# argsim/argsim

Hardware: AMD Instinct MI355X
Metric: sentences/sec per ELBO step (higher is better)
Workload: dtype f32; 1 GPU; BASELINE configs[1]: 1xMI355X fp32, latent_dim 128, vocab 8k, seq_len 64, batch 256 per GPU; FULL synthetic Zipf batches, dim_emb 512, 3 layers, step 20000; global_batch=256, seq_len=64, parallelism=dp1, gru=persistent

## Files before the change

### argsim_amd/csrc/ctx.h

```cpp
#pragma once
#include "../../include/argsim_vae.h"
#include "kernels.h"

#include <fcntl.h>
#include <sys/file.h>
#include <unistd.h>

#include <algorithm>
#include <cmath>
#include <cstdio>
#include <cstring>
#include <string>
#include <vector>

#pragma GCC visibility push(hidden)
namespace avae { namespace host {

struct ParamEntry {
    std::string name;
    int64_t offset;
    int ndim;
    int64_t shape[4];
    int g16;
    int bucket;
};

struct GruP { int64_t W, R, bW, bR; };

}}
#pragma GCC visibility pop

struct avae_ctx {
    avae_config cfg{};
    int device = 0;
    hipStream_t stream = nullptr;
    std::string err;
    std::vector<avae::host::ParamEntry> params;
    int64_t numel = 0;
    std::vector<std::pair<int64_t, int64_t>> buckets;
    float *P = nullptr, *G = nullptr, *M = nullptr, *Vv = nullptr;
    int64_t step = 0;
    avae_grad_hook hook = nullptr; void* hook_user = nullptr;
    std::vector<int> hook_pending;
    int persistent = 1;
    bool first_step_checked = false;
    int gru_ablate = 0, gru_force_slow = 0, gru_stagger = 0, gru_item = 2;
    int skinny = 1;
    int score_plan[4] = {0, 0, 0, 0};
    const int* expect_ptr[3] = {nullptr, nullptr, nullptr}; int expect_val[3] = {0, 0, 0};
    int compact = 2;
    int skip_pad = 1;
    int shared_device = 0; int lock_fd = -1;
    int dyn_split = 1;
    int dyn_thin = 1;
    int enc_top1 = 1;
    int table_l1 = 1;
    int bf16_act = 1;
    int bf16_sv = 1;
    int bf16_tn = 1;
    int logits16 = 1;
    int bf16_nt8 = 1;
    int bf16_direct = 0;
    int gru_spec = 2;
    int bwd_rs = 2;
    int knn_chunk = 0;
    int agg_chunk = 0;
    int ward_form = 0;
    int probe_chunk = 0;
    int gru_bf16 = 1;
    int64_t oE = 0, oKout = 0, oBout = 0, oWmu = 0, oBmu = 0, oWlv = 0, oBlv = 0, oWex = 0, oBex = 0;
    std::vector<avae::host::GruP> enc;
    std::vector<avae::host::GruP> dec;
    float* losses = nullptr;
    float* acc = nullptr;
    int* errw = nullptr;
    unsigned* counters = nullptr;
    float* scratch = nullptr;
    int64_t scratch_n = 0;
    char* ws = nullptr; size_t ws_cap = 0;
    int B = 0, Ss = 0, St = 0;
    int timing = 0, timing_on = 0;
    unsigned short *bfA = nullptr, *bfB = nullptr; size_t bfA_cap = 0, bfB_cap = 0;
    float* slab = nullptr; size_t slab_floats = 0;
    unsigned short* bfP = nullptr; size_t bfP_cap = 0;
    struct Stamp { hipEvent_t a, b; int cls; double flops; const int* dyn; int dyn_max; };
    std::vector<Stamp> stamps; size_t stamps_used = 0;
    int32_t* hint_dev = nullptr; volatile int32_t* hint_host = nullptr;
    const int32_t *cnt_src = nullptr, *cnt_tgt = nullptr;
};

#pragma GCC visibility push(hidden)
namespace avae { namespace host {

#define AV_CHECK(expr)                                                                              \
    do { hipError_t e_ = (expr); if (e_ != hipSuccess) {                                            \
        char b_[512]; snprintf(b_, sizeof b_, "%s:%d: %s -> %s", __FILE__, __LINE__, #expr, hipGetErrorString(e_)); \
        h->err = b_; return 1; } } while (0)
#define AV_TRY(expr) do { int r_ = (expr); if (r_) return r_; } while (0)

inline int fail(avae_ctx* h, const std::string& m) { h->err = m; return 1; }

#define AV_GRU(expr)                                                                                                \
    do { hipError_t e_ = (expr);                                                                                    \
         if (e_ == hipErrorCooperativeLaunchTooLarge)                                                               \
             return fail(h, "persistent GRU kernel: its workgroups cannot all be resident on this device at once (occupancy query x CU count < grid); " \
                            "run with avae_set_option(\"persistent\", 0)");                                         \
         if (e_ != hipSuccess) { char b_[512]; snprintf(b_, sizeof b_, "%s:%d: %s -> %s", __FILE__, __LINE__, #expr, hipGetErrorString(e_)); \
             h->err = b_; return 1; } } while (0)

struct DeviceTurn {
    avae_ctx* h; bool held = false;
    explicit DeviceTurn(avae_ctx* h_) : h(h_) {
        if (!h->shared_device || !h->persistent) return;
        if (h->lock_fd < 0) {
            char path[64]; snprintf(path, sizeof path, "/tmp/argsim_vae_dev%d.lock", h->device);
            h->lock_fd = open(path, O_CREAT | O_RDWR, 0666);
        }
        if (h->lock_fd >= 0 && flock(h->lock_fd, LOCK_EX) == 0) held = true;
    }
    ~DeviceTurn() { if (held) { (void)hipStreamSynchronize(h->stream); (void)flock(h->lock_fd, LOCK_UN); } }
};

struct Timed {
    avae_ctx* h; avae_ctx::Stamp* s = nullptr;
    Timed(avae_ctx* h_, int cls, double flops, const int* dyn = nullptr, int dyn_max = 0) : h(h_) {
        if (!h->timing) return;
        if (h->stamps_used == h->stamps.size()) {
            avae_ctx::Stamp n{};
            if (hipEventCreate(&n.a) != hipSuccess || hipEventCreate(&n.b) != hipSuccess) return;
            h->stamps.push_back(n);
        }
        s = &h->stamps[h->stamps_used++];
        s->cls = cls; s->flops = flops; s->dyn = dyn; s->dyn_max = dyn_max;
        (void)hipEventRecord(s->a, h->stream);
    }
    ~Timed() { if (s) (void)hipEventRecord(s->b, h->stream); }
};

struct Ws {
    int32_t *src_tm, *lens_src, *lens_tgt, *lead, *gold, *rank, *cidx, *ntok, *pred;
    float *emb_src, *emb_tgt, *ew, *dew;
    std::vector<float*> e_gi, e_hs, e_sv[2], e_hp[2];
    std::vector<float*> d_gi, d_hd, d_sv, d_hp;
    float *hpick, *mu, *lv, *z, *eps, *kld, *h0;
    float *xlast, *gib, *svb, *dgib, *dghb, *dxl;
    float *hc, *ho, *logits;
    float *loss_samp, *errt_samp;
    float *dho, *dhc, *dhd[2], *dgi_d, *dgh_d, *dh0, *carry, *dh0sum, *dz, *dmu, *dlv, *dhpick;
    float *dhs[2], *dgi_e, *dgh_e, *demb_src, *demb_tgt;
    std::vector<unsigned short*> e_hs16, d_hd16, e_hp16[2], d_hp16;
    std::vector<char> act_e, act_d, acth_e, acth_d;
    std::vector<unsigned short*> x16_e, x16_d;
    const unsigned short* x16_kept_e(int i) const { return x16_valid ? x16_e[i] : nullptr; }
    const unsigned short* x16_kept_d(int i) const { return x16_valid ? x16_d[i] : nullptr; }
    bool x16_valid = false;
    unsigned short *dgi16_d, *dgh16_d, *dgi16_e, *dgh16_e;
    int32_t* scat;
    int32_t *grp_src, *grp_tgt;
    int32_t *tokrow_src, *tokrow_tgt;
    float* xbuf; size_t xbuf_floats;
    int32_t *ord_perm[3], *ord_slens[3]; int ord_T[3], ord_cpj[3]; bool ord_ok[3];
    int32_t *map_src, *nact_src, *nsrc; bool compact;
    int32_t *map_tgt, *nact_tgt, *ntgt; bool compact_d;
    int Bx;
    int bx_enc() const { return compact ? Bx : 0; }
    int bx_dec() const { return compact_d ? Bx : 0; }
};

struct Bump {
    char* base; size_t off = 0;
    template <class T> T* take(size_t n) {
        off = (off + 255) & ~(size_t)255;
        T* p = base ? reinterpret_cast<T*>(base + off) : nullptr;
        off += n * sizeof(T);
        return p;
    }
    template <class T> T* opt(bool on, size_t n) { return on ? take<T>(n) : nullptr; }
};

struct Pair { const float* A; const float* B; float* C; const float* bias; };

struct GemmCall {
    const float* A; int lda; bool a_mc;
    const float* B; int ldb; bool b_nc;
    float* C; int ldc;
    int M, N, K;
    float alpha = 1.f; const float* bias = nullptr; int accumulate = 0;
    const int* dyn = nullptr; int dyn_kind = 0;
    const Pair* pair = nullptr;
    bool wgrad = false;
    bool allow_atomic = false;
    bool rows_are_batch = false;
    int thin = -1, split_k = 0;
    const unsigned short* A16 = nullptr; const unsigned short* B16 = nullptr;
    unsigned short* keep_a16 = nullptr;
    unsigned short* c16 = nullptr;

    GemmCall& scaled(float a) { alpha = a; return *this; }
    GemmCall& biased(const float* b) { bias = b; return *this; }
    GemmCall& plus() { accumulate = 1; return *this; }
    GemmCall& rows(const int* d) { dyn = d; dyn_kind = d ? 1 : 0; return *this; }
    GemmCall& depth(const int* d) { dyn = d; dyn_kind = d ? 2 : 0; return *this; }
    GemmCall& with(const Pair* p) { pair = p; return *this; }
    GemmCall& atomic() { allow_atomic = true; return *this; }
    GemmCall& batch_rows() { rows_are_batch = true; return *this; }
    GemmCall& form(int thin_, int split_k_ = 1) { thin = thin_; split_k = split_k_; return *this; }
    GemmCall& a16(const unsigned short* p) { A16 = p; return *this; }
    GemmCall& b16(const unsigned short* p) { B16 = p; return *this; }
    GemmCall& keep(unsigned short* p) { keep_a16 = p; return *this; }
};
inline GemmCall nt(const float* A, int lda, const float* B, int ldb, float* C, int ldc, int M, int N, int K) { return GemmCall{A, lda, false, B, ldb, false, C, ldc, M, N, K}; }
inline GemmCall nn(const float* A, int lda, const float* B, int ldb, float* C, int ldc, int M, int N, int K) { return GemmCall{A, lda, false, B, ldb, true, C, ldc, M, N, K}; }
inline GemmCall tn_grad(const float* A, int lda, const float* B, int ldb, float* C, int ldc, int M, int N, int K)
{
    GemmCall c{A, lda, true, B, ldb, true, C, ldc, M, N, K};
    c.wgrad = true;
// ... 59 lines not shown
```

### argsim_amd/csrc/gru.hip

```cpp
#include <algorithm>
#include "kernels.h"
#include "gru_dev.h"
#include <type_traits>

namespace avae {

template <int KS, bool STAMPS>
__global__ __launch_bounds__(256, 2) void gru_fwd_kernel(GruArgs a)
{
    constexpr int D = 16 * KS, HT = KS;
    constexpr int WK = 4 * KS;
    __shared__ __attribute__((aligned(16))) float part[2][2][4][3][256];
    __shared__ __attribute__((aligned(16))) float hps[2][2][16][16];

    const int tid = threadIdx.x, lane = tid & 63, wave = tid >> 6;
    const int n = lane & 15, kh = lane >> 4;
    int jb, g, ht;
    const bool second_half = wg_map(a, HT, &jb, &g, &ht);
    const GruJob& J = a.job[jb];
    const int B = a.B;
    const int row_beg = g * a.rows_per_group;
    const int row_end = min(B, row_beg + a.rows_per_group);
    const int ab = STAMPS ? a.ablate : 0;
    const bool one_sc = row_end - row_beg <= 32;
// ... 185 lines not shown
                 "buffer_load_dwordx4 %5, %8, %9, 0 offen offset:%c15 sc1\n\t"
                 "buffer_load_dwordx4 %6, %8, %9, 0 offen offset:%c16 sc1\n\t"
                 "buffer_load_dwordx4 %7, %8, %9, 0 offen offset:%c17 sc1"
                 : "=&v"(v[0]), "=&v"(v[1]), "=&v"(v[2]), "=&v"(v[3]), "=&v"(v[4]), "=&v"(v[5]), "=&v"(v[6]), "=&v"(v[7])
                 : "v"(voff), "s"(srd), "i"(OFF), "i"(OFF + 64), "i"(OFF + 128), "i"(OFF + 192), "i"(OFF + 256), "i"(OFF + 320),
                   "i"(OFF + 384), "i"(OFF + 448)
                 : "memory");
}
__device__ __forceinline__ void asm_wait8_all(u32x4 (&v)[8])
{
    asm volatile("s_waitcnt vmcnt(0)" : "+v"(v[0]), "+v"(v[1]), "+v"(v[2]), "+v"(v[3]), "+v"(v[4]), "+v"(v[5]), "+v"(v[6]), "+v"(v[7]) :: "memory");
}
__device__ __forceinline__ i32x4 make_srd(const float* p)
{
    const unsigned long long pa = (unsigned long long)p;
    return (i32x4){(int)(unsigned)(pa & 0xffffffffULL), (int)(unsigned)((pa >> 32) & 0xffffULL), -1, 0x00020000};
}

__global__ __launch_bounds__(256, 2) void gru_fwd_item_kernel(GruArgs a)
{
    constexpr int KS = 32, D = 512, HT = 32, WK = 128;
    __shared__ __attribute__((aligned(16))) float part[2][4][3][256];
    __shared__ __attribute__((aligned(16))) float hps[2][16][16];

    const int tid = threadIdx.x, lane = tid & 63, wave = tid >> 6;
    const int n = lane & 15, kh = lane >> 4;
    int jb, g, ht;
    const bool second_half = wg_map(a, HT, &jb, &g, &ht);
    const GruJob& J = a.job[jb];
    const int B = a.B;
    const int row_beg = g * 32;

    const bool bf = a.bf16 != 0;
    float w[3][KS];
#pragma unroll
    for (int gate = 0; gate < 3; ++gate) {
        const float* rp = J.R + (size_t)(ht * 48 + n * 3 + gate) * D + wave * WK;
#pragma unroll
        for (int q = 0; q < KS / 4; ++q) {
            float4 v = *reinterpret_cast<const float4*>(rp + 16 * q + 4 * kh);
            w[gate][4 * q + 0] = opnd(v.x, bf); w[gate][4 * q + 1] = opnd(v.y, bf); w[gate][4 * q + 2] = opnd(v.z, bf); w[gate][4 * q + 3] = opnd(v.w, bf);
        }
    }
    const int gn = tid & 15, gr = tid >> 4;
    const int j = ht * 16 + gn;
    float bR[3];
#pragma unroll
    for (int gate = 0; gate < 3; ++gate) bR[gate] = J.bR[ht * 48 + gn * 3 + gate];
    const int own_wave = (ht * 16) / WK, own_q = ((ht * 16) % WK) / 16;
    int len_a[2] = {0, 0}, len_g[2] = {0, 0};
    if (J.reverse) {
#pragma unroll
        for (int c = 0; c < 2; ++c) { len_a[c] = a.lens[row_beg + 16 * c + n]; len_g[c] = a.lens[row_beg + 16 * c + gr]; }
    }
    const i32x4 srd_hs = make_srd(J.hs), srd_h0 = make_srd(J.h0 ? J.h0 : J.hs);
    const bool fast = group_same_xcd(a.counters + 64 + jb * a.G + g, a.counters + 128 + (jb * a.G + g) * HT, ht, HT, a.err, a.force_slow);
    if (second_half) for (int i = 0; i < a.stagger; ++i) __builtin_amdgcn_s_sleep(32);

    const int total = 2 * (a.p_end - a.p_begin);
    auto item_off = [&](int it, bool* have, bool* from_h0) -> unsigned {
        const int p = a.p_begin + (it >> 1), c = it & 1;
        const int row = row_beg + 16 * c + n;
        *from_h0 = p == 0;
        *have = p > 0 || J.h0 != nullptr;
        if (p == 0) return (unsigned)((size_t)row * D * 4) + (wave * WK + 4 * kh) * 4;
        return (unsigned)((((size_t)pos_map(p - 1, len_a[c], J.reverse) * B + row) * a.ldh) * 4) + (wave * WK + 4 * kh) * 4;
    };
    u32x4 ra[2][8];
    {
        bool have, h0;
        const unsigned off = item_off(0, &have, &h0);
        if (have) asm_issue8<0>(ra[0], off, h0 ? srd_h0 : srd_hs);
        else {
#pragma unroll
            for (int q = 0; q < 8; ++q) ra[0][q] = (u32x4){0u, 0u, 0u, 0u};
        }
    }
    auto item = [&](int p, auto c_tag) __attribute__((always_inline)) {
        constexpr int c = decltype(c_tag)::value, buf = c;
        const int it = 2 * (p - a.p_begin) + c;
        u32x4 (&cur)[8] = ra[c];
        {
            bool have, h0;
            const unsigned off = item_off(it, &have, &h0);
            if (have) {
                asm_wait8_all(cur);
                if (p > a.p_begin) {
                    SpinGuard sg;
                    for (;;) {
                        unsigned mx = 0u;
#pragma unroll
                        for (int q = 0; q < 8; ++q) mx = max(max(mx, max(cur[q].x, cur[q].y)), max(cur[q].z, cur[q].w));
                        if (!__any(mx == kSentinel) || sg.expired(a.err)) break;
                        asm_issue8<0>(cur, off, srd_hs);
                        asm_wait8_all(cur);
                    }
                }
            }
        }
        if (it + 1 < total) {
            bool have, h0;
            const unsigned off = item_off(it + 1, &have, &h0);
            if (have) asm_issue8<0>(ra[c ^ 1], off, h0 ? srd_h0 : srd_hs);
            else {
#pragma unroll
                for (int q = 0; q < 8; ++q) ra[c ^ 1][q] = (u32x4){0u, 0u, 0u, 0u};
            }
        }
        const int grow = row_beg + 16 * c + gr;
        const int gpos = pos_map(p, len_g[c], J.reverse);
        const float* gp = J.gi + ((size_t)gpos * B + grow) * a.ldg + ht * 48 + gn * 3;
        const float gi0 = gp[0], gi1 = gp[1], gi2 = gp[2];
        f32x4 acc[3];
#pragma unroll
        for (int gate = 0; gate < 3; ++gate) acc[gate] = (f32x4){0.f, 0.f, 0.f, 0.f};
#pragma unroll
        for (int ks = 0; ks < KS; ++ks)
#pragma unroll
            for (int gate = 0; gate < 3; ++gate)
                acc[gate] = __builtin_amdgcn_mfma_f32_16x16x4f32(opnd(__uint_as_float(cur[ks >> 2][ks & 3]), bf), w[gate][ks], acc[gate], 0, 0, 0);
#pragma unroll
        for (int gate = 0; gate < 3; ++gate)
            *reinterpret_cast<f32x4*>(&part[buf][wave][gate][lane * 4]) = acc[gate];
        if (wave == own_wave) {
#pragma unroll
            for (int q = 0; q < 8; ++q)
                if (q == own_q) *reinterpret_cast<u32x4*>(&hps[buf][n][4 * kh]) = cur[q];
        }
        __syncthreads();
        {
            const int pidx = ((gr >> 2) * 16 + gn) * 4 + (gr & 3);
            float gh[3];
#pragma unroll
            for (int gate = 0; gate < 3; ++gate)
                gh[gate] = bR[gate] + ((part[buf][0][gate][pidx] + part[buf][1][gate][pidx]) + (part[buf][2][gate][pidx] + part[buf][3][gate][pidx]));
            const float hprev = hps[buf][gr][gn];
            const GruCellOut cell = gru_cell(gi0, gi1, gi2, gh[0], gh[1], gh[2], hprev);
            const float r = cell.r, u = cell.u, nn = cell.n, hnew = cell.h;
            const size_t rix = (size_t)gpos * B + grow;
            float* hdst = J.hs + rix * a.ldh + j;
            if (fast) *hdst = not_sentinel(hnew); else store4_sc1(hdst, not_sentinel(hnew));
            if (J.sv) *reinterpret_cast<float4*>(J.sv + (rix * HT + ht) * 64 + gn * 4) = make_float4(r, u, nn, gh[2]);
            if (J.hp) J.hp[rix * D + j] = hprev;
        }
    };
    for (int p = a.p_begin; p < a.p_end; ++p) {
        item(p, std::integral_constant<int, 0>{});
        item(p, std::integral_constant<int, 1>{});
    }
}


constexpr int kFwdTeamLdsBytes = (96 * 256 + 48 * 256 + 4 * 256) * 4 + 128;
template <bool DIAG, bool PIPE, int T, bool BF = false, bool CMP = false>
__global__ __launch_bounds__(1024, 4) void gru_fwd_team_kernel(GruArgs a)
{
    const int ab = DIAG ? a.ablate : 0;
    constexpr int D = 512, HT = 32, KS = 16 / T, WK = D / KS, NQ = WK / 16, RB = 16 * T;
    extern __shared__ __attribute__((aligned(16))) float lds[];
    float* Wl = lds;
    float* part = Wl + 96 * 256;
    float* hps = part + 48 * 256;
    unsigned* sync = reinterpret_cast<unsigned*>(hps + T * 256);

    const int tid = threadIdx.x, lane = tid & 63, wave = tid >> 6;
    int team, wk;
    if (T == 4 && PIPE && !CMP) { team = wave & 3; wk = wave >> 2; }
    else if (T == 4)         { team = wave >> 2; wk = wave & 3; }
    else if (PIPE && !CMP)   { team = (wave >> 1) & 1; wk = (wave & 1) + 2 * (wave >> 2); }
    else                     { team = (wave >> 2) & 1; wk = (wave & 3) + 4 * (wave >> 3); }
    const int n = lane & 15, kh = lane >> 4;
    const TeamMap tm = team_map(a, RB);
    const int cid = tm.cid, ht = tm.ht;
    const GruJob& J = a.job[tm.jb];
    const int Bs = a.B;
    const int B = (CMP && a.Bx > Bs) ? a.Bx : Bs;
    xcd_publish(a.counters + 64 + cid, a.counters + 128 + cid * HT, ht);

    if constexpr (BF) {
        for (int blk = wave; blk < 48; blk += 16) {
            const int wq = blk / (3 * (NQ / 2)), gate = (blk / (NQ / 2)) % 3, q2 = blk % (NQ / 2);
            const float* rp = J.R + (size_t)(ht * 48 + n * 3 + gate) * D + wq * WK + 32 * q2 + 8 * kh;
            const float4 v0 = *reinterpret_cast<const float4*>(rp), v1 = *reinterpret_cast<const float4*>(rp + 4);
            const u32x4 pk = {pack_bf16(v0.x, v0.y), pack_bf16(v0.z, v0.w), pack_bf16(v1.x, v1.y), pack_bf16(v1.z, v1.w)};
            *reinterpret_cast<u32x4*>(Wl + (size_t)blk * 256 + lane * 4) = pk;
        }
    } else
    for (int blk = wave; blk < 96; blk += 16) {
        const int wq = blk / (3 * NQ), gate = (blk / NQ) % 3, q = blk % NQ;
        const float4 v = *reinterpret_cast<const float4*>(J.R + (size_t)(ht * 48 + n * 3 + gate) * D + wq * WK + 16 * q + 4 * kh);
        *reinterpret_cast<float4*>(Wl + (size_t)blk * 256 + lane * 4) = v;
    }
    if (tid < 2 * T) sync[tid] = 0u;
    const int tt = wk * 64 + lane;
    const bool gate_thread = tt < 256;
    const int gn = tt & 15, gr = (tt >> 4) & 15;
    const int j = ht * 16 + gn;
    float bR[3];
#pragma unroll
    for (int gate = 0; gate < 3; ++gate) bR[gate] = J.bR[ht * 48 + gn * 3 + gate];
    const int own_wk = (ht * 16) / WK, own_q = ((ht * 16) % WK) / 16;
    const float* __restrict__ p_gi = J.gi;
    const int32_t* __restrict__ p_girows = J.gi_rows;
    float* __restrict__ p_svw = J.sv;
    float* __restrict__ p_hpw = J.hp;
    float* __restrict__ p_hsw = J.hs;
    float* const xh = BF ? a.xbuf + (size_t)tm.jb * (a.S + 1) * B * D / 2 : a.xbuf + (size_t)tm.jb * a.S * B * D;
    const __amdgpu_buffer_rsrc_t rs_hs = make_rsrc(xh), rs_h0 = make_rsrc(J.h0 ? J.h0 : xh);
    const __amdgpu_buffer_rsrc_t rs_gi = make_rsrc(p_gi), rs_hsw = make_rsrc(p_hsw);
    const __amdgpu_buffer_rsrc_t rs_svw = make_rsrc(p_svw ? p_svw : p_hsw), rs_hpw = make_rsrc(p_hpw ? p_hpw : p_hsw);
    unsigned short* __restrict__ p_hs16 = BF ? J.hs16 : nullptr;
    unsigned short* __restrict__ p_hp16 = BF ? J.hp16 : nullptr;
    const __amdgpu_buffer_rsrc_t rs_hs16 = make_rsrc(reinterpret_cast<const float*>(p_hs16 ? p_hs16 : reinterpret_cast<unsigned short*>(p_hsw)));
    const __amdgpu_buffer_rsrc_t rs_hp16 = make_rsrc(reinterpret_cast<const float*>(p_hp16 ? p_hp16 : reinterpret_cast<unsigned short*>(p_hsw)));
    auto to_bf16 = [](float v) -> unsigned short { return (unsigned short)(pack_bf16(v, 0.f) & 0xffffu); };
    const bool fast = group_same_xcd(a.counters + 64 + cid, a.counters + 128 + cid * HT, ht, HT, a.err, a.force_slow, true);
    float* tpart = part + team * (KS * 3 * 256);
    float* thps = hps + team * 256;
    unsigned* tsync = sync + team;
    unsigned* ready = sync + T + team;
    unsigned epoch = 0;
    if (ab & 256) { } else {
        const int tq = __builtin_amdgcn_readfirstlane(team);
        if (tq == 0) __builtin_amdgcn_s_setprio(3);
        else if (tq == 1) __builtin_amdgcn_s_setprio(2);
        else if (tq == 2) __builtin_amdgcn_s_setprio(1);
    }

    const bool stamp = (ab & 128) != 0;
    unsigned long long ph[8] = {0, 0, 0, 0, 0, 0, 0, 0}, tprev = __builtin_amdgcn_s_memrealtime();
#define TSTAMP(i) do { if (stamp) { unsigned long long t_ = __builtin_amdgcn_s_memrealtime(); ph[i] += t_ - tprev; tprev = t_; } } while (0)
    unsigned it = 0;
    constexpr int NQA = BF ? NQ / 2 : NQ;
    u32x4 ra[NQA];
    float hc = 0.f, hc0 = 0.f, hc1 = 0.f, hc2 = 0.f, hc3 = 0.f;
    const int* const lens_by_slot = a.slens ? a.slens : a.lens;
    const int* const perm = a.perm;
    auto a_offset = [&](int p, int row0, int len_a) -> unsigned {
        if constexpr (BF) return xch_lane_offset(p == 0 ? 0 : pos_map(p - 1, len_a, J.reverse) + 1, row0, wk * (WK / 8), n, kh, B, D / 2);
        if (p == 0) return (unsigned)((size_t)(CMP ? min(perm ? perm[row0 + n] : row0 + n, Bs - 1) : (perm ? perm[row0 + n] : row0 + n)) * D * 4) + (wk * WK + 4 * kh) * 4;
        return xch_lane_offset(pos_map(p - 1, len_a, J.reverse), row0, wk * (WK / 4), n, kh, B, D);
    };
    auto q_stride = [&](int p) -> unsigned { return (p == 0 && !BF) ? 64u : 1024u; };
    auto next_frag = [&](int p2, int r2, int len2) __attribute__((always_inline)) {
        if (BF || p2 > 0 || J.h0 != nullptr) {
            const int row2 = (tm.slot + r2 * tm.cpj) * RB + team * 16;
            frag_issue<NQA>(ra, (p2 == 0 && !BF) ? rs_h0 : rs_hs, a_offset(p2, row2, len2), q_stride(p2));
        } else {
#pragma unroll
            for (int q = 0; q < NQA; ++q) ra[q] = (u32x4){0u, 0u, 0u, 0u};
        }
    };
    int len_a = J.reverse ? lens_by_slot[tm.slot * RB + team * 16 + n] : 0, len_g = J.reverse ? lens_by_slot[tm.slot * RB + team * 16 + gr] : 0;
    const int len_p0 = J.reverse ? lens_by_slot[tm.slot * RB + team * 16 + 15] : 0;
    int nst0 = a.p_end, nst1 = a.p_end, nst2 = a.p_end, nst3 = a.p_end;
    if (a.slens) {
        nst3 = tm.nrb > 3 ? min(a.p_end, team_steps(a.slens, (tm.slot + 3 * tm.cpj) * RB + team * 16, lane)) : 0;
        nst2 = tm.nrb > 2 ? max(nst3, min(a.p_end, team_steps(a.slens, (tm.slot + 2 * tm.cpj) * RB + team * 16, lane))) : 0;
        nst1 = tm.nrb > 1 ? max(nst2, min(a.p_end, team_steps(a.slens, (tm.slot + 1 * tm.cpj) * RB + team * 16, lane))) : 0;
        nst0 = max(nst1, min(a.p_end, team_steps(a.slens, tm.slot * RB + team * 16, lane)));
    }
    auto nst_of = [&](int r) -> int { return r == 0 ? nst0 : (r == 1 ? nst1 : (r == 2 ? nst2 : nst3)); };
    const int p_stop = nst0;
    int ge_cur = tm.slot * RB + team * 16 + gr;
    if (perm) ge_cur = perm[ge_cur];
    const int* const rowmap = CMP ? a.rowmap : nullptr;
    if (a.slens && gate_thread && !rowmap) {
        for (int r = 0; r < tm.nrb; ++r) {
            const int gs = (tm.slot + r * tm.cpj) * RB + team * 16 + gr, ge = perm ? perm[gs] : gs;
            for (int p = nst_of(r); p < a.p_end; ++p) {
                const unsigned rix = (unsigned)p * (unsigned)Bs + (unsigned)ge;
                if (BF && p_hs16) __builtin_amdgcn_raw_buffer_store_b16((unsigned short)0, rs_hs16, (int)((rix * (unsigned)a.ldh + j) * 2u), 0, 0);
                else bstore1(0.f, rs_hsw, (rix * (unsigned)a.ldh + j) * 4u);
                if (BF && p_hp16) __builtin_amdgcn_raw_buffer_store_b16((unsigned short)0, rs_hp16, (int)((rix * D + j) * 2u), 0, 0);
                else if (p_hpw) bstore1(0.f, rs_hpw, (rix * D + j) * 4u);
            }
        }
    }
    if constexpr (PIPE) { if (a.p_begin < p_stop) next_frag(a.p_begin, 0, len_a); }
    for (int p = a.p_begin; p < p_stop; ++p) {
      for (int r = 0; r < tm.nrb && p < nst_of(r); ++r, ++it) {
        TSTAMP(5);
        const int row0 = (tm.slot + r * tm.cpj) * RB + team * 16;
        const bool poll = p > a.p_begin && !(ab & 16);
        const int grow = row0 + gr;
        const int gpos = pos_map(p, len_g, J.reverse);
        const unsigned prix = (unsigned)gpos * (unsigned)Bs + (unsigned)ge_cur;
        const int crow = (rowmap && gate_thread) ? (ge_cur < Bs ? rowmap[prix] : -1) : (int)prix;
        const bool real = !CMP || crow >= 0;
        const unsigned rix = (unsigned)crow;
        float gi0 = 0.f, gi1 = 0.f, gi2 = 0.f, h0_own = 0.f;
        if (gate_thread && real) {
            const unsigned grix = p_girows ? (unsigned)p_girows[prix] : rix;
            const u32x3 g3 = __builtin_amdgcn_raw_buffer_load_b96(rs_gi, (int)((grix * (unsigned)a.ldg + ht * 48 + gn * 3) * 4u), 0, 0);
            gi0 = __uint_as_float(g3.x); gi1 = __uint_as_float(g3.y); gi2 = __uint_as_float(g3.z);
            if constexpr (BF) { if (p == 0 && J.h0 != nullptr) h0_own = bload1(rs_h0, ((unsigned)ge_cur * D + j) * 4u); }
        }
        const bool same_p = r + 1 < tm.nrb && p < nst_of(r + 1);
        const int r2 = same_p ? r + 1 : 0, p2 = same_p ? p : p + 1;
        int len2 = len_a, len2g = len_g, ge2 = ge_cur;
        if constexpr (PIPE) {
            if (p2 < p_stop) {
                const int row2 = (tm.slot + r2 * tm.cpj) * RB + team * 16;
                if (J.reverse) { len2 = lens_by_slot[row2 + n]; len2g = lens_by_slot[row2 + gr]; }
                ge2 = perm ? perm[row2 + gr] : row2 + gr;
            }
        }
        const bool have = BF || p > 0 || J.h0 != nullptr;
        if (have) {
            const unsigned aoff = a_offset(p, row0, len_a);
            const __amdgpu_buffer_rsrc_t rs = (p == 0 && !BF) ? rs_h0 : rs_hs;
            if constexpr (!PIPE) {
                bool got = false;
                if (poll && a.spec) {
                    frag_issue<NQA>(ra, rs, aoff, q_stride(p));
                    if constexpr (BF) got = !frag_bad16<NQA>(ra); else got = !frag_bad<NQA>(ra);
                }
                if (poll) {
                    if (wk == 0) {
                        if (!got) {
                        const int prow = row0 + 15;
                        const int plen = len_p0;
                        const float* pp = BF ? xh + (xch16_index(pos_map(p - 1, plen, J.reverse) + 1, prow, (lane & 31) * 16 + 15, B, D) >> 1)
                                             : xh + xch_index(pos_map(p - 1, plen, J.reverse), prow, (lane & 31) * 16 + 15, B, D);
                        SpinGuard sg;
                        while (__any(BF ? (load4_sc1(pp) >> 16) == 0xffffu : load4_sc1(pp) == kSentinel) && !sg.expired(a.err)) { }
                        }
                        if (lane == 0) __hip_atomic_store(ready, it + 1u, __ATOMIC_RELAXED, __HIP_MEMORY_SCOPE_WORKGROUP);
                    } else if (!got) {
                        while (__hip_atomic_load(ready, __ATOMIC_RELAXED, __HIP_MEMORY_SCOPE_WORKGROUP) < it + 1u) __builtin_amdgcn_s_sleep(1);
                    }
                }
                if (!got) frag_issue<NQA>(ra, rs, aoff, q_stride(p));
            }
            if (poll) { if constexpr (BF) frag_ensure16<NQA>(ra, rs, aoff, a.err, q_stride(p)); else frag_ensure<NQA>(ra, rs, aoff, a.err, q_stride(p)); }
        } else if constexpr (!PIPE) {
#pragma unroll
            for (int q = 0; q < NQA; ++q) ra[q] = (u32x4){0u, 0u, 0u, 0u};
        }
        TSTAMP(0);
        f32x4 acc[3];
#pragma unroll
        for (int gate = 0; gate < 3; ++gate) acc[gate] = (f32x4){0.f, 0.f, 0.f, 0.f};
        if constexpr (BF) {
#pragma unroll
            for (int q2 = 0; q2 < NQ / 2; ++q2) {
                const bf16x8 a8 = __builtin_bit_cast(bf16x8, ra[q2]);
#pragma unroll
                for (int gate = 0; gate < 3; ++gate) {
                    const bf16x8 b8 = __builtin_bit_cast(bf16x8, *reinterpret_cast<const u32x4*>(Wl + (size_t)((wk * 3 + gate) * (NQ / 2) + q2) * 256 + lane * 4));
                    acc[gate] = __builtin_amdgcn_mfma_f32_16x16x32_bf16(a8, b8, acc[gate], 0, 0, 0);
                }
            }
        } else
        {
            f32x4 bn[3];
#pragma unroll
            for (int gate = 0; gate < 3; ++gate)
                bn[gate] = *reinterpret_cast<const f32x4*>(Wl + (size_t)((wk * 3 + gate) * NQ + 0) * 256 + lane * 4);
#pragma unroll
            for (int q = 0; q < NQ; ++q) {
                f32x4 b[3];
#pragma unroll
                for (int gate = 0; gate < 3; ++gate) b[gate] = bn[gate];
                if (q + 1 < NQ) {
#pragma unroll
                    for (int gate = 0; gate < 3; ++gate)
                        bn[gate] = *reinterpret_cast<const f32x4*>(Wl + (size_t)((wk * 3 + gate) * NQ + q + 1) * 256 + lane * 4);
                }
                __builtin_amdgcn_sched_barrier(0);
#pragma unroll
                for (int e = 0; e < 4; ++e)
#pragma unroll
                    for (int gate = 0; gate < 3; ++gate)
                        acc[gate] = __builtin_amdgcn_mfma_f32_16x16x4f32(__uint_as_float(ra[q][e]), b[gate][e], acc[gate], 0, 0, 0);
                __builtin_amdgcn_sched_barrier(0);
            }
        }
        TSTAMP(1);
        if (it > 0) { epoch += KS; team_barrier(tsync, epoch); }
        TSTAMP(6);
#pragma unroll
        for (int gate = 0; gate < 3; ++gate)
            *reinterpret_cast<f32x4*>(tpart + (wk * 3 + gate) * 256 + lane * 4) = acc[gate];
        if constexpr (!BF) {
            if (wk == own_wk) {
#pragma unroll
                for (int q = 0; q < NQ; ++q)
                    if (q == own_q) *reinterpret_cast<u32x4*>(thps + n * 16 + 4 * kh) = ra[q];
            }
        }
        if constexpr (PIPE) {
            asm volatile("" :: "v"(gi0), "v"(gi1), "v"(gi2), "v"(h0_own), "v"(len2), "v"(len2g), "v"(ge2));
            __builtin_amdgcn_sched_barrier(0);
            if (p2 < p_stop) next_frag(p2, r2, len2);
            __builtin_amdgcn_sched_barrier(0);
        }
        TSTAMP(7);
        epoch += KS; team_barrier(tsync, epoch);
        TSTAMP(2);
        if (gate_thread) {
            const int pidx = ((gr >> 2) * 16 + gn) * 4 + (gr & 3);
            float gh[3];
#pragma unroll
            for (int gate = 0; gate < 3; ++gate) {
                float s4[4] = {0.f, 0.f, 0.f, 0.f};
#pragma unroll
                for (int k = 0; k < KS; ++k) s4[k & 3] += tpart[(k * 3 + gate) * 256 + pidx];
                gh[gate] = bR[gate] + ((s4[0] + s4[1]) + (s4[2] + s4[3]));
            }
            float hprev;
            if constexpr (BF) {
                if (p == 0) hprev = h0_own;
                else if constexpr (PIPE) hprev = r == 0 ? hc0 : (r == 1 ? hc1 : (r == 2 ? hc2 : hc3));
                else hprev = hc;
            } else hprev = thps[gr * 16 + gn];
            const GruCellOut cell = gru_cell(gi0, gi1, gi2, gh[0], gh[1], gh[2], hprev);
            const float r_ = cell.r, u = cell.u, nn = cell.n, hnew = cell.h;
            if constexpr (BF) {
                const unsigned xo = xch16_index(gpos + 1, grow, j, B, D) * 2u;
                if (fast) __builtin_amdgcn_raw_buffer_store_b16(bf16_not_sentinel(hnew), rs_hs, (int)xo, 0, 0);
                else __builtin_amdgcn_raw_buffer_store_b16(bf16_not_sentinel(hnew), rs_hs, (int)xo, 0, 16);
                if constexpr (PIPE) { if (r == 0) hc0 = hnew; else if (r == 1) hc1 = hnew; else if (r == 2) hc2 = hnew; else hc3 = hnew; }
                else hc = hnew;
            } else {
                const unsigned xo = xch_index(gpos, grow, j, B, D) * 4u;
                if (fast) bstore1(not_sentinel(hnew), rs_hs, xo); else bstore1_sc1(not_sentinel(hnew), rs_hs, xo);
            }
            if (real) {
            if (BF && p_hs16) __builtin_amdgcn_raw_buffer_store_b16(to_bf16(hnew), rs_hs16, (int)((rix * (unsigned)a.ldh + j) * 2u), 0, 0);
            else bstore1(hnew, rs_hsw, (rix * (unsigned)a.ldh + j) * 4u);
            if (p_svw) {
                if (BF && a.sv16) {
                    typedef unsigned u32x2 __attribute__((ext_vector_type(2)));
                    const u32x2 s2 = {pack_bf16(r_, u), pack_bf16(nn, gh[2])};
                    __builtin_amdgcn_raw_buffer_store_b64(s2, rs_svw, (int)(((rix * HT + ht) * 64 + gn * 4) * 2u), 0, 0);
                } else bstore4(r_, u, nn, gh[2], rs_svw, ((rix * HT + ht) * 64 + gn * 4) * 4u);
            }
            if (BF && p_hp16) __builtin_amdgcn_raw_buffer_store_b16(to_bf16(hprev), rs_hp16, (int)((rix * D + j) * 2u), 0, 0);
            else if (p_hpw) bstore1(hprev, rs_hpw, (rix * D + j) * 4u);
            }
        }
        len_a = len2; len_g = len2g; ge_cur = ge2;
        TSTAMP(3);
      }
    }
    if (stamp && tt == 0 && a.stamps) {
        for (int i = 0; i < 8; ++i) atomicAdd(a.stamps + i, ph[i]);
        atomicAdd(a.stamps + 8, (unsigned long long)(a.p_end - a.p_begin));
        atomicAdd(a.stamps + 10, 1ULL);
    }
#undef TSTAMP
}

template <int KS, bool STAMPS>
__global__ __launch_bounds__(256, 2) void gru_bwd_kernel(GruArgs a)
{
    constexpr int D = 16 * KS, HT = KS, NKS = 3 * KS;
    __shared__ __attribute__((aligned(16))) float part[2][2][4][256];
    __shared__ float red[4][16];

    const int tid = threadIdx.x, lane = tid & 63, wave = tid >> 6;
    const int n = lane & 15, kh = lane >> 4;
    int jb, g, ht;
    const bool second_half = wg_map(a, HT, &jb, &g, &ht);
    const GruJob& J = a.job[jb];
    const int B = a.B, S = a.S;
    const int row_beg = g * a.rows_per_group;
    const int row_end = min(B, row_beg + a.rows_per_group);
    const int ab = STAMPS ? a.ablate : 0;
    const bool one_sc = row_end - row_beg <= 32;

    const bool bf = a.bf16 != 0;
    float w[NKS];
#pragma unroll
    for (int ks = 0; ks < NKS; ++ks)
        w[ks] = opnd(J.R[(size_t)(wave * 12 * KS + kperm<NKS>(ks, kh)) * D + ht * 16 + n], bf);

    const int gn = tid & 15, gr = tid >> 4;
    const int j = ht * 16 + gn;
    int len_a[2] = {0, 0}, len_g[2] = {0, 0};
    if (J.reverse) {
#pragma unroll
        for (int c = 0; c < 2; ++c) {
            len_a[c] = a.lens[min(row_beg + 16 * c + n, B - 1)];
            len_g[c] = a.lens[min(row_beg + 16 * c + gr, B - 1)];
        }
    }
    const bool want_dh0 = (J.dh0 != nullptr) && a.p_begin == 0;
    const int p_last = want_dh0 ? -1 : a.p_begin;
    const __amdgpu_buffer_rsrc_t rs_dgh = make_rsrc(J.dgh);
    float sb_r = 0.f, sb_u = 0.f, sb_n = 0.f, sb_nr = 0.f;
    bool fast = false;
    if (a.p_end - 1 > p_last && !(ab & 16))
        fast = group_same_xcd(a.counters + 64 + jb * a.G + g, a.counters + 128 + (jb * a.G + g) * HT, ht, HT, a.err, a.force_slow);
    if (second_half && a.p_end - 1 > p_last) for (int i = 0; i < a.stagger; ++i) __builtin_amdgcn_s_sleep(32);
    int buf = 0, done = 0;
    unsigned long long ph[8] = {0, 0, 0, 0, 0, 0, 0, 0}, tprev = __builtin_amdgcn_s_memrealtime();
    for (int p = a.p_end - 1; p >= p_last; --p, ++done) {
        const bool have_next = (p + 1 < S);
        const bool poll = done > 0 && !(ab & 16);
        for (int rb = row_beg; rb < row_end; rb += 32, buf ^= 1) {
            AVAE_STAMP(7);
            float s_r[2], s_u[2], s_n[2], s_hn[2], s_hp[2], s_do[2]; int rix[2]; bool gok[2];
#pragma unroll
            for (int c = 0; c < 2; ++c) {
                const int row = rb + 16 * c + gr;
                gok[c] = row < row_end && p >= 0;
                rix[c] = 0; s_r[c] = s_u[c] = s_n[c] = s_hn[c] = s_hp[c] = s_do[c] = 0.f;
                if (gok[c]) {
                    const int len = J.reverse ? (one_sc ? len_g[c] : a.lens[row]) : 0;
                    rix[c] = pos_map(p, len, J.reverse) * B + row;
                    if (!(ab & 2)) {
                        const float4 sv = *reinterpret_cast<const float4*>(J.sv + ((size_t)rix[c] * HT + ht) * 64 + gn * 4);
                        s_r[c] = sv.x; s_u[c] = sv.y; s_n[c] = sv.z; s_hn[c] = sv.w;
                        s_hp[c] = J.hp[(size_t)rix[c] * D + j];
                        if (J.dh_out) s_do[c] = J.dh_out[(size_t)rix[c] * a.ldh + j];
                    }
                }
            }
            AVAE_STAMP(0);
            const bool c1 = rb + 16 < row_end;
            constexpr int NH = (NKS % 16 == 0) ? 4 : ((NKS % 8 == 0) ? 2 : 1);
            constexpr int HK = NKS / NH;
            constexpr int PQ = (NKS % 4 == 0) ? HK / 4 : 1;
            constexpr int NB = 3;
            u32x4 hv[NB][PQ];
            float hs_[HK];
            auto piece_off = [&](int c, int hf) -> unsigned {
                const int row = min(rb + 16 * c + n, B - 1);
                const int len = J.reverse ? (one_sc ? len_a[c] : a.lens[row]) : 0;
                const int pos1 = pos_map(p + 1, len, J.reverse);
                return (unsigned)((((size_t)pos1 * B + row) * a.ldg + wave * 12 * KS + hf * 4 * HK) * 4);
            };
            const bool do_mm = have_next && !(ab & 1);
            const int nstage = (c1 ? 2 : 1) * NH;
            f32x4 acc[4];
            if constexpr (KS == 32) {
                if (!do_mm) {
#pragma unroll
                    for (int c = 0; c < 2; ++c)
                        if (c == 0 || c1) *reinterpret_cast<f32x4*>(&part[buf][c][wave][lane * 4]) = (f32x4){0.f, 0.f, 0.f, 0.f};
                } else {
                    const unsigned long long pa = (unsigned long long)J.dgh;
                    const i32x4 srd = {(int)(unsigned)(pa & 0xffffffffULL), (int)(unsigned)((pa >> 32) & 0xffffULL), -1, 0x00020000};
                    const unsigned voff0 = piece_off(0, 0) + 16 * kh, voff1 = c1 ? piece_off(1, 0) + 16 * kh : voff0;
                    auto pass = [&](auto nst_tag) __attribute__((always_inline)) -> bool {
                        constexpr int NST = decltype(nst_tag)::value;
                        unsigned mx = 0u;
                        asm_issue6<0>(hv[0], voff0, srd);
                        asm_issue6<384>(hv[1], voff0, srd);
#pragma unroll
                        for (int st = 0; st < NST; ++st) {
                            const int c = st / NH, hf = st % NH;
                            if (st + 2 < NST) {
                                const unsigned vo = ((st + 2) / NH) ? voff1 : voff0;
                                if ((st + 2) % NH == 0) asm_issue6<0>(hv[(st + 2) % NB], vo, srd);
                                if ((st + 2) % NH == 1) asm_issue6<384>(hv[(st + 2) % NB], vo, srd);
                                if ((st + 2) % NH == 2) asm_issue6<768>(hv[(st + 2) % NB], vo, srd);
                                if ((st + 2) % NH == 3) asm_issue6<1152>(hv[(st + 2) % NB], vo, srd);
                            }
                            if (st + 2 < NST) asm_wait6<12>(hv[st % NB]);
                            else if (st + 1 < NST) asm_wait6<6>(hv[st % NB]);
                            else asm_wait6<0>(hv[st % NB]);
                            if (hf == 0) {
#pragma unroll
                                for (int i = 0; i < 4; ++i) acc[i] = (f32x4){0.f, 0.f, 0.f, 0.f};
                            }
#pragma unroll
                            for (int q = 0; q < PQ; ++q)
                                mx = max(max(mx, max(hv[st % NB][q].x, hv[st % NB][q].y)), max(hv[st % NB][q].z, hv[st % NB][q].w));
                            asm volatile("" : "+v"(mx));
#pragma unroll
                            for (int ks = 0; ks < HK; ++ks)
                                acc[ks & 3] = __builtin_amdgcn_mfma_f32_16x16x4f32(opnd(__uint_as_float(hv[st % NB][ks >> 2][ks & 3]), bf),
                                                                                   w[ks + hf * HK], acc[ks & 3], 0, 0, 0);
                            if (hf == NH - 1) {
                                f32x4 s = (acc[0] + acc[1]) + (acc[2] + acc[3]);
                                *reinterpret_cast<f32x4*>(&part[buf][c][wave][lane * 4]) = s;
                            }
                        }
                        return __any(mx == kSentinel);
                    };
                    SpinGuard sg;
                    for (;;) {
                        if (poll) {
                            const int pc = c1 ? (lane >> 5) : 0, prow = min(min(rb + 16 * pc + 15, row_end - 1), B - 1);
                            const int plen = J.reverse ? a.lens[prow] : 0;
                            const float* pp = J.dgh + ((size_t)pos_map(p + 1, plen, J.reverse) * B + prow) * a.ldg + (lane & 31) * 48 + 47;
                            while (__any(load4_sc1(pp) == kSentinel) && !sg.expired(a.err)) { }
                        }
                        const bool bad = c1 ? pass(std::integral_constant<int, 2 * NH>{}) : pass(std::integral_constant<int, NH>{});
                        if (!poll || !bad || sg.expired(a.err)) break;
                    }
                }
            } else {
            if constexpr (NKS % 4 == 0) {
                if (do_mm) {
#pragma unroll
                    for (int s0 = 0; s0 < NB - 1; ++s0)
                        if (s0 < nstage) frag_issue<PQ>(hv[s0], rs_dgh, piece_off(s0 / NH, s0 % NH) + 16 * kh);
                }
            }
#pragma unroll
            for (int c = 0; c < 2; ++c) {
#pragma unroll
                for (int hf = 0; hf < NH; ++hf) {
                    const int st = c * NH + hf;
                    if (st < nstage) {
                        if (hf == 0) {
#pragma unroll
                            for (int i = 0; i < 4; ++i) acc[i] = (f32x4){0.f, 0.f, 0.f, 0.f};
                        }
                        if (do_mm) {
                            if constexpr (NKS % 4 == 0) {
                                if (st + NB - 1 < nstage)
                                    frag_issue<PQ>(hv[(st + NB - 1) % NB], rs_dgh, piece_off((st + NB - 1) / NH, (st + NB - 1) % NH) + 16 * kh);
                                if (poll) frag_ensure<PQ>(hv[st % NB], rs_dgh, piece_off(c, hf) + 16 * kh, a.err);
#pragma unroll
                                for (int ks = 0; ks < HK; ++ks)
                                    acc[ks & 3] = __builtin_amdgcn_mfma_f32_16x16x4f32(opnd(__uint_as_float(hv[st % NB][ks >> 2][ks & 3]), bf),
                                                                                       w[ks + hf * HK], acc[ks & 3], 0, 0, 0);
                            } else {
                                load_frag_scalar<HK, NKS>(hs_, J.dgh + piece_off(c, 0) / 4, hf * HK, kh, poll, a.err);
#pragma unroll
                                for (int ks = 0; ks < HK; ++ks)
                                    acc[ks & 3] = __builtin_amdgcn_mfma_f32_16x16x4f32(opnd(hs_[ks], bf), w[ks + hf * HK], acc[ks & 3], 0, 0, 0);
                            }
                        }
                        if (hf == NH - 1) {
                            f32x4 s = (acc[0] + acc[1]) + (acc[2] + acc[3]);
                            *reinterpret_cast<f32x4*>(&part[buf][c][wave][lane * 4]) = s;
                        }
                    }
                }
            }
            }
            AVAE_STAMP(2);
            __syncthreads();
            AVAE_STAMP(3);
            float o_dr[2], o_du[2], o_dn[2], o_car[2];
#pragma unroll
            for (int c = 0; c < 2; ++c) {
                const int row = rb + 16 * c + gr;
                if (row >= row_end) continue;
                const int pidx = ((gr >> 2) * 16 + gn) * 4 + (gr & 3);
                float carried = (part[buf][c][0][pidx] + part[buf][c][1][pidx]) + (part[buf][c][2][pidx] + part[buf][c][3][pidx]);
                float* carryp = J.carry + (size_t)row * D + j;
                if (have_next) carried += *carryp;
                if (p < 0) { J.dh0[(size_t)row * D + j] = carried; continue; }
                const float dH = carried + s_do[c];
                const float r = s_r[c], u = s_u[c], nn = s_n[c];
                const float dn = dH * (1.f - u) * (1.f - nn * nn);
                const float du = dH * (s_hp[c] - nn) * u * (1.f - u);
                const float dr = dn * s_hn[c] * r * (1.f - r);
                float* dgh = J.dgh + (size_t)rix[c] * a.ldg + ht * 48 + gn * 3;
                const float x0 = not_sentinel(dr), x1 = not_sentinel(du), x2 = not_sentinel(dn * r);
                if (fast) { dgh[0] = x0; dgh[1] = x1; dgh[2] = x2; }
                else { store4_sc1(dgh, x0); store4_sc1(dgh + 1, x1); store4_sc1(dgh + 2, x2); }
                o_dr[c] = dr; o_du[c] = du; o_dn[c] = dn; o_car[c] = dH * u;
                sb_r += dr; sb_u += du; sb_n += dn; sb_nr += dn * r;
            }
            AVAE_STAMP(4);
            if (p >= 0) {
#pragma unroll
                for (int c = 0; c < 2; ++c) {
                    const int row = rb + 16 * c + gr;
                    if (row >= row_end) continue;
                    J.carry[(size_t)row * D + j] = o_car[c];
                    if (!(ab & 4)) {
                        float* dgi = J.dgi + (size_t)rix[c] * a.ldg + ht * 48 + gn * 3;
                        dgi[0] = o_dr[c]; dgi[1] = o_du[c]; dgi[2] = o_dn[c];
                    }
                }
            }
            AVAE_STAMP(6);
        }
    }
    if (STAMPS && tid == 0 && a.stamps) {
        for (int i = 0; i < 8; ++i) atomicAdd(a.stamps + 16 + i, ph[i]);
        atomicAdd(a.stamps + 16 + 8, (unsigned long long)(a.p_end - a.p_begin));
        atomicAdd(a.stamps + 16 + 9, (unsigned long long)(fast ? 1 : 0));
        atomicAdd(a.stamps + 16 + 10, 1ULL);
    }
    if (J.dbW || J.dbR) {
        if (tid < 64) red[tid >> 4][tid & 15] = 0.f;
        __syncthreads();
        atomicAdd(&red[0][gn], sb_r); atomicAdd(&red[1][gn], sb_u); atomicAdd(&red[2][gn], sb_n); atomicAdd(&red[3][gn], sb_nr);
        __syncthreads();
        if (tid < 48) {
            const int gate = tid >> 4, u = tid & 15;
            if (J.dbW) atomicAdd(J.dbW + ht * 48 + u * 3 + gate, red[gate][u]);
            if (J.dbR) atomicAdd(J.dbR + ht * 48 + u * 3 + gate, red[gate == 2 ? 3 : gate][u]);
        }
    }
}

constexpr int kBwdTeamLdsBytes = (4 * 24 * 256 + 16 * 256 + 64) * 4 + 64;
template <int NB, bool PIPE, int T, bool DIAG = false, bool BF = false, bool CMP = false>
__global__ __launch_bounds__(1024, 4) void gru_bwd_team_kernel(GruArgs a)
{
    unsigned long long ph[8] = {0, 0, 0, 0, 0, 0, 0, 0}, tprev = DIAG ? __builtin_amdgcn_s_memrealtime() : 0ULL;
#define BSTAMP(i) do { if constexpr (DIAG) { unsigned long long t_ = __builtin_amdgcn_s_memrealtime(); ph[i] += t_ - tprev; tprev = t_; } } while (0)
    constexpr int D = 512, HT = 32, PQ = 6, KS = 16 / T, WKB = 3 * D / KS, KPL = BF ? 32 : 16, NH = WKB / (PQ * KPL), KB4 = 96 / KS, RB = 16 * T;
    extern __shared__ __attribute__((aligned(16))) float lds[];
    float* Wl = lds;
    float* part = Wl + 96 * 256;
    float* red = part + 16 * 256;
    unsigned* sync = reinterpret_cast<unsigned*>(red + 64);

    const int tid = threadIdx.x, lane = tid & 63, wave = tid >> 6;
    int team, wk;
    if (T == 4 && PIPE && !CMP) { team = wave & 3; wk = wave >> 2; }
    else if (T == 4)         { team = wave >> 2; wk = wave & 3; }
    else if (PIPE && !CMP)   { team = (wave >> 1) & 1; wk = (wave & 1) + 2 * (wave >> 2); }
    else                     { team = wave >> 3; wk = wave & 7; }
    const int n = lane & 15, kh = lane >> 4;
    const TeamMap tm = team_map(a, RB);
    const int cid = tm.cid, ht = tm.ht;
    const GruJob& J = a.job[tm.jb];
    const int Bs = a.B, S = a.S;
    const int B = (CMP && a.Bx > Bs) ? a.Bx : Bs;
    xcd_publish(a.counters + 64 + cid, a.counters + 128 + cid * HT, ht);

    auto r_row = [&](int kx) -> const float* { const int rem = kx % 48; return J.R + (size_t)((kx - rem) + (rem & 15) * 3 + (rem >> 4)) * D + ht * 16 + n; };
    if constexpr (BF) {
        for (int blk = wave; blk < 48; blk += 16) {
            const int wq = blk / (KB4 / 2), kp = blk % (KB4 / 2);
            const float* r0 = r_row(wq * WKB + 32 * kp + 8 * kh);
            const u32x4 pk = {pack_bf16(r0[0], r0[3 * D]), pack_bf16(r0[6 * D], r0[9 * D]), pack_bf16(r0[12 * D], r0[15 * D]), pack_bf16(r0[18 * D], r0[21 * D])};
            *reinterpret_cast<u32x4*>(Wl + (size_t)blk * 256 + lane * 4) = pk;
        }
    } else
    for (int blk = wave; blk < 96; blk += 16) {
        const int wq = blk / KB4, ks4 = blk % KB4;
        const float* rp = r_row(wq * WKB + 16 * ks4 + 4 * kh);
        *reinterpret_cast<float4*>(Wl + (size_t)blk * 256 + lane * 4) = make_float4(rp[0], rp[3 * D], rp[6 * D], rp[9 * D]);
    }
    if (tid < 2 * T) sync[tid] = 0u;
    if (tid < 64) red[tid] = 0.f;
    const int tt = wk * 64 + lane, gn = tt & 15, gr = (tt >> 4) & 15;
    const bool gate_thread = tt < 256;
    const int j = ht * 16 + gn;
    unsigned long long tp0 = 0, tp1 = 0;
    if constexpr (DIAG) { asm volatile("s_waitcnt vmcnt(0) lgkmcnt(0)" ::: "memory"); tp0 = __builtin_amdgcn_s_memrealtime(); }
    const bool fast = group_same_xcd(a.counters + 64 + cid, a.counters + 128 + cid * HT, ht, HT, a.err, a.force_slow, true);
    if constexpr (DIAG) {
        tp1 = __builtin_amdgcn_s_memrealtime();
        if (tt == 0 && a.stamps && ((a.ablate & 256) ? T == 2 : T == 4)) {
            atomicAdd(a.stamps + 16 + 11, tp0 - tprev);
            atomicAdd(a.stamps + 16 + 12, tp1 - tp0);
        }
    }
    float* tpart = part + team * (KS * 256);
    unsigned* tsync = sync + team;
    unsigned* ready = sync + T + team;
    unsigned epoch = 0;
    {
        const int tq = __builtin_amdgcn_readfirstlane(team);
        if (tq == 0) __builtin_amdgcn_s_setprio(3);
        else if (tq == 1) __builtin_amdgcn_s_setprio(2);
        else if (tq == 2) __builtin_amdgcn_s_setprio(1);
    }
    const float* __restrict__ p_sv = J.sv;
    const float* __restrict__ p_hp = J.hp;
    const float* __restrict__ p_do = J.dh_out;
    float* __restrict__ p_dgi = J.dgi;
    float* __restrict__ p_dghw = J.dgh;
    unsigned short* __restrict__ p_dgi16 = BF ? J.dgi16 : nullptr;
    unsigned short* __restrict__ p_dgh16 = BF ? J.dgh16 : nullptr;
    float* p_dh0 = J.dh0;
    float* p_carry = J.carry;
    const int* p_lens = a.slens ? a.slens : a.lens;
    const int* const perm = a.perm;
    int* p_err = a.err;
    const int j_rev = J.reverse, ldg = a.ldg, ldh = a.ldh;
    float* const xg = a.xbuf + (size_t)tm.jb * S * B * (3 * D) / (BF ? 2 : 1);
    const unsigned long long pa = (unsigned long long)xg;
    const i32x4 srd = {(int)(unsigned)(pa & 0xffffffffULL), (int)(unsigned)((pa >> 32) & 0xffffULL), -1, 0x00020000};
    float sb_r = 0.f, sb_u = 0.f, sb_n = 0.f, sb_nr = 0.f;
    const bool want_dh0 = (p_dh0 != nullptr) && a.p_begin == 0;
    const int p_last = want_dh0 ? -1 : a.p_begin;
    int done = 0;
    unsigned it = 0;
    float carry_reg = 0.f;
    float carry_r0 = 0.f, carry_r1 = 0.f, carry_r2 = 0.f, carry_r3 = 0.f;
    u32x4 hv[NB][PQ];
    const __amdgpu_buffer_rsrc_t rs_dgh = make_rsrc(xg);
    const __amdgpu_buffer_rsrc_t rs_sv = make_rsrc(p_sv), rs_hp = make_rsrc(p_hp), rs_do = make_rsrc(p_do ? p_do : p_hp);
    const unsigned short* __restrict__ p_hp16 = BF ? J.hp16 : nullptr;
    const __amdgpu_buffer_rsrc_t rs_hp16 = make_rsrc(reinterpret_cast<const float*>(p_hp16 ? p_hp16 : reinterpret_cast<const unsigned short*>(p_hp)));
    const __amdgpu_buffer_rsrc_t rs_dgi = make_rsrc(p_dgi), rs_dghw = make_rsrc(p_dghw);
    const __amdgpu_buffer_rsrc_t rs_dgi16 = make_rsrc(reinterpret_cast<const float*>(p_dgi16 ? p_dgi16 : reinterpret_cast<unsigned short*>(p_dgi)));
    const __amdgpu_buffer_rsrc_t rs_dgh16 = make_rsrc(reinterpret_cast<const float*>(p_dgh16 ? p_dgh16 : reinterpret_cast<unsigned short*>(p_dghw)));
    auto a_offset = [&](int p, int row0, int len_a) -> unsigned {
        if constexpr (BF) return xch_lane_offset(pos_map(p + 1, len_a, j_rev), row0, wk * (WKB / 8), n, kh, B, 3 * D / 2);
        return xch_lane_offset(pos_map(p + 1, len_a, j_rev), row0, wk * (WKB / 4), n, kh, B, 3 * D);
    };
    auto issue_piece = [&](int piece, u32x4 (&dst)[PQ], unsigned vo) __attribute__((always_inline)) {
        asm_issue6x(dst, vo, srd, 6144 * piece, 6144 * piece + 4096);
    };
    auto head = [&](unsigned vo) __attribute__((always_inline)) {
#pragma unroll
        for (int s0 = 0; s0 < NB && s0 < NH; ++s0) issue_piece(s0, hv[s0], vo);
    };
    int nst0 = a.p_end, nst1 = a.p_end, nst2 = a.p_end, nst3 = a.p_end;
    if (a.slens) {
        nst3 = tm.nrb > 3 ? min(a.p_end, team_steps(a.slens, (tm.slot + 3 * tm.cpj) * RB + team * 16, lane)) : 0;
        nst2 = tm.nrb > 2 ? max(nst3, min(a.p_end, team_steps(a.slens, (tm.slot + 2 * tm.cpj) * RB + team * 16, lane))) : 0;
        nst1 = tm.nrb > 1 ? max(nst2, min(a.p_end, team_steps(a.slens, (tm.slot + 1 * tm.cpj) * RB + team * 16, lane))) : 0;
        nst0 = max(nst1, min(a.p_end, team_steps(a.slens, tm.slot * RB + team * 16, lane)));
    }
    auto nst_of = [&](int r) -> int { return r == 0 ? nst0 : (r == 1 ? nst1 : (r == 2 ? nst2 : nst3)); };
    auto next_head = [&](int p2, int r2, int len2) __attribute__((always_inline)) {
        if (p2 + 1 < nst_of(r2)) {
            const int row2 = (tm.slot + r2 * tm.cpj) * RB + team * 16;
            const unsigned vo2 = a_offset(p2, row2, len2);
#pragma unroll
            for (int s0 = 0; s0 < NB && s0 < NH; ++s0)
#pragma unroll
                for (int q = 0; q < PQ; ++q) hv[s0][q] = load16_sc1(rs_dgh, vo2 + 6144u * s0 + 1024u * q);
        }
    };
    int len_a = j_rev ? p_lens[tm.slot * RB + team * 16 + n] : 0, len_g = j_rev ? p_lens[tm.slot * RB + team * 16 + gr] : 0;
    const int len_p0 = j_rev ? p_lens[tm.slot * RB + team * 16 + 15] : 0;
    int ge_cur = tm.slot * RB + team * 16 + gr;
    if (perm) ge_cur = perm[ge_cur];
    const int* const rowmap = CMP ? a.rowmap : nullptr;
    const bool dgi_by_pos = rowmap != nullptr && J.dgi_by_pos != 0;
    if (a.slens && gate_thread && (!rowmap || dgi_by_pos)) {
        for (int r = 0; r < tm.nrb; ++r) {
            const int gs = (tm.slot + r * tm.cpj) * RB + team * 16 + gr, ge = perm ? perm[gs] : gs;
            if (CMP && ge >= Bs) continue;
            for (int p = nst_of(r); p < a.p_end; ++p) {
                const unsigned orow = (((unsigned)p * (unsigned)Bs + (unsigned)ge) * (unsigned)ldg + ht * 48 + gn * 3) * 4u;
                if (BF && p_dgh16 != nullptr) {
                    if ((gn & 1) == 0) {
                        const u32x3 z3 = {0u, 0u, 0u};
                        if (!rowmap) __builtin_amdgcn_raw_buffer_store_b96(z3, rs_dgh16, (int)(orow >> 1), 0, 0);
                        if (p_dgi16 != nullptr) __builtin_amdgcn_raw_buffer_store_b96(z3, rs_dgi16, (int)(orow >> 1), 0, 0);
                    }
                    if (p_dgi16 == nullptr) bstore3(0.f, 0.f, 0.f, rs_dgi, orow);
                } else { if (!rowmap) bstore3(0.f, 0.f, 0.f, rs_dghw, orow); bstore3(0.f, 0.f, 0.f, rs_dgi, orow); }
            }
        }
    }
    const int p_first = nst0 - 1;
    if constexpr (PIPE) next_head(p_first, 0, len_a);
    for (int p = p_first; p >= p_last; --p, ++done) {
      for (int r = 0; r < tm.nrb && (p < 0 || p < nst_of(r)); ++r, ++it) {
        const int row0 = (tm.slot + r * tm.cpj) * RB + team * 16;
        int gn_l = gn, gr_l = gr, ln_l = lane;
        asm volatile("" : "+v"(gn_l), "+v"(gr_l), "+v"(ln_l));
        const int grow = row0 + gr_l, j_l = ht * 16 + gn_l;
        const bool have_next = p + 1 < nst_of(r);
        const bool poll = done > 0 && !(DIAG && (a.ablate & 16));
        const bool same_p = r + 1 < tm.nrb && (p < 0 || p < nst_of(r + 1));
        const int r2 = same_p ? r + 1 : 0, p2 = same_p ? p : p - 1;
        int len2 = len_a, len2g = len_g, ge2 = ge_cur;
        if constexpr (PIPE) {
            if (p2 >= p_last) {
                const int row2 = (tm.slot + r2 * tm.cpj) * RB + team * 16;
                if (j_rev) { len2 = p_lens[row2 + n]; len2g = p_lens[row2 + gr]; }
                ge2 = perm ? perm[row2 + gr] : row2 + gr;
            }
        }
        BSTAMP(7);
        const int gpos = pos_map(p < 0 ? 0 : p, len_g, j_rev);
        const unsigned prix = (unsigned)gpos * (unsigned)Bs + (unsigned)ge_cur;
        const bool inb = !CMP || ge_cur < Bs;
        const int crow = (rowmap && gate_thread && p >= 0) ? (inb ? rowmap[prix] : -1) : (int)prix;
        const bool real = !CMP || crow >= 0;
        const unsigned rix = (unsigned)crow;
        float4 sv = make_float4(0.f, 0.f, 0.f, 0.f); float s_hp = 0.f, s_do = 0.f;
        if (p >= 0 && gate_thread && real) {
            if (BF && a.sv16) {
                typedef unsigned u32x2 __attribute__((ext_vector_type(2)));
                const u32x2 s2 = __builtin_amdgcn_raw_buffer_load_b64(rs_sv, (int)(((rix * HT + ht) * 64 + gn_l * 4) * 2u), 0, 0);
                sv = make_float4(__uint_as_float(s2.x << 16), __uint_as_float(s2.x & 0xffff0000u), __uint_as_float(s2.y << 16), __uint_as_float(s2.y & 0xffff0000u));
            } else
            sv = bload4(rs_sv, ((rix * HT + ht) * 64 + gn_l * 4) * 4u);
            if (BF && p_hp16) s_hp = __uint_as_float((unsigned)(unsigned short)__builtin_amdgcn_raw_buffer_load_b16(rs_hp16, (int)((rix * D + j_l) * 2u), 0, 0) << 16);
            else s_hp = bload1(rs_hp, (rix * D + j_l) * 4u);
            s_do = p_do ? bload1(rs_do, (rix * (unsigned)ldh + j_l) * 4u) : 0.f;
        }
        float* carryp = p_carry + (size_t)grow * D + j_l;
        float s_carry = 0.f;
        if constexpr (PIPE) {
            if (done == 0 && have_next && gate_thread) { const float c0 = *carryp; if (r == 0) carry_r0 = c0; else if (r == 1) carry_r1 = c0; else if (r == 2) carry_r2 = c0; else carry_r3 = c0; }
            s_carry = r == 0 ? carry_r0 : (r == 1 ? carry_r1 : (r == 2 ? carry_r2 : carry_r3));
        }
        else { if (done == 0 && have_next && gate_thread) carry_reg = *carryp; }
        BSTAMP(0);
        f32x4 sum = {0.f, 0.f, 0.f, 0.f};
        if (have_next) {
            const unsigned voff = a_offset(p, row0, len_a);
            f32x4 acc[2];
            auto pass = [&]() __attribute__((always_inline)) -> bool {
                unsigned mx = 0u;
                auto ldsB = [&](int st_, int q_) __attribute__((always_inline)) {
                    return *reinterpret_cast<const f32x4*>(Wl + (size_t)((wk * KB4 + st_ * 6 + q_) * 64 + lane) * 4);
                };
                f32x4 bq = {0.f, 0.f, 0.f, 0.f};
                if constexpr (!BF) bq = ldsB(0, 0);
#pragma unroll
                for (int st = 0; st < NH; ++st) {
                    const int issued = (NB + st < NH) ? NB + st : NH;
                    const int younger = issued - 1 - st;
                    if (younger == 2) asm_wait6<12>(hv[st % NB]);
                    else if (younger == 1) asm_wait6<6>(hv[st % NB]);
                    else asm_wait6<0>(hv[st % NB]);
                    if (st == 0) { acc[0] = (f32x4){0.f, 0.f, 0.f, 0.f}; acc[1] = (f32x4){0.f, 0.f, 0.f, 0.f}; }
#pragma unroll
                    for (int q = 0; q < PQ; ++q) {
                        if constexpr (BF) mx = pk_max_u16(pk_max_u16(mx, pk_max_u16(hv[st % NB][q].x, hv[st % NB][q].y)), pk_max_u16(hv[st % NB][q].z, hv[st % NB][q].w));
                        else mx = max(max(mx, max(hv[st % NB][q].x, hv[st % NB][q].y)), max(hv[st % NB][q].z, hv[st % NB][q].w));
                    }
                    asm volatile("" : "+v"(mx));
                    if constexpr (BF) {
#pragma unroll
                        for (int q = 0; q < PQ; ++q) {
                            const bf16x8 b8 = __builtin_bit_cast(bf16x8, *reinterpret_cast<const u32x4*>(Wl + (size_t)((wk * (KB4 / 2) + st * PQ + q) * 64 + lane) * 4));
                            acc[q & 1] = __builtin_amdgcn_mfma_f32_16x16x32_bf16(__builtin_bit_cast(bf16x8, hv[st % NB][q]), b8, acc[q & 1], 0, 0, 0);
                        }
                    } else
#pragma unroll
                    for (int q = 0; q < PQ; ++q) {
                        const f32x4 b = bq;
                        if (q + 1 < PQ) bq = ldsB(st, q + 1); else if (st + 1 < NH) bq = ldsB(st + 1, 0);
                        __builtin_amdgcn_sched_barrier(0);
#pragma unroll
                        for (int e = 0; e < 4; ++e)
                            acc[e & 1] = __builtin_amdgcn_mfma_f32_16x16x4f32(__uint_as_float(hv[st % NB][q][e]), b[e], acc[e & 1], 0, 0, 0);
                        __builtin_amdgcn_sched_barrier(0);
                    }
                    if (st + NB < NH) issue_piece(st + NB, hv[st % NB], voff);
                }
                sum = acc[0] + acc[1];
                if constexpr (BF) return __any(any_half_sentinel(mx));
                return __any(mx == kSentinel);
            };
            auto probe = [&](SpinGuard& sg) __attribute__((always_inline)) {
                const int len_p = PIPE ? (j_rev ? p_lens[row0 + 15] : 0) : len_p0;
                const float* pp = BF ? xg + (xch16_index(pos_map(p + 1, len_p, j_rev), row0 + 15, (ln_l & 31) * 48 + 47, B, 3 * D) >> 1)
                                     : xg + xch_index(pos_map(p + 1, len_p, j_rev), row0 + 15, (ln_l & 31) * 48 + 47, B, 3 * D);
                for (;;) {
                    unsigned v = 0u;
                    if (ln_l < 32) v = load4_sc1(pp);
                    if (!__any(BF ? (v >> 16) == 0xffffu : v == kSentinel) || sg.expired(p_err)) break;
                }
            };
            SpinGuard sg;
            if constexpr (!PIPE) {
                if (poll) {
                    if (wk == 0) {
                        probe(sg);
                        if (lane == 0) __hip_atomic_store(ready, it + 1u, __ATOMIC_RELAXED, __HIP_MEMORY_SCOPE_WORKGROUP);
                    } else {
                        while (__hip_atomic_load(ready, __ATOMIC_RELAXED, __HIP_MEMORY_SCOPE_WORKGROUP) < it + 1u) __builtin_amdgcn_s_sleep(1);
                    }
                }
                head(voff);
            }
            BSTAMP(1);
            for (;;) {
                const bool bad = pass();
                if (!poll || !bad || sg.expired(p_err)) break;
                probe(sg);
                head(voff);
            }
        }
        if constexpr (PIPE) {
            asm volatile("" :: "v"(sv.x), "v"(sv.y), "v"(sv.z), "v"(sv.w), "v"(s_hp), "v"(s_do), "v"(s_carry), "v"(len2), "v"(len2g), "v"(ge2));
            __builtin_amdgcn_sched_barrier(0);
            if (p2 >= p_last) next_head(p2, r2, len2);
            __builtin_amdgcn_sched_barrier(0);
        }
        BSTAMP(2);
        if (it > 0) { epoch += KS; team_barrier(tsync, epoch); }
        BSTAMP(3);
        *reinterpret_cast<f32x4*>(tpart + wk * 256 + lane * 4) = sum;
        BSTAMP(4);
        epoch += KS; team_barrier(tsync, epoch);
        BSTAMP(5);
        if (gate_thread) {
            const int pidx = ((gr >> 2) * 16 + gn) * 4 + (gr & 3);
            float s4[4] = {0.f, 0.f, 0.f, 0.f};
#pragma unroll
            for (int k = 0; k < KS; ++k) s4[k & 3] += tpart[k * 256 + pidx];
            float carried = (s4[0] + s4[1]) + (s4[2] + s4[3]);
            if constexpr (PIPE) carried += s_carry;
            else if (have_next) carried += carry_reg;
            if (p < 0) { if (inb) p_dh0[(size_t)ge_cur * D + j_l] = carried; len_a = len2; len_g = len2g; ge_cur = ge2; continue; }
            const float dH = carried + s_do;
            const float r_ = sv.x, u = sv.y, nn = sv.z;
            const float dn = dH * (1.f - u) * (1.f - nn * nn);
            const float du = dH * (s_hp - nn) * u * (1.f - u);
            const float dr = dn * sv.w * r_ * (1.f - r_);
            if constexpr (BF) {
                const unsigned short x0 = bf16_not_sentinel(dr), x1 = bf16_not_sentinel(du), x2 = bf16_not_sentinel(dn * r_);
                const unsigned o0 = xch16_index(gpos, grow, ht * 48 + gn_l, B, 3 * D) * 2u;
                if (fast) {
                    __builtin_amdgcn_raw_buffer_store_b16(x0, rs_dgh, (int)o0, 0, 0); __builtin_amdgcn_raw_buffer_store_b16(x1, rs_dgh, (int)(o0 + 512u), 0, 0);
                    __builtin_amdgcn_raw_buffer_store_b16(x2, rs_dgh, (int)(o0 + 1024u), 0, 0);
                } else {
                    __builtin_amdgcn_raw_buffer_store_b16(x0, rs_dgh, (int)o0, 0, 16); __builtin_amdgcn_raw_buffer_store_b16(x1, rs_dgh, (int)(o0 + 512u), 0, 16);
                    __builtin_amdgcn_raw_buffer_store_b16(x2, rs_dgh, (int)(o0 + 1024u), 0, 16);
                }
            } else {
                const float x0 = not_sentinel(dr), x1 = not_sentinel(du), x2 = not_sentinel(dn * r_);
                const unsigned o0 = xch_index(gpos, grow, ht * 48 + gn_l, B, 3 * D) * 4u;
                if (fast) { bstore1(x0, rs_dgh, o0); bstore1(x1, rs_dgh, o0 + 1024u); bstore1(x2, rs_dgh, o0 + 2048u); }
                else { bstore1_sc1(x0, rs_dgh, o0); bstore1_sc1(x1, rs_dgh, o0 + 1024u); bstore1_sc1(x2, rs_dgh, o0 + 2048u); }
            }
            const unsigned orow = (rix * (unsigned)ldg + ht * 48 + gn_l * 3) * 4u;
            const unsigned orow_i = dgi_by_pos ? (prix * (unsigned)ldg + ht * 48 + gn_l * 3) * 4u : orow;
            if (BF && p_dgh16 != nullptr) {
                const float dnr = dn * r_;
                const float o_r = __int_as_float(__builtin_amdgcn_update_dpp(0, __float_as_int(dr), 0xF5, 0xF, 0xF, false));
                const float o_u = __int_as_float(__builtin_amdgcn_update_dpp(0, __float_as_int(du), 0xF5, 0xF, 0xF, false));
                const float o_n = __int_as_float(__builtin_amdgcn_update_dpp(0, __float_as_int(dn), 0xF5, 0xF, 0xF, false));
                const float o_nr = __int_as_float(__builtin_amdgcn_update_dpp(0, __float_as_int(dnr), 0xF5, 0xF, 0xF, false));
                if ((gn_l & 1) == 0) {
                    const u32x3 vh = {pack_bf16(dr, du), pack_bf16(dnr, o_r), pack_bf16(o_u, o_nr)};
                    const u32x3 vi = {pack_bf16(dr, du), pack_bf16(dn, o_r), pack_bf16(o_u, o_n)};
                    if (real) __builtin_amdgcn_raw_buffer_store_b96(vh, rs_dgh16, (int)(orow >> 1), 0, 0);
                    if (p_dgi16 != nullptr && (real || (dgi_by_pos && inb))) __builtin_amdgcn_raw_buffer_store_b96(vi, rs_dgi16, (int)(orow_i >> 1), 0, 0);
                }
                if (p_dgi16 == nullptr && (real || (dgi_by_pos && inb))) bstore3(dr, du, dn, rs_dgi, orow_i);
                if constexpr (PIPE) { const float c1 = dH * u; if (r == 0) carry_r0 = c1; else if (r == 1) carry_r1 = c1; else if (r == 2) carry_r2 = c1; else carry_r3 = c1; }
                else carry_reg = dH * u;
            } else {
            if (real) bstore3(dr, du, dn * r_, rs_dghw, orow);
            if constexpr (PIPE) { const float c1 = dH * u; if (r == 0) carry_r0 = c1; else if (r == 1) carry_r1 = c1; else if (r == 2) carry_r2 = c1; else carry_r3 = c1; }
            else carry_reg = dH * u;
            if (real || (dgi_by_pos && inb)) bstore3(dr, du, dn, rs_dgi, orow_i);
            }
            sb_r += dr; sb_u += du; sb_n += dn; sb_nr += dn * r_;
        }
        len_a = len2; len_g = len2g; ge_cur = ge2;
        BSTAMP(6);
      }
    }
    if (gate_thread && p_last >= 0 && a.p_end - 1 >= p_last) {
        if constexpr (!PIPE) p_carry[(size_t)(tm.slot * RB + team * 16 + gr) * D + j] = carry_reg;
        else
            for (int r = 0; r < tm.nrb; ++r)
                p_carry[(size_t)((tm.slot + r * tm.cpj) * RB + team * 16 + gr) * D + j] = r == 0 ? carry_r0 : (r == 1 ? carry_r1 : (r == 2 ? carry_r2 : carry_r3));
    }
    if constexpr (DIAG) {
        if (tt == 0 && a.stamps && ((a.ablate & 256) ? T == 2 : T == 4)) {
            for (int i = 0; i < 8; ++i) atomicAdd(a.stamps + 16 + i, ph[i]);
            atomicAdd(a.stamps + 16 + 8, (unsigned long long)(a.p_end - a.p_begin));
            atomicAdd(a.stamps + 16 + 10, 1ULL);
        }
    }
#undef BSTAMP
    if (J.dbW || J.dbR) {
        atomicAdd(&red[gn], sb_r); atomicAdd(&red[16 + gn], sb_u); atomicAdd(&red[32 + gn], sb_n); atomicAdd(&red[48 + gn], sb_nr);
        __syncthreads();
        if (tid < 48) {
            const int gate = tid >> 4, u = tid & 15;
            if (J.dbW) atomicAdd(J.dbW + ht * 48 + u * 3 + gate, red[gate * 16 + u]);
            if (J.dbR) atomicAdd(J.dbR + ht * 48 + u * 3 + gate, red[(gate == 2 ? 3 : gate) * 16 + u]);
        }
    }
}

__global__ __launch_bounds__(256) void gru_first_step_fwd_kernel(const float* __restrict__ gi, const float* __restrict__ bR, float* __restrict__ h_out,
                                                                 int ldo, float* __restrict__ sv, int B, int D, const int32_t* __restrict__ lens)
{
    const int i = blockIdx.x * blockDim.x + threadIdx.x;
    if (i >= B * D) return;
    const int b = i / D, j = i - b * D, c = (j >> 4) * 48 + (j & 15) * 3;
    const float* g = gi + (size_t)b * 3 * D + c;
    const bool live = !lens || lens[b] > 0;
    const GruCellOut cell = gru_cell(g[0], g[1], g[2], bR[c], bR[c + 1], bR[c + 2], 0.f);
    h_out[(size_t)b * ldo + j] = live ? cell.h : 0.f;
    if (sv) *reinterpret_cast<float4*>(sv + ((size_t)b * D + j) * 4) = make_float4(cell.r, cell.u, cell.n, bR[c + 2]);
}
hipError_t gru_first_step_fwd(hipStream_t st, const float* gi, const float* bR, float* h_out, int ldo, float* sv, int B, int D, const int32_t* lens)
{
    hipLaunchKernelGGL(gru_first_step_fwd_kernel, dim3((B * D + 255) / 256), dim3(256), 0, st, gi, bR, h_out, ldo, sv, B, D, lens);
    return hipGetLastError();
}
__global__ __launch_bounds__(256) void gru_first_step_bwd_kernel(const float* __restrict__ dh, int ldd, const float* __restrict__ sv,
                                                                 float* __restrict__ dgi, float* __restrict__ dgh, int B, int D, const int32_t* __restrict__ lens)
{
    const int i = blockIdx.x * blockDim.x + threadIdx.x;
    if (i >= B * D) return;
    const int b = i / D, j = i - b * D, c = (j >> 4) * 48 + (j & 15) * 3;
    const float4 s = *reinterpret_cast<const float4*>(sv + ((size_t)b * D + j) * 4);
    const float dH = (!lens || lens[b] > 0) ? dh[(size_t)b * ldd + j] : 0.f;
    const float r_ = s.x, u = s.y, nn = s.z;
    const float dn = dH * (1.f - u) * (1.f - nn * nn);
    const float du = dH * (0.f - nn) * u * (1.f - u);
    const float dr = dn * s.w * r_ * (1.f - r_);
    float* a = dgi + (size_t)b * 3 * D + c; float* g = dgh + (size_t)b * 3 * D + c;
    a[0] = dr; a[1] = du; a[2] = dn;
    g[0] = dr; g[1] = du; g[2] = dn * r_;
}
hipError_t gru_first_step_bwd(hipStream_t st, const float* dh, int ldd, const float* sv, float* dgi, float* dgh, int B, int D, const int32_t* lens)
{
    hipLaunchKernelGGL(gru_first_step_bwd_kernel, dim3((B * D + 255) / 256), dim3(256), 0, st, dh, ldd, sv, dgi, dgh, B, D, lens);
    return hipGetLastError();
}

constexpr int kGruSyncWords = 64 + 64 + 1536;
bool gru_dim_supported(int D) { return D == 16 || D == 32 || D == 64 || D == 128 || D == 256 || D == 512; }

#ifdef AVAE_DIAG
constexpr bool kDiagBuild = true;
#else
constexpr bool kDiagBuild = false;
#endif
bool gru_diag_build() { return kDiagBuild; }

template <bool FWD, int KSV, bool DIAG>
static hipError_t launch_ks(hipStream_t st, const GruArgs& a, int grid, bool need_resident)
{
    auto kernel = [] { if constexpr (FWD) return gru_fwd_kernel<KSV, DIAG>; else return gru_bwd_kernel<KSV, DIAG>; }();
    if (need_resident) { hipError_t e = resident(kernel, 256, 0, grid); if (e != hipSuccess) return e; }
    hipLaunchKernelGGL(kernel, dim3(grid), dim3(256), 0, st, a);
    return hipGetLastError();
}
template <bool FWD>
static hipError_t launch(hipStream_t st, const GruArgs& a, int grid, bool need_resident)
{
#ifdef AVAE_DIAG
#define AVAE_GRU_CASE(KSV) case KSV: return a.ablate ? launch_ks<FWD, KSV, true>(st, a, grid, need_resident) : launch_ks<FWD, KSV, false>(st, a, grid, need_resident);
#else
#define AVAE_GRU_CASE(KSV) case KSV: return launch_ks<FWD, KSV, false>(st, a, grid, need_resident);
#endif
    switch (a.D / 16) {
        AVAE_GRU_CASE(1)
        AVAE_GRU_CASE(2)
        AVAE_GRU_CASE(4)
        AVAE_GRU_CASE(8)
        AVAE_GRU_CASE(16)
        AVAE_GRU_CASE(32)
        default: return hipErrorInvalidValue;
    }
#undef AVAE_GRU_CASE
}

static hipError_t check(const GruArgs& a, int* grid)
{
    if (!gru_dim_supported(a.D) || a.njobs < 1 || a.njobs > kMaxGruJobs) return hipErrorInvalidValue;
    if (a.rows_per_group % 16 || a.G * a.rows_per_group < a.B) return hipErrorInvalidValue;
    if (!kDiagBuild && a.ablate) return hipErrorInvalidValue;
    *grid = a.njobs * a.G * (a.D / 16);
    return hipSuccess;
}

__global__ __launch_bounds__(256) void gru_prepare_kernel(unsigned* sync_words, int nsync, uint4* buf, size_t n16)
{
    const size_t stride = (size_t)gridDim.x * blockDim.x;
    size_t i = (size_t)blockIdx.x * blockDim.x + threadIdx.x;
    if (i < (size_t)nsync) sync_words[i] = 0u;
    const uint4 s4 = make_uint4(kSentinel, kSentinel, kSentinel, kSentinel);
    for (; i < n16; i += stride) buf[i] = s4;
}
struct GruH0 { const float* p[kMaxGruJobs]; };
__global__ __launch_bounds__(256) void gru_prepare16_kernel(unsigned* sync_words, int nsync, uint4* buf, size_t n16, size_t chunks_per_job,
                                                            size_t seed_chunks, GruH0 h0s, int D, const int* perm, int ext_rows)
{
    const size_t stride = (size_t)gridDim.x * blockDim.x;
    size_t i = (size_t)blockIdx.x * blockDim.x + threadIdx.x;
    if (i < (size_t)nsync) sync_words[i] = 0u;
    const uint4 s4 = make_uint4(kSentinel, kSentinel, kSentinel, kSentinel);
    for (; i < n16; i += stride) {
        const size_t job = i / chunks_per_job, c = i - job * chunks_per_job;
        uint4 v = s4;
        if (c < seed_chunks) {
            v = make_uint4(0u, 0u, 0u, 0u);
            const float* h0 = h0s.p[job];
            if (h0) {
                const size_t rb = c / ((size_t)(D >> 3) * 16), rem = c - rb * ((size_t)(D >> 3) * 16);
                const size_t k8 = rem >> 4, slot = rb * 16 + (rem & 15), row = perm ? (size_t)perm[slot] : slot;
                if (row < (size_t)ext_rows) {
                const float4 a0 = *reinterpret_cast<const float4*>(h0 + row * D + k8 * 8), a1 = *reinterpret_cast<const float4*>(h0 + row * D + k8 * 8 + 4);
                v = make_uint4(pack_bf16(a0.x, a0.y), pack_bf16(a0.z, a0.w), pack_bf16(a1.x, a1.y), pack_bf16(a1.z, a1.w));
                }
            }
        }
        buf[i] = v;
    }
}
static hipError_t fill_sentinel2d(hipStream_t st, float* base, size_t rows, size_t width, size_t ld)
{
    return hipMemset2DAsync(base, ld * sizeof(float), 0xFF, width * sizeof(float), rows, st);
}

static hipError_t prepare_exchange(hipStream_t st, const GruArgs& a, bool fwd, const GruPlan& p)
{
    const bool team = p.form == GruForm::team, bf = team && a.bf16 && !p.diag;
    const size_t Bg = p.Bg;
    const size_t rows = (size_t)a.S * Bg, width = fwd ? a.D : 3 * (size_t)a.D, ld = fwd ? a.ldh : a.ldg;
    if (bf && fwd) {
        GruH0 h0s{};
        for (int i = 0; i < a.njobs; ++i) h0s.p[i] = a.job[i].h0;
        const size_t chunks_per_job = ((size_t)a.S + 1) * Bg * a.D / 8;
        hipLaunchKernelGGL(gru_prepare16_kernel, dim3(2048), dim3(256), 0, st, a.counters, kGruSyncWords, reinterpret_cast<uint4*>(a.xbuf),
                           (size_t)a.njobs * chunks_per_job, chunks_per_job, Bg * a.D / 8, h0s, a.D, a.perm, a.B);
        return hipGetLastError();
    }
    if (team) {
        const size_t n16 = (size_t)a.njobs * rows * width / 4;
        hipLaunchKernelGGL(gru_prepare_kernel, dim3(2048), dim3(256), 0, st, a.counters, kGruSyncWords,
                           reinterpret_cast<uint4*>(a.xbuf), bf ? n16 / 2 : n16);
        return hipGetLastError();
    }
    float* base0 = fwd ? a.job[0].hs : a.job[0].dgh;
    bool side_by_side = (size_t)a.njobs * width == ld && (((uintptr_t)base0) & 15) == 0 && ((rows * ld) & 3) == 0;
    for (int i = 0; i < a.njobs && side_by_side; ++i)
        side_by_side = (fwd ? a.job[i].hs : a.job[i].dgh) == base0 + i * width;
    if (side_by_side) {
        hipLaunchKernelGGL(gru_prepare_kernel, dim3(2048), dim3(256), 0, st, a.counters, kGruSyncWords,
                           reinterpret_cast<uint4*>(base0), rows * ld / 4);
        return hipGetLastError();
    }
    hipError_t e = hipMemsetAsync(a.counters, 0, sizeof(unsigned) * kGruSyncWords, st);
    for (int i = 0; i < a.njobs && e == hipSuccess; ++i)
        e = fill_sentinel2d(st, fwd ? a.job[i].hs : a.job[i].dgh, rows, width, ld);
    return e;
}

static bool team_rows(int njobs, int B, int* T, int* C)
{
    for (int t = 4; t >= 2; t >>= 1) {
        const int rb = 16 * t;
        if (B % rb) continue;
        const int nrbj = B / rb, np = njobs * nrbj;
        if (np < 8) continue;
        if (np == 8) { *T = t; *C = 8; return true; }
        const int cpj = 8 / njobs;
        if (nrbj % cpj || nrbj / cpj > 4) continue;
        *T = t; *C = 8;
        return true;
    }
    for (int i = 0; i < 2; ++i) {
        const int t = (njobs == 2) == (i == 0) ? 4 : 2, rb = 16 * t;
        if (B % rb == 0 && njobs * (B / rb) <= 8) { *T = t; *C = njobs * (B / rb); return true; }
    }
    return false;
}
int gru_team_batch(int B)
{
    int T = 0, C = 0;
    for (int bx = (B + 15) / 16 * 16; bx <= B + 256; bx += 16)
        if (team_rows(1, bx, &T, &C) && team_rows(2, bx, &T, &C)) return bx;
    return 0;
}
static bool team_geometry(const GruArgs& a, bool fwd, int Bg, int* T, int* C)
{
    if (a.D != 512 || a.njobs > 2 || a.p_begin != 0) return false;
    const size_t per_job = (size_t)a.S * Bg * a.D * (fwd ? 1 : 3);
    if (!a.xbuf || (((uintptr_t)a.xbuf) & 15) || a.xbuf_floats < per_job * a.njobs || per_job * 4 >= (1ull << 32)) return false;
    const size_t widest = std::max<size_t>((size_t)std::max(a.ldg, a.ldh), (size_t)4 * a.D);
    if ((size_t)a.S * a.B * widest * 4 >= (1ull << 32)) return false;
    return team_rows(a.njobs, Bg, T, C);
}

GruPlan gru_plan(const GruArgs& a, bool fwd, bool persistent)
{
    GruPlan p{};
    p.Bg = a.Bx > a.B ? a.Bx : a.B;
    if (!persistent || (fwd && a.p_end - a.p_begin < 2)) { p.form = GruForm::stepwise; return p; }
    const bool ablate_ok = !a.ablate || (kDiagBuild && !(a.ablate & ~(16 | 128 | 256)));
    int T = 0, C = 0;
    if (!(team_geometry(a, fwd, p.Bg, &T, &C) && a.item_pipeline == 2 && ablate_ok && (!fwd || !a.ablate || T == 4))) {
        const bool item = fwd && a.D == 512 && a.rows_per_group == 32 && a.B % 32 == 0 && a.G * 32 == a.B && !a.ablate && a.item_pipeline;
        p.form = item ? GruForm::item : GruForm::persistent;
        return p;
    }
    const bool rs = !fwd && a.bwd_rs && !a.bf16 && !a.ablate && a.p_end == a.S && a.xbuf_floats >= gru_bwd_rs_xbuf_floats(a.njobs, p.Bg);
    p.form = rs ? GruForm::team_rs : GruForm::team;
    p.T = T; p.C = C; p.cpj = C / a.njobs;
    p.pipe = a.njobs * (p.Bg / (16 * T)) > C;
    p.diag = kDiagBuild && (fwd ? a.ablate != 0 : (a.ablate & 128) != 0);
    return p;
}

static hipError_t check_operands(const GruArgs& a, const GruPlan& p, bool fwd)
{
    const bool team = p.team(), bf = p.full() && a.bf16;
    bool ok = (!a.sv16 || bf) && (!(a.rowmap || a.Bx > a.B) || p.full())
              && (a.Bx <= a.B || (a.slens && a.perm && a.rowmap));
    for (int i = 0; i < a.njobs; ++i) {
        const GruJob& j = a.job[i];
        ok = ok && (!j.hp16 || bf) && (fwd ? (!j.hs16 || bf) && (!j.gi_rows || team) : (!(j.dgi16 || j.dgh16) || bf));
    }
    return ok ? hipSuccess : hipErrorInvalidValue;
}

hipError_t gru_forward(hipStream_t st, const GruArgs& a, bool persistent)
{
    int grid; hipError_t e = check(a, &grid); if (e != hipSuccess) return e;
    const GruPlan p = gru_plan(a, true, persistent);
    e = check_operands(a, p, true); if (e != hipSuccess) return e;
    if (p.form == GruForm::stepwise) {
        for (int q = a.p_begin; q < a.p_end; ++q) {
            GruArgs b = a; b.p_begin = q; b.p_end = q + 1;
            e = launch<true>(st, b, grid, false); if (e != hipSuccess) return e;
        }
        return hipSuccess;
    }
    e = prepare_exchange(st, a, true, p); if (e != hipSuccess) return e;
    switch (p.form) {
    case GruForm::team: {
        return team_dispatch(p.T, [&](auto T, auto PIPE, auto BF, auto CMP) {
            if constexpr (kDiagBuild && T == 4 && !BF && !CMP) if (p.diag) return launch_team(st, gru_fwd_team_kernel<true, PIPE, 4>, a, kFwdTeamLdsBytes, p.C);
            return launch_team(st, gru_fwd_team_kernel<false, PIPE, T, BF, CMP>, a, kFwdTeamLdsBytes, p.C);
        }, p.pipe, a.bf16 && !p.diag, a.rowmap != nullptr);
    }
    case GruForm::item:
        e = resident(gru_fwd_item_kernel, 256, 0, grid); if (e != hipSuccess) return e;
        hipLaunchKernelGGL(gru_fwd_item_kernel, dim3(grid), dim3(256), 0, st, a);
        return hipGetLastError();
    default:
        return launch<true>(st, a, grid, true);
    }
}

hipError_t gru_backward(hipStream_t st, const GruArgs& a, bool persistent)
{
    int grid; hipError_t e = check(a, &grid); if (e != hipSuccess) return e;
    const GruPlan p = gru_plan(a, false, persistent);
    e = check_operands(a, p, false); if (e != hipSuccess) return e;
    switch (p.form) {
    case GruForm::team_rs:
        hipLaunchKernelGGL(gru_prepare_kernel, dim3(2048), dim3(256), 0, st, a.counters, kGruSyncWords,
                           reinterpret_cast<uint4*>(a.xbuf), gru_bwd_rs_xbuf_floats(a.njobs, p.Bg) / 4);
        e = hipGetLastError(); if (e != hipSuccess) return e;
        return gru_bwd_rs_launch(st, a, p);
    case GruForm::team: {
        e = prepare_exchange(st, a, false, p); if (e != hipSuccess) return e;
        return team_dispatch(p.T, [&](auto T, auto PIPE, auto BF, auto CMP) {
            if constexpr (kDiagBuild && !BF && !CMP) if (p.diag) return launch_team(st, gru_bwd_team_kernel<2, PIPE, T, true>, a, kBwdTeamLdsBytes, p.C);
            return launch_team(st, gru_bwd_team_kernel<2, PIPE, T, false, BF, CMP>, a, kBwdTeamLdsBytes, p.C);
        }, p.pipe, a.bf16 && !p.diag, a.rowmap != nullptr);
    }
    case GruForm::persistent:
        e = prepare_exchange(st, a, false, p); if (e != hipSuccess) return e;
        return launch<false>(st, a, grid, true);
    default:
        break;
    }
    for (int q = a.p_end - 1; q >= a.p_begin; --q) {
        GruArgs b = a; b.p_begin = q; b.p_end = q + 1;
        for (int i = 0; i < b.njobs; ++i) b.job[i].dh0 = nullptr;
        e = launch<false>(st, b, grid, false); if (e != hipSuccess) return e;
        if (q == 0) {
            bool any = false; for (int i = 0; i < a.njobs; ++i) any |= a.job[i].dh0 != nullptr;
            if (any) {
                GruArgs d = a; d.p_begin = 0; d.p_end = 0;
                e = launch<false>(st, d, grid, false); if (e != hipSuccess) return e;
            }
        }
    }
    return hipSuccess;
}

}
```

### argsim_amd/csrc/gru_dev.h

```cpp
#pragma once
#include <type_traits>
#include "kernels.h"
#include "mfma_tile.h"

namespace avae {

typedef unsigned short u16x2 __attribute__((ext_vector_type(2)));
__device__ __forceinline__ unsigned xch16_index(int pos, int row, int k, int B, int K)
{
    return ((((unsigned)pos * (unsigned)(B >> 4) + (unsigned)(row >> 4)) * (unsigned)(K >> 3) + (unsigned)(k >> 3)) * 16u + (unsigned)(row & 15)) * 8u + (unsigned)(k & 7);
}
__device__ __forceinline__ unsigned short bf16_not_sentinel(float v)
{
    const unsigned short h = (unsigned short)(pack_bf16(v, 0.f) & 0xffffu);
    return h == 0xffffu ? (unsigned short)0x7fc0u : h;
}
__device__ __forceinline__ unsigned pk_max_u16(unsigned a, unsigned b)
{
    return __builtin_bit_cast(unsigned, __builtin_elementwise_max(__builtin_bit_cast(u16x2, a), __builtin_bit_cast(u16x2, b)));
}
__device__ __forceinline__ bool any_half_sentinel(unsigned mx) { return (mx & 0xffffu) == 0xffffu || (mx >> 16) == 0xffffu; }
__device__ __forceinline__ float opnd(float x, bool bf) { return bf ? __uint_as_float(pack_bf16(0.f, x)) : x; }
__device__ __forceinline__ bf16x8 pack_bf16x8(const u32x4& p0, const u32x4& p1)
{
// ... 125 lines not shown
#pragma unroll
    for (int q = 0; q < NQ; ++q) mx = max(max(mx, max(v[q].x, v[q].y)), max(v[q].z, v[q].w));
    return __any(mx == kSentinel);
}
template <int NQ>
__device__ __forceinline__ void frag_ensure(u32x4 (&v)[NQ], __amdgpu_buffer_rsrc_t rs, unsigned off, int* err)
{
    if (frag_bad<NQ>(v)) {
        SpinGuard sg;
        do { frag_issue<NQ>(v, rs, off); } while (frag_bad<NQ>(v) && !sg.expired(err));
    }
}
template <int NQ>
__device__ __forceinline__ void frag_ensure(u32x4 (&v)[NQ], __amdgpu_buffer_rsrc_t rs, unsigned off, int* err, unsigned qstride)
{
    if (frag_bad<NQ>(v)) {
        SpinGuard sg;
        do { frag_issue<NQ>(v, rs, off, qstride); } while (frag_bad<NQ>(v) && !sg.expired(err));
    }
}
template <int NQ>
__device__ __forceinline__ bool frag_bad16(const u32x4 (&v)[NQ])
{
    unsigned mx = 0u;
#pragma unroll
    for (int q = 0; q < NQ; ++q) {
        const unsigned a = __builtin_bit_cast(unsigned, __builtin_elementwise_max(__builtin_bit_cast(unsigned short __attribute__((ext_vector_type(2))), v[q].x), __builtin_bit_cast(unsigned short __attribute__((ext_vector_type(2))), v[q].y)));
        const unsigned b = __builtin_bit_cast(unsigned, __builtin_elementwise_max(__builtin_bit_cast(unsigned short __attribute__((ext_vector_type(2))), v[q].z), __builtin_bit_cast(unsigned short __attribute__((ext_vector_type(2))), v[q].w)));
        const unsigned c = __builtin_bit_cast(unsigned, __builtin_elementwise_max(__builtin_bit_cast(unsigned short __attribute__((ext_vector_type(2))), a), __builtin_bit_cast(unsigned short __attribute__((ext_vector_type(2))), b)));
        mx = __builtin_bit_cast(unsigned, __builtin_elementwise_max(__builtin_bit_cast(unsigned short __attribute__((ext_vector_type(2))), mx), __builtin_bit_cast(unsigned short __attribute__((ext_vector_type(2))), c)));
    }
    return __any((mx & 0xffffu) == 0xffffu || (mx >> 16) == 0xffffu);
}
template <int NQ>
__device__ __forceinline__ void frag_ensure16(u32x4 (&v)[NQ], __amdgpu_buffer_rsrc_t rs, unsigned off, int* err, unsigned qstride)
{
    if (frag_bad16<NQ>(v)) {
        SpinGuard sg;
        do { frag_issue<NQ>(v, rs, off, qstride); } while (frag_bad16<NQ>(v) && !sg.expired(err));
    }
}

typedef int i32x4 __attribute__((ext_vector_type(4)));
template <int OFF>
__device__ __forceinline__ void asm_issue6(u32x4 (&v)[6], unsigned voff, i32x4 srd)
{
    asm volatile("buffer_load_dwordx4 %0, %6, %7, 0 offen offset:%c8 sc1\n\t"
                 "buffer_load_dwordx4 %1, %6, %7, 0 offen offset:%c9 sc1\n\t"
                 "buffer_load_dwordx4 %2, %6, %7, 0 offen offset:%c10 sc1\n\t"
                 "buffer_load_dwordx4 %3, %6, %7, 0 offen offset:%c11 sc1\n\t"
                 "buffer_load_dwordx4 %4, %6, %7, 0 offen offset:%c12 sc1\n\t"
                 "buffer_load_dwordx4 %5, %6, %7, 0 offen offset:%c13 sc1"
                 : "=&v"(v[0]), "=&v"(v[1]), "=&v"(v[2]), "=&v"(v[3]), "=&v"(v[4]), "=&v"(v[5])
                 : "v"(voff), "s"(srd), "i"(OFF), "i"(OFF + 64), "i"(OFF + 128), "i"(OFF + 192), "i"(OFF + 256), "i"(OFF + 320)
                 : "memory");
}
__device__ __forceinline__ void asm_issue6x(u32x4 (&v)[6], unsigned voff, i32x4 srd, int soff0, int soff1)
{
    asm volatile("buffer_load_dwordx4 %0, %6, %7, %8 offen offset:0 sc1\n\t"
                 "buffer_load_dwordx4 %1, %6, %7, %8 offen offset:1024 sc1\n\t"
                 "buffer_load_dwordx4 %2, %6, %7, %8 offen offset:2048 sc1\n\t"
                 "buffer_load_dwordx4 %3, %6, %7, %8 offen offset:3072 sc1\n\t"
                 "buffer_load_dwordx4 %4, %6, %7, %9 offen offset:0 sc1\n\t"
                 "buffer_load_dwordx4 %5, %6, %7, %9 offen offset:1024 sc1"
                 : "=&v"(v[0]), "=&v"(v[1]), "=&v"(v[2]), "=&v"(v[3]), "=&v"(v[4]), "=&v"(v[5])
                 : "v"(voff), "s"(srd), "s"(soff0), "s"(soff1)
                 : "memory");
}
template <int N>
__device__ __forceinline__ void asm_wait6(u32x4 (&v)[6])
{
    asm volatile("s_waitcnt vmcnt(%c6)" : "+v"(v[0]), "+v"(v[1]), "+v"(v[2]), "+v"(v[3]), "+v"(v[4]), "+v"(v[5]) : "i"(N) : "memory");
}

template <int N, int NKS>
__device__ __forceinline__ void load_frag_scalar(float* dst, const float* base, int ks0, int kh, bool poll, int* err)
{
    SpinGuard sg;
    for (;;) {
        unsigned v[N]; bool bad = false;
#pragma unroll
        for (int i = 0; i < N; ++i) { v[i] = load4_sc1(base + kperm<NKS>(ks0 + i, kh)); bad |= v[i] == kSentinel; }
        if (!poll || !__any(bad) || sg.expired(err)) {
#pragma unroll
            for (int i = 0; i < N; ++i) dst[i] = __uint_as_float(v[i]);
            return;
        }
    }
}

__device__ __forceinline__ void xcd_publish(unsigned* ctr2, unsigned* ids, int ht)
{
    if (threadIdx.x == 0) {
        const unsigned my = __builtin_amdgcn_s_getreg((31 << 11) | 20) & 0xfu;
        __hip_atomic_store(ids + ht, my + 1u, __ATOMIC_RELAXED, __HIP_MEMORY_SCOPE_AGENT);
        asm volatile("s_waitcnt vmcnt(0)" ::: "memory");
        __hip_atomic_fetch_add(ctr2, 1u, __ATOMIC_RELAXED, __HIP_MEMORY_SCOPE_AGENT);
    }
}
__device__ __forceinline__ bool group_same_xcd(unsigned* ctr2, unsigned* ids, int ht, int HT, int* err, int force_slow, bool published = false)
{
    __shared__ int s_fast;
    if (threadIdx.x < 64) {
        const unsigned my = __builtin_amdgcn_s_getreg((31 << 11) | 20) & 0xfu;
        bool ok = true;
        if (threadIdx.x == 0) {
            if (!published) {
            __hip_atomic_store(ids + ht, my + 1u, __ATOMIC_RELAXED, __HIP_MEMORY_SCOPE_AGENT);
            asm volatile("s_waitcnt vmcnt(0)" ::: "memory");
            __hip_atomic_fetch_add(ctr2, 1u, __ATOMIC_RELAXED, __HIP_MEMORY_SCOPE_AGENT);
            }
            SpinGuard sg;
            while (__hip_atomic_load(ctr2, __ATOMIC_RELAXED, __HIP_MEMORY_SCOPE_AGENT) < (unsigned)HT)
                if (sg.expired(err)) { ok = false; break; }
        }
        ok = __all(ok);
        bool same = true;
        for (int i = threadIdx.x; i < HT; i += 64)
            same = same && __hip_atomic_load(ids + i, __ATOMIC_RELAXED, __HIP_MEMORY_SCOPE_AGENT) == my + 1u;
        same = __all(same) && ok && !force_slow;
        if (threadIdx.x == 0) s_fast = same ? 1 : 0;
    }
    __syncthreads();
    return s_fast != 0;
}

__device__ __forceinline__ bool wg_map(const GruArgs& a, int HT, int* jb, int* g, int* ht)
{
    const int per_job = a.G * HT, bid = blockIdx.x;
    const int alt = (bid >> 3) & 1, idx = ((bid >> 4) << 3) | (bid & 7);
    if (a.njobs == 2 && (per_job & 7) == 0) {
        *jb = alt; *g = idx % a.G; *ht = idx / a.G;
        return alt != 0;
    }
    if (a.njobs == 1 && a.G == 16) {
        *jb = 0; *g = (bid & 7) + 8 * alt; *ht = bid >> 4;
        return alt != 0;
    }
    *jb = bid / per_job;
    const int rem = bid - *jb * per_job;
    *g = rem % a.G; *ht = rem / a.G;
    return false;
}

__device__ __forceinline__ unsigned xch_index(int pos, int row, int k, int B, int K)
{
    return ((((unsigned)pos * (unsigned)(B >> 4) + (unsigned)(row >> 4)) * (unsigned)(K >> 2) + (unsigned)(k >> 2)) * 16u + (unsigned)(row & 15)) * 4u + (unsigned)(k & 3);
}
__device__ __forceinline__ unsigned xch_lane_offset(int pos, int row0, int kc0, int n, int kh, int B, int K)
{
    return ((((unsigned)pos * (unsigned)(B >> 4) + (unsigned)(row0 >> 4)) * (unsigned)(K >> 2) + (unsigned)(kc0 + kh)) * 16u + (unsigned)n) * 16u;
}

__device__ __forceinline__ void team_barrier(unsigned* word, unsigned target)
{
    asm volatile("s_waitcnt lgkmcnt(0)" ::: "memory");
    if ((threadIdx.x & 63) == 0) __hip_atomic_fetch_add(word, 1u, __ATOMIC_RELAXED, __HIP_MEMORY_SCOPE_WORKGROUP);
    while (__hip_atomic_load(word, __ATOMIC_RELAXED, __HIP_MEMORY_SCOPE_WORKGROUP) < target) __builtin_amdgcn_s_sleep(1);
    __builtin_amdgcn_fence(__ATOMIC_ACQUIRE, "workgroup");
}


struct TeamMap { int cid, ht, jb, slot, cpj, nrb; };
__device__ __forceinline__ TeamMap team_map(const GruArgs& a, int rows_per_block)
{
    TeamMap m;
    const int C = gridDim.x / 32;
    m.cid = blockIdx.x % C; m.ht = blockIdx.x / C;
    m.cpj = C / a.njobs;
    m.jb = m.cid / m.cpj; m.slot = m.cid % m.cpj;
    m.nrb = ((a.Bx > a.B ? a.Bx : a.B) / rows_per_block) / m.cpj;
    return m;
}

__device__ __forceinline__ int team_steps(const int* slens, int row0, int lane)
{
    int v = slens[row0 + (lane & 15)];
#pragma unroll
    for (int o = 1; o < 16; o <<= 1) v = max(v, __shfl_xor(v, o, 64));
    return __builtin_amdgcn_readfirstlane(v);
}

template <class K>
static hipError_t resident(K kernel, int threads, int dyn_lds, int grid)
{
    struct Entry { const void* k; int threads, lds, cap; };
    static Entry cache[32]; static int ncache = 0;
    const void* kp = reinterpret_cast<const void*>(kernel);
    for (int i = 0; i < ncache; ++i)
        if (cache[i].k == kp && cache[i].threads == threads && cache[i].lds == dyn_lds)
            return grid <= cache[i].cap ? hipSuccess : hipErrorCooperativeLaunchTooLarge;
    int per_cu = 0, dev = 0, cus = 0;
    hipError_t e = hipOccupancyMaxActiveBlocksPerMultiprocessor(&per_cu, kernel, threads, (size_t)dyn_lds);
    if (e == hipSuccess) e = hipGetDevice(&dev);
    if (e == hipSuccess) e = hipDeviceGetAttribute(&cus, hipDeviceAttributeMultiprocessorCount, dev);
    if (e != hipSuccess) return e;
    const int cap = per_cu * cus;
    if (ncache < 32) cache[ncache++] = Entry{kp, threads, dyn_lds, cap};
    return grid <= cap ? hipSuccess : hipErrorCooperativeLaunchTooLarge;
}

template <class K>
static hipError_t launch_team(hipStream_t st, K kernel, const GruArgs& a, int lds_bytes, int C)
{
    static const void* attr_done[64]; static int nattr = 0;
    const void* kp = reinterpret_cast<const void*>(kernel);
    bool seen = false;
    for (int i = 0; i < nattr; ++i) seen |= attr_done[i] == kp;
    if (!seen) {
        hipError_t e = hipFuncSetAttribute(kp, hipFuncAttributeMaxDynamicSharedMemorySize, lds_bytes);
        if (e != hipSuccess) return e;
        if (nattr < 64) attr_done[nattr++] = kp;
    }
    const int grid = C * 32;
    hipError_t e = resident(kernel, 1024, lds_bytes, grid);
    if (e != hipSuccess) return e;
    hipLaunchKernelGGL(kernel, dim3(grid), dim3(1024), lds_bytes, st, a);
    return hipGetLastError();
}

template <class F>
static hipError_t with_flags(F&& f) { return f(); }
template <class F, class... Bs>
static hipError_t with_flags(F&& f, bool b, Bs... rest)
{
    return b ? with_flags([&](auto... c) { return f(std::true_type{}, c...); }, rest...)
             : with_flags([&](auto... c) { return f(std::false_type{}, c...); }, rest...);
}
template <class F, class... Bs>
static hipError_t team_dispatch(int T, F&& f, Bs... flags)
{
    return T == 4 ? with_flags([&](auto... c) { return f(std::integral_constant<int, 4>{}, c...); }, flags...)
                  : with_flags([&](auto... c) { return f(std::integral_constant<int, 2>{}, c...); }, flags...);
}

}
```

### argsim_amd/csrc/handle.cpp

```cpp
#include "ctx.h"

using namespace avae;
using namespace avae::host;

static std::string g_create_err;

namespace avae { namespace host {

int grow_scratch(avae_ctx* h, size_t need, const char* what)
{
    if (h->scratch_n >= (int64_t)need) return 0;
    AV_CHECK(hipStreamSynchronize(h->stream));
    if (h->scratch) AV_CHECK(hipFree(h->scratch));
    h->scratch = nullptr; h->scratch_n = 0;
    if (hipMalloc(reinterpret_cast<void**>(&h->scratch), need) != hipSuccess) {
        (void)hipGetLastError();
        h->scratch = nullptr;
        char b_[256]; snprintf(b_, sizeof b_, "%s: %.0f MB of scratch could not be allocated on the device", what, (double)need / 1048576.0);
        return fail(h, b_);
    }
    h->scratch_n = (int64_t)need;
    return 0;
}

// ... 68 lines not shown

int check_gru_err(avae_ctx* h)
{
    int e = 0;
    AV_CHECK(hipMemcpyAsync(&e, h->errw, sizeof(int), hipMemcpyDeviceToHost, h->stream));
    AV_CHECK(hipStreamSynchronize(h->stream));
    if (e) {
        (void)hipMemsetAsync(h->errw, 0, sizeof(int), h->stream);
        return fail(h, "GRU persistent kernel: an exchange wait timed out -- its workgroups were not all resident at once.  A persistent "
                       "launch needs every CU of the device (one handle = one GPU = one process, include/argsim_vae.h): another process or "
                       "stream computing on this GPU holds CUs the launch is waiting for.  Give the handle the device to itself, or "
                       "run with avae_set_option(\"persistent\", 0) (one launch per time step)");
    }
    return 0;
}
int dyn_fraction(avae_ctx* h, const avae_ctx::Stamp& s, std::vector<std::pair<const int*, int>>& seen, double* f)
{
    *f = 1.0;
    if (!s.dyn || s.dyn_max <= 0) return 0;
    int c = -1;
    for (auto& e : seen) if (e.first == s.dyn) c = e.second;
    if (c < 0) {
        AV_CHECK(hipMemcpy(&c, s.dyn, sizeof(int), hipMemcpyDeviceToHost));
        if (c < 0) c = 0;
        seen.push_back({s.dyn, c});
    }
    *f = (double)std::min(c, s.dyn_max) / (double)s.dyn_max;
    return 0;
}

}}

extern "C" {

int avae_create(const avae_config* cfg, int device, avae_handle* out)
{
    if (!cfg || !out) { g_create_err = "null argument"; return 1; }
    *out = nullptr;
    if (!gru_dim_supported(cfg->dim_emb)) { g_create_err = "dim_emb must be one of 16, 32, 64, 128, 256, 512 (the GRU kernels are instantiated for these widths only; the reference leaves dim_emb free, config.json uses 512)"; return 1; }
    if (cfg->compute_dtype < 0 || cfg->compute_dtype > 2) { g_create_err = "compute_dtype must be 0 (fp32 MFMA), 1 (bf16 GEMM operands) or 2 (fp32 via split bf16 MFMA)"; return 1; }
    if (cfg->dim_rep % 4 || cfg->dim_tgt % 4 || cfg->rnn_layers < 1 || cfg->rnn_layers > 8) { g_create_err = "dim_rep and dim_tgt must be multiples of 4 (16-byte rows); 1 <= rnn_layers <= 8"; return 1; }
    int ndev = 0;
    if (hipGetDeviceCount(&ndev) != hipSuccess || ndev <= 0) { g_create_err = "no HIP device available: the gfx950 kernels cannot run (no CPU fallback)"; return 1; }
    if (device < 0 || device >= ndev) { g_create_err = "bad device index"; return 1; }
    avae_ctx* h = new avae_ctx();
    h->cfg = *cfg; h->device = device;
    if (h->cfg.kl_beta == 0.f) h->cfg.kl_beta = 1.f;
    build_params(h);
    hipError_t e = hipSetDevice(device);
    if (e == hipSuccess) e = hipMalloc(reinterpret_cast<void**>(&h->losses), 64 * sizeof(float));
    if (e == hipSuccess) e = hipMalloc(reinterpret_cast<void**>(&h->errw), 128 * sizeof(int));
    if (e == hipSuccess) e = hipMalloc(reinterpret_cast<void**>(&h->counters), 2048 * sizeof(unsigned));
    if (e == hipSuccess) e = hipMemset(h->losses, 0, 64 * sizeof(float));
    if (e == hipSuccess) e = hipMemset(h->errw, 0, 128 * sizeof(int));
    if (e == hipSuccess) e = hipMemset(h->counters, 0, 2048 * sizeof(unsigned));
    if (e != hipSuccess) { g_create_err = std::string("hip init failed: ") + hipGetErrorString(e); delete h; return 1; }
    h->acc = h->losses + 8;
    *out = h;
    return 0;
}

void avae_destroy(avae_handle h)
{
    if (!h) return;
    (void)hipSetDevice(h->device);
    if (h->stream) (void)hipStreamSynchronize(h->stream); else (void)hipDeviceSynchronize();
    if (h->ws) (void)hipFree(h->ws);
    if (h->losses) (void)hipFree(h->losses);
    if (h->errw) (void)hipFree(h->errw);
    if (h->hint_host) (void)hipHostFree(const_cast<int32_t*>(h->hint_host));
    if (h->counters) (void)hipFree(h->counters);
    if (h->scratch) (void)hipFree(h->scratch);
    if (h->bfA) (void)hipFree(h->bfA);
    if (h->slab) (void)hipFree(h->slab);
    if (h->bfP) (void)hipFree(h->bfP);
    if (h->bfB) (void)hipFree(h->bfB);
    if (h->lock_fd >= 0) (void)close(h->lock_fd);
    delete h;
}

const char* avae_last_error(avae_handle h) { return h ? h->err.c_str() : g_create_err.c_str(); }

int avae_set_stream(avae_handle h, void* s) { if (!h) return 1; h->stream = reinterpret_cast<hipStream_t>(s); return 0; }

int avae_get_dims(avae_handle h, int32_t* V, int32_t* D, int32_t* R, int32_t* L)
{
    if (!h) return 1;
    if (V) *V = h->cfg.dim_tgt; if (D) *D = h->cfg.dim_emb; if (R) *R = h->cfg.dim_rep; if (L) *L = h->cfg.rnn_layers;
    return 0;
}

int64_t avae_state_numel(avae_handle h) { return h ? h->numel : 0; }

int avae_bind_state(avae_handle h, float* p, float* g, float* m, float* v)
{
    if (!h) return 1;
    if (((uintptr_t)p | (uintptr_t)g | (uintptr_t)m | (uintptr_t)v) & 15) return fail(h, "state buffers must be 16-byte aligned");
    h->P = p; h->G = g; h->M = m; h->Vv = v;
    return 0;
}

int avae_param_count(avae_handle h) { return h ? (int)h->params.size() : 0; }
const char* avae_param_name(avae_handle h, int i) { return (h && i >= 0 && i < (int)h->params.size()) ? h->params[i].name.c_str() : nullptr; }

int avae_param_info(avae_handle h, const char* name, int64_t* offset, int32_t* ndim, int64_t shape[4])
{
    if (!h) return 1;
    const ParamEntry* e = find_param(h, name);
    if (!e) return fail(h, std::string("unknown variable: ") + (name ? name : "(null)"));
    if (offset) *offset = e->offset; if (ndim) *ndim = e->ndim;
    if (shape) for (int i = 0; i < 4; ++i) shape[i] = e->shape[i];
    return 0;
}

static int xfer_tensor(avae_handle h, const char* name, int kind, float* buf, bool get)
{
    if (!h) return 1;
    AV_TRY(check_bound(h));
    const ParamEntry* e = find_param(h, name);
    if (!e) return fail(h, std::string("unknown variable: ") + (name ? name : "(null)"));
    float* base = state_buf(h, kind);
    if (!base) return fail(h, "bad tensor kind");
    float* flat = base + e->offset;
    int64_t n = e->shape[0] * e->shape[1] * e->shape[2] * e->shape[3];
    if (!e->g16) {
        AV_CHECK(hipMemcpyAsync(get ? buf : flat, get ? flat : buf, n * sizeof(float), hipMemcpyDeviceToDevice, h->stream));
    } else {
        int D = h->cfg.dim_emb, cols = (int)(e->ndim == 2 ? e->shape[1] : 1);
        if (get) AV_CHECK(g16_permute(h->stream, buf, flat, D, cols, false));
        else     AV_CHECK(g16_permute(h->stream, flat, buf, D, cols, true));
    }
    return 0;
}
int avae_get_tensor(avae_handle h, const char* name, int kind, float* buf) { return xfer_tensor(h, name, kind, buf, true); }
int avae_set_tensor(avae_handle h, const char* name, int kind, const float* buf) { return xfer_tensor(h, name, kind, const_cast<float*>(buf), false); }

int avae_get_step(avae_handle h, int64_t* s) { if (!h || !s) return 1; *s = h->step; return 0; }
int avae_set_step(avae_handle h, int64_t s) { if (!h) return 1; h->step = s; return 0; }

int avae_set_grad_hook(avae_handle h, avae_grad_hook hook, void* user) { if (!h) return 1; h->hook = hook; h->hook_user = user; return 0; }

int avae_set_option(avae_handle h, const char* key, int value)
{
    if (!h || !key) return 1;
    if (!strcmp(key, "persistent")) { h->persistent = value; return 0; }
    if (!strcmp(key, "gru_item")) { h->gru_item = value; return 0; }
    if (!strcmp(key, "gru_stagger")) { h->gru_stagger = value; return 0; }
    if (!strcmp(key, "gru_force_slow")) { h->gru_force_slow = value; return 0; }
    if (!strcmp(key, "gru_bf16")) { h->gru_bf16 = value != 0; return 0; }
    if (!strcmp(key, "bwd_rs")) { h->bwd_rs = value; return 0; }
    if (!strcmp(key, "dyn_split")) { h->dyn_split = value != 0; return 0; }
    if (!strcmp(key, "shared_device")) { h->shared_device = value != 0; return 0; }
    if (!strcmp(key, "gru_spec")) { h->gru_spec = value; return 0; }
    if (!strcmp(key, "bf16_nt8")) { h->bf16_nt8 = value != 0; return 0; }
    if (!strcmp(key, "logits16")) { h->logits16 = value != 0; return 0; }
    if (!strcmp(key, "bf16_direct")) { h->bf16_direct = value != 0; return 0; }
    if (!strcmp(key, "bf16_tn")) { h->bf16_tn = value != 0; return 0; }
    if (!strcmp(key, "bf16_sv")) { h->bf16_sv = value != 0; return 0; }
    if (!strcmp(key, "bf16_act")) { h->bf16_act = value != 0; return 0; }
    if (!strcmp(key, "table_l1")) { h->table_l1 = value != 0; return 0; }
    if (!strcmp(key, "enc_top1")) { h->enc_top1 = value != 0; return 0; }
    if (!strcmp(key, "dyn_thin")) { h->dyn_thin = value != 0; return 0; }
    if (!strcmp(key, "skip_pad")) { h->skip_pad = value != 0; return 0; }
    if (!strcmp(key, "compact")) { h->compact = value; return 0; }
    if (!strcmp(key, "skinny")) { h->skinny = value; return 0; }
    if (!strcmp(key, "knn_chunk")) { if (value < 0) return fail(h, "knn_chunk must be >= 0"); h->knn_chunk = value; return 0; }
    if (!strcmp(key, "agg_chunk")) { if (value < 0) return fail(h, "agg_chunk must be >= 0"); h->agg_chunk = value; return 0; }
    if (!strcmp(key, "ward_form")) { if (value < 0 || value > 2) return fail(h, "ward_form must be 0 (planner), 1 (one-workgroup) or 2 (launch-per-merge)"); h->ward_form = value; return 0; }
    if (!strcmp(key, "probe_chunk")) { if (value < 0) return fail(h, "probe_chunk must be >= 0"); h->probe_chunk = value; return 0; }
    if (!strcmp(key, "gru_ablate")) {
        if (value && !gru_diag_build()) return fail(h, "gru_ablate needs the diagnostic build of libargsim_vae.so (make -C argsim_amd/csrc DIAG=1)");
        h->gru_ablate = value; return 0;
    }
    if (!strcmp(key, "timing")) { h->timing = value; h->timing_on = value; h->stamps_used = 0; return 0; }
    if (!strcmp(key, "timing_pause")) { h->timing = value ? 0 : h->timing_on; return 0; }
    return fail(h, "unknown option");
}
int avae_timing_collect(avae_handle h, double* out)
{
    if (!h || !out) return 1;
    AV_CHECK(hipStreamSynchronize(h->stream));
    for (int i = 0; i < 9; ++i) out[i] = 0.0;
    std::vector<std::pair<const int*, int>> seen;
    for (size_t i = 0; i < h->stamps_used; ++i) {
        float ms = 0.f;
        AV_CHECK(hipEventElapsedTime(&ms, h->stamps[i].a, h->stamps[i].b));
        double f = 1.0;
        AV_TRY(dyn_fraction(h, h->stamps[i], seen, &f));
        int c = h->stamps[i].cls;
        out[3 * c] += ms; out[3 * c + 1] += 1.0; out[3 * c + 2] += h->stamps[i].flops * f;
    }
    h->stamps_used = 0;
    return 0;
}
int avae_bucket_count(avae_handle h) { return h ? (int)h->buckets.size() : 0; }
int avae_bucket_info(avae_handle h, int i, int64_t* offset, int64_t* count)
{
    if (!h || i < 0 || i >= (int)h->buckets.size()) return 1;
    *offset = h->buckets[i].first; *count = h->buckets[i].second; return 0;
}

}
```

### argsim_amd/csrc/hooks.cpp

```cpp
#include "ctx.h"

using namespace avae;
using namespace avae::host;

extern "C" {

int avae_debug_team_batch(int32_t B) { return B > 0 ? gru_team_batch(B) : 0; }
int avae_debug_gemm_plan(const int32_t* in, int32_t n, int32_t* out)
{
    if (!in || !out || n < 0) return 1;
    for (int r = 0; r < n; ++r, in += 19, out += 15) {
        const GemmShape s{in[0] != 0, in[1] != 0, in[2], in[3], in[4], in[5], in[6], in[7], in[8], in[9], in[10], in[11] != 0, in[12] != 0,
                          in[13] != 0, in[14] != 0, in[15], in[16] != 0, in[17] != 0, in[18] != 0};
        const GemmPlan p = gemm_plan(s);
        out[0] = p.n;
        for (int i = 0; i < 2; ++i) {
            const GemmLaunch l = i < p.n ? p.launch[i] : GemmLaunch{0, 0, 0, 0, 0, 0, 0};
            const int32_t f[7] = {l.row0, l.rows, l.thin, l.split_k, l.accumulate, l.zero, l.dyn};
            std::copy(f, f + 7, out + 1 + 7 * i);
        }
    }
    return 0;
}
int avae_debug_gemm_call(avae_handle h, int a_mc, int b_nc, const float* A, const float* Bm, float* Cm, const float* bias, int M, int N, int K,
// ... 64 lines not shown
    if (!h || !out || !n_out) return 1;
    if (h->B < 1) return fail(h, "avae_debug_train_ce: no training forward has run on this handle");
    Ws w;
    AV_TRY(get_ws(h, w, h->B, h->Ss, h->St, true));
    int n = 0;
    AV_CHECK(hipMemcpyAsync(&n, w.ntok, sizeof(int), hipMemcpyDeviceToHost, h->stream));
    AV_CHECK(hipStreamSynchronize(h->stream));
    n = std::min(n, (int)max_n);
    AV_CHECK(hipMemcpyAsync(out, w.loss_samp, (size_t)n * sizeof(float), hipMemcpyDeviceToDevice, h->stream));
    *n_out = n;
    return 0;
}
int avae_debug_timing(avae_handle h, double* out, int max_n, int* n)
{
    if (!h || !out || !n) return 1;
    AV_CHECK(hipStreamSynchronize(h->stream));
    *n = (int)std::min<size_t>(h->stamps_used, (size_t)max_n);
    std::vector<std::pair<const int*, int>> seen;
    for (int i = 0; i < *n; ++i) {
        float ms = 0.f;
        AV_CHECK(hipEventElapsedTime(&ms, h->stamps[i].a, h->stamps[i].b));
        double f = 1.0;
        AV_TRY(dyn_fraction(h, h->stamps[i], seen, &f));
        const double fl = h->stamps[i].flops * f;
        out[3 * i] = h->stamps[i].cls; out[3 * i + 1] = ms; out[3 * i + 2] = fl;
    }
    return 0;
}
int avae_debug_stamps(avae_handle h, unsigned long long* out)
{
    if (!h || !out) return 1;
    AV_CHECK(hipStreamSynchronize(h->stream));
    AV_CHECK(hipMemcpy(out, h->errw + 16, 32 * sizeof(unsigned long long), hipMemcpyDeviceToHost));
    AV_CHECK(hipMemset(h->errw + 16, 0, 32 * sizeof(unsigned long long)));
    return 0;
}
int avae_debug_gemm(avae_handle h, int a_mc, int b_nc, const float* A, const float* Bm, float* Cm, const float* bias,
                    int M, int N, int K, int lda, int ldb, int ldc, float alpha, int accumulate, int split_k)
{
    if (!h) return 1;
    GemmCall c{A, lda, a_mc != 0, Bm, ldb, b_nc != 0, Cm, ldc, M, N, K};
    c.alpha = alpha; c.bias = bias; c.accumulate = accumulate;
    return gemm(h, c.form(split_k == -3 ? 3 : (split_k < 0 ? 1 : (split_k >= 1000 ? 2 : 0)), split_k < 0 ? 1 : (split_k >= 1000 ? split_k - 1000 : split_k)));
}
int avae_debug_gemm_dyn(avae_handle h, const float* A, const float* Bm, float* Cm, int M, int N, int K, const int* rows)
{
    if (!h) return 1;
    return gemm(h, nt(A, K, Bm, K, Cm, N, M, N, K).rows(rows).form(0));
}
int avae_debug_gemm_c16(avae_handle h, const float* A, const float* Bm, unsigned short* C16, int M, int N, int K, float alpha, const int* rows)
{
    if (!h) return 1;
    if (h->cfg.compute_dtype != 1 || !gemm_bf16_c16_takes(M, N, K, rows, h->bf16_nt8)) return 3;
    GemmCall c = nt(A, K, Bm, K, nullptr, N, M, N, K).scaled(alpha).rows(rows).form(0);
    c.c16 = C16;
    return gemm(h, c);
}
int avae_debug_gemm_tn16(avae_handle h, const float* A, const float* Bm, float* Cm, int M, int N, int K, int lda, int ldb, int ldc, float alpha)
{
    if (!h) return 1;
    return gemm_tn16(h, tn_grad(A, lda, Bm, ldb, Cm, ldc, M, N, K).scaled(alpha));
}
int avae_debug_softmax_ce(avae_handle h, float* logits, unsigned short* panel, int logits16, const int32_t* gold, const int32_t* cidx,
                          const int32_t* n_dev, int n_max, int V, int write_grad, float inv_n, float* loss_samp, float* errt,
                          int32_t* pred, int* form_out)
{
    if (!h || !form_out) return 1;
    CeArgs c{};
    c.logits = logits; c.gold = gold; c.cidx = cidx; c.n_dev = n_dev; c.n_max = n_max; c.V = V;
    c.write_grad = write_grad; c.inv_n = inv_n;
    c.loss_samp = loss_samp; c.errt_samp = errt; c.pred = pred; c.loss_acc = nullptr;
    c.grad16 = panel; c.logits16 = logits16;
    *form_out = softmax_ce_form(c);
    AV_CHECK(softmax_ce(h->stream, c));
    return 0;
}
int avae_debug_argmax_rows(avae_handle h, const float* logits, int32_t* pred, int n, int V)
{
    if (!h) return 1;
    AV_CHECK(argmax_rows(h->stream, logits, pred, n, V));
    return 0;
}
int avae_debug_op_layout(int64_t n, int64_t V, int64_t out[6])
{
    if (!out || n < 0 || V < 0) return 1;
    int32_t base[1];
    out[0] = (int64_t)embed_scatter_scratch_ints((size_t)n, (size_t)V);
    out[1] = (int64_t)id_groups_ints((size_t)n, (size_t)V);
    out[2] = id_groups_rank(base, (int)n, (int)V) - base;
    out[3] = id_groups_uid(base, (int)n, (int)V) - base;
    out[4] = id_groups_count(base, (int)n, (int)V) - base;
    out[5] = id_groups_supported((int)V) ? 1 : 0;
    return 0;
}
int avae_debug_op(avae_handle h, const char* op, void* const* p, const int64_t* i, const float* f)
{
    if (!h || !op || !p || !i || !f) return 1;
    const std::string o(op);
    hipStream_t st = h->stream;
    auto F = [&](int k) { return static_cast<float*>(p[k]); };
    auto I = [&](int k) { return static_cast<int32_t*>(p[k]); };
    if (o == "prep_ids") {
        PrepArgs a{};
        a.src = I(0); a.tgt = I(1); a.keep_mask = static_cast<const uint8_t*>(p[2]); a.src_tm = I(3); a.lens_src = I(4); a.lens_tgt = I(5);
        a.lead = I(6); a.gold = I(7); a.rank = I(8); a.cidx = I(9); a.ntok = I(10); a.zero2 = F(11); a.chunk_counts = I(12);
        a.B = (int)i[0]; a.Ss = (int)i[1]; a.St = (int)i[2]; a.eos = (int)i[3]; a.bos = (int)i[4]; a.train = (int)i[5]; a.seed = (uint64_t)i[6];
        a.keepwd = f[0];
        AV_CHECK(prep_ids(st, a));
    } else if (o == "embed_gather") AV_CHECK(embed_gather(st, F(0), I(1), F(2), (int)i[0], (int)i[1], (int)i[2]));
    else if (o == "embed_scatter_add2") AV_CHECK(embed_scatter_add2(st, F(0), I(1), F(2), (int)i[0], I(3), F(4), (int)i[1], (int)i[2], (int)i[3], I(5)));
    else if (o == "id_groups_build") AV_CHECK(id_groups_build(st, I(0), (int)i[0], (int)i[1], I(1), i[2] != 0));
    else if (o == "rank_rows") AV_CHECK(rank_rows(st, I(0), I(1), I(2), (int)i[0], (int)i[1]));
    else if (o == "rows_gather_ranked") AV_CHECK(rows_gather_ranked(st, F(0), F(1), I(2), I(3), (int)i[0], (int)i[1], (int)i[2]));
    else if (o == "rows_group_sum") AV_CHECK(rows_group_sum(st, F(0), I(1), F(2), (int)i[0], (int)i[1], (int)i[2], I(3)));
    else if (o == "rows_add_indexed") AV_CHECK(rows_add_indexed(st, F(0), F(1), I(2), I(3), (int)i[0], (int)i[1]));
    else if (o == "rows_gather") AV_CHECK(rows_gather(st, F(0), F(1), I(2), I(3), (int)i[0], (int)i[1], I(4)));
    else if (o == "rows_expand") AV_CHECK(rows_expand(st, F(0), F(1), I(2), (int)i[0], (int)i[1], I(3)));
    else if (o == "zero_rows_dyn") AV_CHECK(zero_rows_dyn(st, F(0), I(1), (int)i[0], (int)i[1]));
    else if (o == "zero_fill") AV_CHECK(zero_fill(st, p[0], (size_t)i[0]));
    else if (o == "row_order") {
        RowOrder ro[4];
        const int n = (int)i[0];
        for (int k = 0; k < std::min(n, 4); ++k) ro[k] = RowOrder{I(3 * k), (int)i[5 + 3 * k], (int)i[6 + 3 * k], (int)i[7 + 3 * k], I(3 * k + 1), I(3 * k + 2)};
        AV_CHECK(row_order(st, ro, n, (int)i[1], (int)i[2], (int)i[3], I(3 * std::min(std::max(n, 0), 4)), (int)i[4]));
    } else if (o == "row_map") AV_CHECK(row_map(st, I(0), (int)i[0], (int)i[1], (int)i[2], I(1), I(2), I(3)));
    else if (o == "pick_last") AV_CHECK(pick_last(st, F(0), F(1), I(2), (int)i[0], (int)i[1], I(3)));
    else if (o == "pick_last16") AV_CHECK(pick_last16(st, F(0), static_cast<const unsigned short*>(p[1]), I(2), (int)i[0], (int)i[1], I(3)));
    else if (o == "pick_last_add") AV_CHECK(pick_last_add(st, F(0), F(1), I(2), (int)i[0], (int)i[1], I(3)));
    else if (o == "pick_last_bwd") AV_CHECK(pick_last_bwd(st, F(0), F(1), I(2), (int)i[0], (int)i[1], (int)i[2]));
    else if (o == "latent_fwd") AV_CHECK(latent_fwd(st, F(0), F(1), F(2), F(3), F(4), F(5), (int)i[0], (int)i[1], (uint64_t)i[2], f[0], F(6)));
    else if (o == "latent_bwd") AV_CHECK(latent_bwd(st, F(0), F(1), F(2), F(3), F(4), F(5), (int)i[0], (int)i[1], f[0], f[1]));
    else if (o == "colsum") AV_CHECK(colsum(st, F(0), (int)i[0], (int)i[1], (int)i[2], F(1), I(2)));
    else if (o == "add3") AV_CHECK(add3(st, F(0), F(1), F(2), F(3), i[0]));
    else if (o == "finalize_losses") AV_CHECK(finalize_losses(st, F(0), F(1), I(2), (int)i[0], F(3), (int)i[1], f[0], f[1], f[2]));
    else if (o == "adam_tf") {
        const AdamArgs a{F(0), F(1), F(2), F(3), i[0], f[0], f[1], f[2], f[3], static_cast<const int*>(p[4])};
        AV_CHECK(adam_tf(st, a));
    } else if (o == "g16_permute") AV_CHECK(g16_permute(st, F(0), F(1), (int)i[0], (int)i[1], i[2] != 0));
    else if (o == "gru_first_step_fwd") AV_CHECK(gru_first_step_fwd(st, F(0), F(1), F(2), (int)i[0], F(3), (int)i[1], (int)i[2], I(4)));
    else if (o == "gru_first_step_bwd") AV_CHECK(gru_first_step_bwd(st, F(0), (int)i[0], F(1), F(2), F(3), (int)i[1], (int)i[2], I(4)));
    else return fail(h, "avae_debug_op: no such launcher: " + o);
    return 0;
}

static void gru_shape(const int64_t* i, GruArgs& a)
{
    a.njobs = (int)i[0]; a.S = (int)i[1]; a.B = (int)i[2]; a.D = (int)i[3]; a.ldg = (int)i[4]; a.ldh = (int)i[5]; a.Bx = (int)i[6];
    a.G = (int)i[7]; a.rows_per_group = (int)i[8]; a.p_begin = (int)i[9]; a.p_end = (int)i[10]; a.item_pipeline = (int)i[11];
    a.bf16 = (int)i[12]; a.bwd_rs = (int)i[13]; a.xbuf_floats = (size_t)std::max<int64_t>(i[14], 0);
    if (a.G == 0 && a.D >= 16 && a.njobs >= 1 && a.B >= 1) gru_geometry(a.D, a.njobs, a.B, &a.G, &a.rows_per_group);
}
static void gru_plan_out(const GruArgs& a, const GruPlan& p, int64_t out[10])
{
    const int64_t v[10] = {(int64_t)p.form, p.T, p.C, p.cpj, p.Bg, p.pipe, a.G, a.rows_per_group, (int64_t)gru_bwd_rs_xbuf_floats(a.njobs, p.Bg), 0};
    std::copy(v, v + 10, out);
}
int avae_debug_gru_plan(const int64_t* i, int fwd, int persistent, int64_t out[10])
{
    if (!i || !out) return 1;
    alignas(16) static float dummy[4] = {0.f, 0.f, 0.f, 0.f};
    GruArgs a{};
    gru_shape(i, a);
    a.xbuf = a.xbuf_floats > 0 ? dummy : nullptr;
    gru_plan_out(a, gru_plan(a, fwd != 0, persistent != 0), out);
    return 0;
}
int avae_debug_gru(avae_handle h, int fwd, int persistent, const int64_t* i, void* const* jobs, void* const* shared, int64_t plan_out[10])
{
    if (!h || !i || !jobs || !shared || !plan_out) return 1;
    GruArgs a{};
    gru_shape(i, a);
    if (a.njobs < 1 || a.njobs > kMaxGruJobs) return fail(h, "avae_debug_gru: njobs in 1..3");
    if (a.p_begin != 0 || a.p_end != a.S) return fail(h, "avae_debug_gru: whole-sequence launches only (p_begin = 0, p_end = S)");
    a.stagger = (int)i[15]; a.force_slow = (int)i[16]; a.sv16 = (int)i[17]; a.spec = (int)i[18];
    for (int k = 0; k < a.njobs; ++k) {
        void* const* p = jobs + 19 * k;
        auto F = [&](int q) { return static_cast<float*>(p[q]); };
        auto H = [&](int q) { return static_cast<unsigned short*>(p[q]); };
        GruJob& j = a.job[k];
        j.gi = F(0); j.gi_rows = static_cast<const int32_t*>(p[1]); j.R = F(2); j.bR = F(3); j.h0 = F(4); j.hs = F(5); j.sv = F(6); j.hp = F(7);
        j.hs16 = H(8); j.hp16 = H(9); j.dh_out = F(10); j.dgi = F(11); j.dgh = F(12); j.dgi16 = H(13); j.dgh16 = H(14); j.dh0 = F(15);
        j.carry = F(16); j.dbW = F(17); j.dbR = F(18);
        j.reverse = (int)i[19 + 2 * k]; j.dgi_by_pos = (int)i[20 + 2 * k];
    }
    a.lens = static_cast<const int*>(shared[0]); a.slens = static_cast<const int*>(shared[1]); a.perm = static_cast<const int*>(shared[2]);
    a.rowmap = static_cast<const int*>(shared[3]); a.xbuf = static_cast<float*>(shared[4]);
    a.counters = h->counters; a.err = h->errw; a.stamps = reinterpret_cast<unsigned long long*>(h->errw + 16); a.ablate = 0;
    gru_plan_out(a, gru_plan(a, fwd != 0, persistent != 0), plan_out);
    AV_CHECK(hipSetDevice(h->device));
    AV_GRU(fwd ? gru_forward(h->stream, a, persistent != 0) : gru_backward(h->stream, a, persistent != 0));
    return check_gru_err(h);
}

int avae_debug_sample_rows(avae_handle h, const float* logits, int n, int V, int t0, const avae_sample_config* sc, int32_t* pred, float* logp)
{
    if (!h) return 1;
    SampleParams sp{};
    if (!sample_params(h, sc, V, &sp)) return 1;
    if (n < 1 || V < 1 || t0 < 0 || t0 >= (1 << 20)) return fail(h, "sample rows: bad shape or step");
    AV_CHECK(sample_rows(h->stream, logits, n, V, t0, sp, nullptr, h->cfg.eos, pred, logp));
    return 0;
}

int avae_debug_sample_rows_p(avae_handle h, const float* logits, int n, int V, int t0, const avae_sample_p_config* sc, int32_t* pred, float* logp,
                             int32_t* nkept, const int32_t* lead)
{
    if (!h) return 1;
    SampleParams sp{};
    float top_p = 0.f;
    if (!sample_params_p(h, sc, V, &sp, &top_p)) return 1;
    if (n < 1 || V < 1 || t0 < 0 || t0 >= (1 << 20)) return fail(h, "sample rows: bad shape or step");
    if (top_p > 0.f) AV_CHECK(sample_rows_p(h->stream, logits, n, V, t0, sp, top_p, lead, h->cfg.eos, pred, logp, nkept));
    else {
        AV_CHECK(sample_rows(h->stream, logits, n, V, t0, sp, lead, h->cfg.eos, pred, logp));
        if (nkept) AV_CHECK(hipMemsetAsync(nkept, 0xff, (size_t)n * sizeof(int32_t), h->stream));
    }
    return 0;
}

int avae_debug_beam_select(avae_handle h, const float* logits, int n, int width, int V, const float* cum, const int32_t* fin,
                           int32_t* parent, int32_t* token, float* cum_out, int32_t* fin_out)
{
    if (!h) return 1;
    if (!logits || !cum || !fin || !parent || !token || !cum_out || !fin_out) return fail(h, "beam select: every array must be given");
    if (n < 1 || n > (1 << 20) || V < 1 || width < 1 || width > 32 || width > V) return fail(h, "beam select: bad shape or width");
    AV_CHECK(hipSetDevice(h->device));
    const size_t rows = (size_t)n * width;
    float *cand_sc, *lat_cum; int32_t *cand_tok, *cand_cnt, *len_out, *live;
    AV_TRY(place_scratch(h, "beam select", [&](Bump& b) {
        cand_sc = b.take<float>(rows * width); lat_cum = b.take<float>(rows);
        cand_tok = b.take<int32_t>(rows * width); cand_cnt = b.take<int32_t>(rows); len_out = b.take<int32_t>(rows); live = b.take<int32_t>(1);
    }));
    AV_CHECK(beam_rows(h->stream, logits, (int)rows, V, width, cum, fin, h->cfg.eos, cand_sc, cand_tok, cand_cnt));
    BeamStep a{};
    a.n = n; a.Win = width; a.W = width; a.eos = h->cfg.eos;
    a.cand_sc = cand_sc; a.cand_tok = cand_tok; a.cand_cnt = cand_cnt; a.fin_in = fin; a.len_in = nullptr;
    a.lat_parent = parent; a.lat_token = token; a.lat_cum = lat_cum; a.cum_out = cum_out; a.fin_out = fin_out; a.len_out = len_out;
    a.live = live;
    AV_CHECK(hipMemsetAsync(a.live, 0, sizeof(int32_t), h->stream));
    AV_CHECK(beam_select(h->stream, a));
    return 0;
}

}
```

### argsim_amd/csrc/kernels.h

```cpp
#pragma once
#include <hip/hip_runtime.h>
#include <stdint.h>

#include "gemm_plan.h"

namespace avae {

struct GemmArgs {
    const float* A; const float* B; float* C; const float* bias;
    int M, N, K, lda, ldb, ldc;
    float alpha;
    int accumulate;
    int split_k;
    const int* dyn; int dyn_kind;
    int dyn_expect;
    int thin;
    const float* A2; const float* B2; float* C2; const float* bias2;
    float* slab = nullptr; size_t slab_floats = 0;
    unsigned short* c16 = nullptr;
    int nt8 = 1;
};
hipError_t gemm_f32(hipStream_t st, bool a_mc, bool b_nc, const GemmArgs& g);
struct GemmF32Form { int tile; bool fast, db, persist; unsigned gx, gy, gz; hipError_t err; };
GemmF32Form gemm_f32_form(bool a_mc, bool b_nc, const GemmArgs& g);
hipError_t gemm_f32s(hipStream_t st, bool a_mc, bool b_nc, const GemmArgs& g);
hipError_t gemm_bf16_direct(hipStream_t st, bool a_mc, bool b_nc, const GemmArgs& g);

hipError_t cvt_bf16(hipStream_t st, const float* src, int ld, bool transpose, int rows_or_K, int cols_or_X,
                    unsigned short* dst, int ldd);
hipError_t gemm_bf16_nt(hipStream_t st, const unsigned short* A, int lda, const unsigned short* B, int ldb, const GemmArgs& g);
bool gemm_bf16_p8_ok(const GemmArgs& g, int lda, int ldb);
hipError_t gemm_bf16_p8(hipStream_t st, const unsigned short* A, int lda, const unsigned short* B, int ldb, const GemmArgs& g, int s2);
bool gemm_bf16_c16_ok(const GemmArgs& g, int lda, int ldb);
bool gemm_bf16_c16_takes(int M, int N, int K, const int* rows, int nt8);
bool gemm_bf16_p8_tn_ok(const GemmArgs& g, int lda, int ldb);
hipError_t gemm_bf16_p8_tn(hipStream_t st, const unsigned short* A, int lda, const unsigned short* B, int ldb, const GemmArgs& g, int s2);
hipError_t gemm_bf16_tn(hipStream_t st, const unsigned short* A, int lda, const unsigned short* B, int ldb, const GemmArgs& g);
hipError_t transpose_bf16(hipStream_t st, const unsigned short* src, int ld, int K, int X, unsigned short* dst, int ldk);

constexpr int kMaxGruJobs = 3;
struct GruJob {
    const float* gi;
    const int32_t* gi_rows;
    const float* R;
    const float* bR;
    const float* h0;
    float* hs;
    float* sv;
    float* hp;
    int reverse;
    unsigned short* hs16;
    unsigned short* hp16;
    const float* dh_out;
    float* dgi;
    float* dgh;
    unsigned short* dgi16;
    unsigned short* dgh16;
    float* dh0;
    float* carry;
    int dgi_by_pos;
    float* dbW;
    float* dbR;
};
struct GruArgs {
    GruJob job[kMaxGruJobs];
    int njobs, S, B, D, ldg, ldh;
    const int* lens;
    const int* slens;
    const int* perm;
    const int* rowmap;
    int Bx;
    int G;
    int rows_per_group;
    int p_begin, p_end;
    unsigned* counters;
    int* err;
    unsigned long long* stamps;
    int item_pipeline;
    float* xbuf;
    size_t xbuf_floats;
    int stagger;
    int force_slow;
    int sv16;
    int bf16;
    int spec;
    int bwd_rs;
    int ablate;
};
enum class GruForm { stepwise, persistent, item, team, team_rs };
struct GruPlan {
    GruForm form;
    int T, C, cpj, Bg;
    bool pipe, diag;
    bool team() const { return form == GruForm::team || form == GruForm::team_rs; }
    bool full() const { return team() && !diag; }
};
GruPlan gru_plan(const GruArgs& a, bool fwd, bool persistent);
hipError_t gru_forward(hipStream_t st, const GruArgs& a, bool persistent);
hipError_t gru_backward(hipStream_t st, const GruArgs& a, bool persistent);
int gru_team_batch(int B);
bool gru_dim_supported(int D);
size_t gru_bwd_rs_xbuf_floats(int njobs, int rows);
hipError_t gru_bwd_rs_launch(hipStream_t st, const GruArgs& a, const GruPlan& p);
hipError_t gru_first_step_fwd(hipStream_t st, const float* gi, const float* bR, float* h_out, int ldo, float* sv, int B, int D, const int32_t* lens = nullptr);
hipError_t gru_first_step_bwd(hipStream_t st, const float* dh, int ldd, const float* sv, float* dgi, float* dgh, int B, int D, const int32_t* lens = nullptr);
bool gru_diag_build();

struct PrepArgs {
    const int32_t* src; const int32_t* tgt;
    int B, Ss, St, eos, bos;
    int train; float keepwd; uint64_t seed; const uint8_t* keep_mask;
    int32_t* src_tm;
    int32_t* lens_src;
    int32_t* lens_tgt;
    int32_t* lead;
    int32_t* gold;
    int32_t* rank;
    int32_t* cidx;
    int32_t* ntok;
    float* zero2;
    int32_t* chunk_counts;
};
constexpr int kPrepChunks = 1024;
hipError_t prep_ids(hipStream_t st, const PrepArgs& p);

hipError_t embed_gather(hipStream_t st, const float* E, const int32_t* ids, float* out, int n, int D, int V);
hipError_t embed_scatter_add2(hipStream_t st, float* dE, const int32_t* ids0, const float* dout0, int n0, const int32_t* ids1,
                              const float* dout1, int n1, int D, int V, int32_t* scratch);
bool id_groups_supported(int V);
inline size_t id_groups_ints(size_t n, size_t V) { return 4 * V + 2 + n + (n / 32 + V + 1) + 2 * V + 4; }
hipError_t id_groups_build(hipStream_t st, const int32_t* ids, int n, int V, int32_t* scratch, bool lists);
const int32_t* id_groups_rank(int32_t* scratch, int n, int V);
const int32_t* id_groups_uid(int32_t* scratch, int n, int V);
const int32_t* id_groups_count(int32_t* scratch, int n, int V);
hipError_t rank_rows(hipStream_t st, int32_t* out, const int32_t* ids, const int32_t* rank, int n, int V);
hipError_t rows_gather_ranked(hipStream_t st, float* dst, const float* src, const int32_t* ids, const int32_t* rank, int n, int W, int V);
hipError_t rows_group_sum(hipStream_t st, float* dst, const int32_t* ids, const float* src, int n, int W, int V, int32_t* scratch);
hipError_t rows_add_indexed(hipStream_t st, float* dst, const float* src, const int32_t* uid, const int32_t* nuniq, int n_max, int D);
inline size_t embed_scatter_scratch_ints(size_t n, size_t V) { return 4 * V + 2 + n + (n / 32 + V + 1); }
struct RowOrder { const int32_t* lens; int add, T, cpj; int32_t* perm; int32_t* slens; };
hipError_t row_order(hipStream_t st, const RowOrder* orders, int n, int Breal, int B, int S, int32_t* steps_sum = nullptr, int sum_rows = 0);
hipError_t rows_gather(hipStream_t st, float* dst, const float* src, const int32_t* idx, const int32_t* n_dev, int n_max, int D, const int32_t* map = nullptr);
hipError_t rows_expand(hipStream_t st, float* dst, const float* src, const int32_t* rank, int rows, int D, const int32_t* map = nullptr);
hipError_t pick_last(hipStream_t st, float* h, const float* hs, const int32_t* lens, int B, int W, const int32_t* map = nullptr);
hipError_t pick_last16(hipStream_t st, float* h, const unsigned short* hs16, const int32_t* lens, int B, int W, const int32_t* map = nullptr);
hipError_t pick_last_add(hipStream_t st, float* dhs, const float* d, const int32_t* lens, int B, int W, const int32_t* map = nullptr);
hipError_t row_map(hipStream_t st, const int32_t* lens, int add, int S, int B, int32_t* map, int32_t* nact, int32_t* count);
hipError_t zero_rows_dyn(hipStream_t st, float* X, const int32_t* count, int rows_max, int W);
hipError_t pick_last_bwd(hipStream_t st, float* dhs, const float* dh, const int32_t* lens, int S, int B, int W);

hipError_t latent_fwd(hipStream_t st, const float* mu, const float* lv, const float* eps_in, float* eps_out, float* z,
                      float* kld, int n, int train, uint64_t seed, float free_bits, float* acc);
hipError_t latent_bwd(hipStream_t st, const float* dz, const float* mu, const float* lv, const float* eps_used,
                      float* dmu, float* dlv, int B, int R, float coef, float free_bits);

struct CeArgs {
    float* logits;
    const int32_t* gold;
    const int32_t* cidx;
    const int32_t* n_dev;
    int n_max, V;
    int write_grad; float inv_n;
    float* loss_samp; float* errt_samp; int32_t* pred;
    float* loss_acc;
    unsigned short* grad16;
    int logits16;
};
int softmax_ce_form(const CeArgs& a);
hipError_t softmax_ce(hipStream_t st, const CeArgs& a);
hipError_t argmax_rows(hipStream_t st, const float* logits, int32_t* pred, int n, int V);
struct SampleParams { float inv_t; int top_k; int noise; uint64_t seed; };
hipError_t sample_rows(hipStream_t st, const float* logits, int n, int V, int t, const SampleParams& sp, const int32_t* lead, int eos,
                       int32_t* pred, float* logp);
hipError_t sample_rows_p(hipStream_t st, const float* logits, int n, int V, int t, const SampleParams& sp, float top_p, const int32_t* lead,
                         int eos, int32_t* pred, float* logp, int32_t* nkept);

hipError_t colsum(hipStream_t st, const float* X, int M, int N, int ldx, float* out, const int32_t* m_dev);
hipError_t add3(hipStream_t st, float* out, const float* a, const float* b, const float* c, int64_t n);
hipError_t zero_fill(hipStream_t st, void* p, size_t bytes);

struct AdamArgs { float* p; const float* g; float* m; float* v; int64_t n; float lr_t, b1, b2, eps;
                  const int* skip_if; };
hipError_t adam_tf(hipStream_t st, const AdamArgs& a);

struct ScoreDraw {
    const float* mu; const float* lv;
    const float* eps_in;
    float* eps_out;
    float* z;
    float* lat;
    int* err;
    int k, B, R, rc; uint64_t seed;
};
hipError_t score_draw(hipStream_t st, const ScoreDraw& a);
hipError_t tile_ids(hipStream_t st, int32_t* dst, const int32_t* src, int n, int rc, int S);
hipError_t lead_rows(hipStream_t st, const int32_t* lead, int T, int n, int rc, int32_t* ids0, int32_t* tokrow);
struct ScoreRows {
    const float* loss;
    const int32_t* rank;
    int T, n, rc, k0, r0, B;
    float* logpx;
    int32_t* ntok;
};
hipError_t score_rows(hipStream_t st, const ScoreRows& a);
hipError_t score_bound(hipStream_t st, const float* logpx, const float* lat, int k, int B, float* logw, float* bound);

hipError_t beam_rows(hipStream_t st, const float* logits, int rows, int V, int W, const float* cum, const int32_t* fin, int eos,
                     float* cand_sc, int32_t* cand_tok, int32_t* cand_cnt);
struct BeamStep {
    int n, Win, W, eos;
    const float* cand_sc; const int32_t* cand_tok; const int32_t* cand_cnt;
    const int32_t* fin_in; const int32_t* len_in;
    int32_t* lat_parent; int32_t* lat_token; float* lat_cum;
    float* cum_out; int32_t* fin_out; int32_t* len_out;
    int32_t* live;
};
hipError_t beam_select(hipStream_t st, const BeamStep& a);
hipError_t beam_gather(hipStream_t st, const float* const* hd, int L, int n, int Win, int W, int D, const int32_t* parent, float* state_out);
struct BeamEnd {
    int n, W, n_run, steps, eos;
    const int32_t* lat_parent; const int32_t* lat_token; const float* lat_cum;
    const float* cum; const int32_t* len;
    const float* lenpow;
    int32_t* out_ids;
    float* score_out; float* cum_out; int32_t* len_out;
    int32_t* o_parent; int32_t* o_token; float* o_cum; size_t out_step;
};
hipError_t beam_backtrack(hipStream_t st, const BeamEnd& a);

struct KnnArgs {
    const float* q; const float* bank;
    int n, N, dim, k, metric;
    int64_t idx_base, self_base; int carry;
    int64_t* out_idx; float* out_score;
};
struct KnnPlan { int qrows, qtiles, parts, chunk; };
KnnPlan knn_plan(int n, int N, int k, int chunk_opt);
size_t knn_ws_bytes(const KnnPlan& p, int n, int N, int k);
hipError_t knn_search(hipStream_t st, const KnnArgs& g, const KnnPlan& p, void* ws);

struct AggArgs {
    const float* z; const float* mu; const float* lv;
    int n, N, dim;
    int64_t self_base;
    float* logq; float* logqx;
};
// ... 76 lines not shown
```

### argsim_amd/csrc/model.cpp

```cpp
#include "ctx.h"

using namespace avae;

namespace avae { namespace host {

static bool phantom_batch(const avae_ctx* h, int B)
{
    return h->compact && h->skip_pad && h->persistent && h->cfg.dim_emb == 512 && gru_team_batch(B) > B;
}
bool use_table(const avae_ctx* h, int rows, int B)
{
    if (!h->table_l1 || !id_groups_supported(h->cfg.dim_tgt)) return false;
    return rows >= h->cfg.dim_tgt || (rows >= 1024 && phantom_batch(h, B));
}

void layout(avae_ctx* h, Bump& b, Ws& w, int B, int Ss, int St, bool train)
{
    const int D = h->cfg.dim_emb, V = h->cfg.dim_tgt, R = h->cfg.dim_rep, L = h->cfg.rnn_layers;
    const size_t T = St + 1, rs = (size_t)Ss * B, rt = T * B;
    w.src_tm = b.take<int32_t>(rs); w.lens_src = b.take<int32_t>(B); w.lens_tgt = b.take<int32_t>(B);
    w.lead = b.take<int32_t>(rt); w.gold = b.take<int32_t>(rt); w.rank = b.take<int32_t>(rt);
    w.cidx = b.take<int32_t>(rt); w.ntok = b.take<int32_t>(4 + kPrepChunks); w.pred = b.take<int32_t>(rt);
    w.emb_src = b.take<float>(rs * D); w.emb_tgt = b.take<float>(rt * D);
    const bool tab_s = use_table(h, (int)rs, B), tab_t = use_table(h, (int)rt, B);
// ... 134 lines not shown
        return gemm_launch(h, two, l);
    }
    const float* A = c.A + (size_t)l.row0 * c.lda; float* C = c.C + (size_t)l.row0 * c.ldc;
    const int M = l.rows, N = c.N, K = c.K;
    const int* dyn = l.dyn ? c.dyn : nullptr; const int dyn_kind = l.dyn ? c.dyn_kind : 0;
    const Pair* pair = c.pair;
    GemmArgs g{A, c.B, C, c.bias, M, N, K, c.lda, c.ldb, c.ldc, c.alpha, l.accumulate, l.split_k, dyn, dyn_kind, dyn_expected(h, dyn, dyn_kind), l.thin,
               pair ? pair->A : nullptr, pair ? pair->B : nullptr, pair ? pair->C : nullptr, pair ? pair->bias : nullptr};
    Timed t(h, 0, 2.0 * M * N * K * (pair ? 2 : 1), dyn, dyn_kind == 1 ? M : (dyn_kind == 2 ? K : 0));
    if (h->cfg.compute_dtype == 1 && h->bf16_direct) {
        AV_CHECK(gemm_bf16_direct(h->stream, c.a_mc, c.b_nc, g));
        return 0;
    }
    if (h->cfg.compute_dtype == 1) {
        const int Kp = (K + 7) & ~7;
        unsigned short* a16 = nullptr;
        if (c.keep_a16 && !c.a_mc && Kp == K) a16 = c.keep_a16 + (size_t)l.row0 * K;
        if (!a16) { AV_TRY(grow_bf16(h, &h->bfA, &h->bfA_cap, (size_t)M * Kp)); a16 = h->bfA; }
        AV_TRY(grow_bf16(h, &h->bfB, &h->bfB_cap, (size_t)N * Kp));
        AV_CHECK(cvt_bf16(h->stream, A, c.lda, c.a_mc, c.a_mc ? K : M, c.a_mc ? M : K, a16, Kp));
        AV_CHECK(cvt_bf16(h->stream, c.B, c.ldb, c.b_nc, c.b_nc ? K : N, c.b_nc ? N : K, h->bfB, Kp));
        g.nt8 = h->bf16_nt8;
        g.c16 = c.c16;
        AV_CHECK(gemm_bf16_nt(h->stream, a16, Kp, h->bfB, Kp, g));
        return 0;
    }
    if (c.c16) return fail(h, "the fp16 output panel exists in compute_dtype 1 only");
    if (h->cfg.compute_dtype == 2 && !l.thin) AV_CHECK(gemm_f32s(h->stream, c.a_mc, c.b_nc, g));
    else AV_CHECK(gemm_f32(h->stream, c.a_mc, c.b_nc, g));
    return 0;
}

int gemm(avae_ctx* h, const GemmCall& c)
{
    const GemmPlan p = gemm_plan(gemm_shape(h, c));
    for (int i = 0; i < p.n; ++i) {
        const GemmLaunch& l = p.launch[i];
        float* C = c.C + (size_t)l.row0 * c.ldc;
        if (l.zero == kZeroAll) AV_CHECK(zero_fill(h->stream, C, sizeof(float) * (size_t)l.rows * c.N));
        if (l.zero == kZeroDynRows) AV_CHECK(zero_rows_dyn(h->stream, C, c.dyn, l.rows, c.N));
        AV_TRY(gemm_launch(h, c, l));
    }
    return 0;
}

static int gemm_bf16_pre(avae_ctx* h, const GemmCall& c)
{
    const GemmLaunch l = bf16_launch(h, c);
    const int M = c.M, N = c.N, K = c.K;
    GemmArgs g{nullptr, c.B, c.C, c.bias, M, N, K, c.lda, c.ldb, c.ldc, c.alpha, l.accumulate, l.split_k, c.dyn, c.dyn_kind, 0, 0, nullptr, nullptr, nullptr, nullptr};
    Timed t(h, 0, 2.0 * M * N * K, c.dyn, c.dyn_kind == 1 ? M : (c.dyn_kind == 2 ? K : 0));
    const int Kp = (K + 7) & ~7;
    const unsigned short* Ap = c.A16; int lda_p = c.lda;
    if (c.a_mc) {
        AV_TRY(grow_bf16(h, &h->bfA, &h->bfA_cap, (size_t)M * Kp));
        AV_CHECK(transpose_bf16(h->stream, c.A16, c.lda, K, M, h->bfA, Kp));
        Ap = h->bfA; lda_p = Kp;
    }
    AV_TRY(grow_bf16(h, &h->bfB, &h->bfB_cap, (size_t)N * Kp));
    AV_CHECK(cvt_bf16(h->stream, c.B, c.ldb, c.b_nc, c.b_nc ? K : N, c.b_nc ? N : K, h->bfB, Kp));
    g.nt8 = h->bf16_nt8;
    AV_CHECK(gemm_bf16_nt(h->stream, Ap, lda_p, h->bfB, Kp, g));
    return 0;
}

int gemm_tn16(avae_ctx* h, const GemmCall& c)
{
    const GemmLaunch l = bf16_launch(h, c);
    const int M = c.M, N = c.N, K = c.K;
    GemmArgs g{nullptr, nullptr, c.C, nullptr, M, N, K, c.lda, c.ldb, c.ldc, c.alpha, l.accumulate, l.split_k, c.dyn, c.dyn_kind, 0, 0, nullptr, nullptr, nullptr, nullptr};
    Timed t(h, 0, 2.0 * M * N * K, c.dyn, c.dyn ? K : 0);
    const unsigned short* A16 = c.A16; const unsigned short* B16 = c.B16;
    int la = c.lda, lb = c.ldb;
    if (!A16) {
        la = (M + 7) & ~7;
        AV_TRY(grow_bf16(h, &h->bfA, &h->bfA_cap, (size_t)K * la));
        AV_CHECK(cvt_bf16(h->stream, c.A, c.lda, false, K, M, h->bfA, la));
        A16 = h->bfA;
    }
    if (!B16) {
        lb = (N + 7) & ~7;
        AV_TRY(grow_bf16(h, &h->bfB, &h->bfB_cap, (size_t)K * lb));
        AV_CHECK(cvt_bf16(h->stream, c.B, c.ldb, false, K, N, h->bfB, lb));
        B16 = h->bfB;
    }
    g.nt8 = h->bf16_nt8;
    if (h->bf16_nt8 && l.split_k > 1) {
        if (!h->slab) {
            const size_t n = (size_t)512 << 16;
            AV_CHECK(hipMalloc(reinterpret_cast<void**>(&h->slab), n * sizeof(float)));
            h->slab_floats = n;
        }
        g.slab = h->slab; g.slab_floats = h->slab_floats;
    }
    AV_CHECK(gemm_bf16_tn(h->stream, A16, la, B16, lb, g));
    return 0;
}
static bool tn16_ok(const avae_ctx* h, int M, int N) { return h->cfg.compute_dtype == 1 && h->bf16_tn && gemm_tn16_shape(M, N); }

void gru_geometry(int D, int njobs, int B, int* G, int* rpg)
{
    int HT = D / 16;
    int gmax = 512 / (njobs * HT); if (gmax < 1) gmax = 1; if (gmax > 16) gmax = 16;
    int g = (B + 15) / 16; if (g > gmax) g = gmax; if (g < 1) g = 1;
    int r = (B + g - 1) / g; r = (r + 15) / 16 * 16;
    g = (B + r - 1) / r;
    *G = g; *rpg = r;
}

struct Sched { float keepwd, anneal, lr; };
static Sched schedule(const avae_ctx* h)
{
    float rate = h->cfg.accelerate * (float)h->step;
    Sched s;
    s.keepwd = 1.f / (1.f + expf(-rate));
    s.anneal = tanhf(rate);
    s.lr = h->cfg.learn_rate / (sqrtf(rate) + 1.f);
    return s;
}

static bool top_one_step(const avae_ctx* h) { return h->enc_top1 && h->cfg.rnn_layers >= 2; }

struct FillHint { int32_t real, rows; };
static FillHint fill_hint(const avae_ctx* h)
{
    const uint64_t pair = h->hint_host ? *reinterpret_cast<const volatile uint64_t*>(h->hint_host) : 0xffffffffull;
    return {(int32_t)(uint32_t)(pair & 0xffffffffull), (int32_t)(uint32_t)(pair >> 32)};
}
static double expected_fill(const avae_ctx* h)
{
    const FillHint f = fill_hint(h);
    return (f.real > 0 && f.rows > 0) ? std::min(1.0, (double)f.real / (double)f.rows) : 1.0;
}
static int rs_pick(const avae_ctx* h)
{
    if (h->bwd_rs != 2) return h->bwd_rs;
    return expected_fill(h) < 0.40 ? 1 : 0;
}
static int spec_pick(const avae_ctx* h)
{
    if (h->gru_spec != 2) return h->gru_spec;
    return expected_fill(h) < 0.60 ? 1 : 0;
}

void gru_common(avae_ctx* h, const Ws& w, GruArgs& a, int njobs, int S, int B, int ldg, int ldh, const int32_t* lens, int Bx)
{
    const int D = h->cfg.dim_emb;
    a.njobs = njobs; a.S = S; a.B = B; a.D = D; a.ldg = ldg; a.ldh = ldh; a.lens = lens;
    a.Bx = Bx;
    gru_geometry(D, njobs, B, &a.G, &a.rows_per_group);
    a.p_begin = 0; a.p_end = S; a.counters = h->counters; a.err = h->errw; a.ablate = h->gru_ablate; a.force_slow = h->gru_force_slow;
    a.bf16 = h->cfg.compute_dtype == 1 && h->gru_bf16; a.stagger = h->gru_stagger; a.item_pipeline = h->gru_item;
    a.xbuf = w.xbuf; a.xbuf_floats = w.xbuf_floats; a.stamps = reinterpret_cast<unsigned long long*>(h->errw + 16); a.bwd_rs = h->bwd_rs != 0;
}
int build_row_orders(avae_ctx* h, Ws& w, int B, int Ss, int T, bool with_dec, bool with_enc)
{
    if (!h->skip_pad || !h->persistent || w.Bx % 16) return 0;
    if (w.Bx != B && !h->compact) return 0;
    const int D = h->cfg.dim_emb;
    RowOrder ord[3]; int n = 0, which[3];
    auto want = [&](int k, int njobs, int S, int ldg, int ldh, const int32_t* lens, int add) {
        GruArgs a{};
        gru_common(h, w, a, njobs, S, B, ldg, ldh, lens, w.Bx);
        const GruPlan p = gru_plan(a, true, true);
        if (p.form != GruForm::team) return;
        ord[n] = RowOrder{lens, add, p.T, p.cpj, w.ord_perm[k], w.ord_slens[k]};
        which[n++] = k; w.ord_T[k] = p.T; w.ord_cpj[k] = p.cpj;
    };
    if (with_enc) want(0, 2, Ss, 6 * D, 2 * D, w.lens_src, 0);
    if (with_enc && top_one_step(h)) want(1, 1, Ss, 6 * D, 2 * D, w.lens_src, 0);
    if (with_dec) want(2, 1, T, 3 * D, D, w.lens_tgt, 1);
    if (!n) return 0;
    const bool hint = which[0] == 0 && h->compact == 2;
    if (hint && !h->hint_host) {
        int32_t* hp = nullptr;
        if (hipHostMalloc(reinterpret_cast<void**>(&hp), 64, hipHostMallocDefault) == hipSuccess) { hp[0] = -1; hp[1] = 0; h->hint_host = hp; }
    }
    h->hint_dev = reinterpret_cast<int32_t*>(h->errw + 100);
    hipError_t e = row_order(h->stream, ord, n, B, w.Bx, std::max(Ss, T), hint ? h->hint_dev : nullptr, Ss * B);
    if (e == hipErrorInvalidValue) return 0;
    AV_CHECK(e);
    if (hint && h->hint_host) {
        AV_CHECK(hipMemcpyAsync(const_cast<int32_t*>(h->hint_host), h->hint_dev, 2 * sizeof(int32_t), hipMemcpyDeviceToHost, h->stream));
    }
    for (int i = 0; i < n; ++i) w.ord_ok[which[i]] = true;
    return 0;
}
static bool both_team_bf16(avae_ctx* h, const GruArgs& a, bool train)
{
    return train && a.bf16 && gru_plan(a, true, h->persistent != 0).full() && gru_plan(a, false, h->persistent != 0).full();
}
static void attach_sv16(avae_ctx* h, GruArgs& a, bool train) { a.sv16 = h->bf16_sv && both_team_bf16(h, a, train); }
static void attach_order(avae_ctx* h, const Ws& w, GruArgs& a, bool fwd, int k)
{
    const GruPlan p = gru_plan(a, fwd, h->persistent != 0);
    if (!w.ord_ok[k] || !p.team() || p.T != w.ord_T[k] || p.cpj != w.ord_cpj[k]) return;
    a.slens = w.ord_slens[k]; a.perm = w.ord_perm[k];
}

static int build_compact(avae_ctx* h, Ws& w, int B, int Ss, int T, bool train)
{
    w.compact = false; w.compact_d = false;
    h->expect_ptr[0] = h->expect_ptr[1] = h->expect_ptr[2] = nullptr;
    if (!h->compact || !h->persistent || Ss < 2 || !use_table(h, Ss * B, B)) return 0;
    const bool phantom = w.Bx != B;
    if (phantom && !(w.ord_ok[0] && (w.ord_ok[1] || !top_one_step(h)))) return 0;
    if (h->compact == 2 && !phantom) {
        const FillHint f = fill_hint(h);
        if (f.real < 0 || f.rows <= 0 || (double)f.real >= 0.92 * (double)f.rows) return 0;
    }
    const int D = h->cfg.dim_emb;
    auto team = [&](int njobs, int S, int ldg, int ldh, const int32_t* lens) {
        GruArgs q{};
        gru_common(h, w, q, njobs, S, B, ldg, ldh, lens, w.Bx);
        return gru_plan(q, true, true).full() && (!train || gru_plan(q, false, true).full());
    };
    if (!team(2, Ss, 6 * D, 2 * D, w.lens_src) || (top_one_step(h) && !team(1, Ss, 6 * D, 2 * D, w.lens_src))) return 0;
    AV_CHECK(row_map(h->stream, w.lens_src, 0, Ss, B, w.map_src, w.nact_src, w.nsrc));
    w.compact = true;
    {
        const FillHint f = fill_hint(h);
        const double fill = (f.real > 0 && f.rows > 0) ? std::min(1.0, (double)f.real / (double)f.rows) : 0.0;
        h->expect_ptr[0] = w.nsrc; h->expect_val[0] = (int)(fill * Ss * B);
        h->expect_ptr[1] = w.ntgt; h->expect_val[1] = (int)(fill * T * B);
        h->expect_ptr[2] = w.ntok; h->expect_val[2] = (int)(fill * T * B);
    }
    if (T < 2 || !use_table(h, T * B, B) || h->compact == 3) return 0;
    if ((phantom && !w.ord_ok[2]) || !team(1, T, 3 * D, D, nullptr)) return 0;
    AV_CHECK(row_map(h->stream, w.lens_tgt, 1, T, B, w.map_tgt, w.nact_tgt, w.ntgt));
    w.compact_d = true;
    return 0;
}
int build_compact_dec(avae_ctx* h, Ws& w, int B, int T)
{
    w.compact = false; w.compact_d = false;
    h->expect_ptr[0] = h->expect_ptr[1] = h->expect_ptr[2] = nullptr;
    if (!h->compact || h->compact == 3 || !h->persistent || T < 2 || !use_table(h, T * B, B)) return 0;
    if (w.Bx == B || !w.ord_ok[2]) return 0;
    GruArgs q{};
    gru_common(h, w, q, 1, T, B, 3 * h->cfg.dim_emb, h->cfg.dim_emb, nullptr, w.Bx);
    if (!gru_plan(q, true, true).full()) return 0;
    AV_CHECK(row_map(h->stream, w.lens_tgt, 1, T, B, w.map_tgt, w.nact_tgt, w.ntgt));
    w.compact_d = true;
    return 0;
}

static int run_encoder(avae_ctx* h, Ws& w, int B, int Ss, bool save)
{
    const int D = h->cfg.dim_emb, V = h->cfg.dim_tgt, L = h->cfg.rnn_layers;
    const int rs = Ss * B;
    const bool table = use_table(h, rs, B);
    h->cnt_src = table ? id_groups_count(w.grp_src, rs, V) : nullptr;
    const int32_t* const cdyn = w.compact ? w.nsrc : nullptr;
    const int32_t* const cmap = w.compact ? w.map_src : nullptr;
    if (!table) AV_CHECK(embed_gather(h->stream, h->P + h->oE, w.src_tm, w.emb_src, rs, D, V));
    const float* x = w.emb_src; int In = D;
    for (int i = 0; i < L; ++i) {
        const GruP& p = h->enc[i];
        const bool top1 = i == L - 1 && top_one_step(h);
        if (i == 0 && table) {
            const int32_t* cnt = id_groups_count(w.grp_src, rs, V);
            AV_CHECK(id_groups_build(h->stream, w.src_tm, rs, V, w.grp_src, save));
            AV_CHECK(rows_gather(h->stream, w.emb_src, h->P + h->oE, id_groups_uid(w.grp_src, rs, V), cnt, std::min(V, rs), D));
            AV_TRY(gemm(h, nt(w.emb_src, D, h->P + p.W, D, w.ew, 6 * D, std::min(V, rs), 6 * D, D).biased(h->P + p.bW).rows(cnt)));
        } else if (i > 0 && w.act_e[i - 1]) {
            AV_TRY(gemm_bf16_pre(h, nt(nullptr, In, h->P + p.W, In, w.e_gi[i], 6 * D, rs, top1 ? 3 * D : 6 * D, In).a16(w.e_hs16[i - 1]).biased(h->P + p.bW).rows(cdyn)));
        } else {
        AV_TRY(gemm(h, nt(x, In, h->P + p.W, In, w.e_gi[i], 6 * D, rs, top1 ? 3 * D : 6 * D, In).biased(h->P + p.bW).rows(cdyn).keep(save ? w.x16_e[i] : nullptr)));
        }
        GruArgs a{};
        gru_common(h, w, a, top1 ? 1 : 2, Ss, B, 6 * D, 2 * D, w.lens_src, w.bx_enc());
        const bool table0 = i == 0 && table, indirect = table0 && gru_plan(a, true, h->persistent != 0).form == GruForm::team;
        if (indirect) AV_CHECK(rank_rows(h->stream, w.tokrow_src, w.src_tm, id_groups_rank(w.grp_src, rs, V), rs, V));
        else if (table0) AV_CHECK(rows_gather_ranked(h->stream, w.e_gi[0], w.ew, w.src_tm, id_groups_rank(w.grp_src, rs, V), rs, 6 * D, V));
        for (int d = 0; d < a.njobs; ++d) {
            GruJob& j = a.job[d];
            j.gi = (indirect ? w.ew : w.e_gi[i]) + d * 3 * D;
            j.gi_rows = indirect ? w.tokrow_src : nullptr;
            j.R = h->P + p.R + (int64_t)d * 3 * D * D;
            j.bR = h->P + p.bR + d * 3 * D;
            j.h0 = nullptr;
            j.hs = w.e_hs[i] + d * D;
            j.sv = save ? w.e_sv[d][i] : nullptr;
            j.hp = save ? w.e_hp[d][i] : nullptr;
            j.reverse = d;
        }
        attach_sv16(h, a, save);
        if (w.e_hs16[i] && tn16_ok(h, 3 * D, D) && both_team_bf16(h, a, save)) {
            w.act_e[i] = 1; w.acth_e[i] = 1;
            for (int d = 0; d < a.njobs; ++d) { a.job[d].hs16 = w.e_hs16[i] + d * D; a.job[d].hp16 = w.e_hp16[d][i]; }
        }
        attach_order(h, w, a, true, top1 ? 1 : 0);
        a.rowmap = cmap;
        a.spec = spec_pick(h);
        { Timed t(h, 1, 2.0 * a.njobs * Ss * (double)B * D * 3 * D);
          DeviceTurn turn(h);
          AV_GRU(gru_forward(h->stream, a, h->persistent != 0)); }
        if (top1) {
            const int64_t oWb = p.W + (int64_t)3 * D * In;
            if (w.act_e[i - 1]) AV_CHECK(pick_last16(h->stream, w.xlast, w.e_hs16[i - 1], w.lens_src, B, In, cmap));
            else
            AV_CHECK(pick_last(h->stream, w.xlast, x, w.lens_src, B, In, cmap));
            AV_TRY(gemm(h, nt(w.xlast, In, h->P + oWb, In, w.gib, 3 * D, B, 3 * D, In).biased(h->P + p.bW + 3 * D).batch_rows()));
        }
        x = w.e_hs[i]; In = 2 * D;
    }
// ... 452 lines not shown
```

Measured before the change: 15630 sentences/sec.

## Use a four-slot ring for GRU team exchange buffers with sentinel rearm

Replaces the per-timestep exchange buffer in the fp32 team GRU forward and backward kernels with a 4-slot ring indexed by step modulo 4. After each step the last k-split wave re-writes sentinels into the slot two steps ahead, so the prepare kernel only has to clear 4 slots instead of S. The goals are to shrink the sentinel-initialisation pass and to keep the exchange buffer small enough to stay cache-resident. In exchange it adds rearm stores inside the recurrent loop and a tighter dependence on step ordering, with possible races if a team runs ahead by more than the ring depth.

```diff
diff --git a/argsim_amd/csrc/ctx.h b/argsim_amd/csrc/ctx.h
--- a/argsim_amd/csrc/ctx.h
+++ b/argsim_amd/csrc/ctx.h
@@ -62,6 +62,7 @@
     int bf16_nt8 = 1;
     int bf16_direct = 0;
     int gru_spec = 2;
+    int gru_ring = 1;
     int bwd_rs = 2;
     int knn_chunk = 0;
     int agg_chunk = 0;
diff --git a/argsim_amd/csrc/gru.hip b/argsim_amd/csrc/gru.hip
--- a/argsim_amd/csrc/gru.hip
+++ b/argsim_amd/csrc/gru.hip
@@ -361,9 +361,10 @@
 
 
 constexpr int kFwdTeamLdsBytes = (96 * 256 + 48 * 256 + 4 * 256) * 4 + 128;
-template <bool DIAG, bool PIPE, int T, bool BF = false, bool CMP = false>
+template <bool DIAG, bool PIPE, int T, bool BF = false, bool CMP = false, bool RING = false>
 __global__ __launch_bounds__(1024, 4) void gru_fwd_team_kernel(GruArgs a)
 {
+    static_assert(!RING || (!PIPE && !BF && !DIAG), "the exchange ring: fp32, one row block per workgroup");
     const int ab = DIAG ? a.ablate : 0;
     constexpr int D = 512, HT = 32, KS = 16 / T, WK = D / KS, NQ = WK / 16, RB = 16 * T;
     extern __shared__ __attribute__((aligned(16))) float lds[];
@@ -414,7 +415,8 @@
     float* __restrict__ p_svw = J.sv;
     float* __restrict__ p_hpw = J.hp;
     float* __restrict__ p_hsw = J.hs;
-    float* const xh = BF ? a.xbuf + (size_t)tm.jb * (a.S + 1) * B * D / 2 : a.xbuf + (size_t)tm.jb * a.S * B * D;
+    constexpr bool ring = RING;
+    float* const xh = BF ? a.xbuf + (size_t)tm.jb * (a.S + 1) * B * D / 2 : a.xbuf + (size_t)tm.jb * (ring ? min(a.S, kGruRing) : a.S) * B * D;
     const __amdgpu_buffer_rsrc_t rs_hs = make_rsrc(xh), rs_h0 = make_rsrc(J.h0 ? J.h0 : xh);
     const __amdgpu_buffer_rsrc_t rs_gi = make_rsrc(p_gi), rs_hsw = make_rsrc(p_hsw);
     const __amdgpu_buffer_rsrc_t rs_svw = make_rsrc(p_svw ? p_svw : p_hsw), rs_hpw = make_rsrc(p_hpw ? p_hpw : p_hsw);
@@ -448,7 +450,7 @@
     auto a_offset = [&](int p, int row0, int len_a) -> unsigned {
         if constexpr (BF) return xch_lane_offset(p == 0 ? 0 : pos_map(p - 1, len_a, J.reverse) + 1, row0, wk * (WK / 8), n, kh, B, D / 2);
         if (p == 0) return (unsigned)((size_t)(CMP ? min(perm ? perm[row0 + n] : row0 + n, Bs - 1) : (perm ? perm[row0 + n] : row0 + n)) * D * 4) + (wk * WK + 4 * kh) * 4;
-        return xch_lane_offset(pos_map(p - 1, len_a, J.reverse), row0, wk * (WK / 4), n, kh, B, D);
+        return xch_lane_offset(ring ? ((p - 1) & (kGruRing - 1)) : pos_map(p - 1, len_a, J.reverse), row0, wk * (WK / 4), n, kh, B, D);
     };
     auto q_stride = [&](int p) -> unsigned { return (p == 0 && !BF) ? 64u : 1024u; };
     auto next_frag = [&](int p2, int r2, int len2) __attribute__((always_inline)) {
@@ -531,7 +533,7 @@
                         const int prow = row0 + 15;
                         const int plen = len_p0;
                         const float* pp = BF ? xh + (xch16_index(pos_map(p - 1, plen, J.reverse) + 1, prow, (lane & 31) * 16 + 15, B, D) >> 1)
-                                             : xh + xch_index(pos_map(p - 1, plen, J.reverse), prow, (lane & 31) * 16 + 15, B, D);
+                                             : xh + xch_index(ring ? ((p - 1) & (kGruRing - 1)) : pos_map(p - 1, plen, J.reverse), prow, (lane & 31) * 16 + 15, B, D);
                         SpinGuard sg;
                         while (__any(BF ? (load4_sc1(pp) >> 16) == 0xffffu : load4_sc1(pp) == kSentinel) && !sg.expired(a.err)) { }
                         }
@@ -633,7 +635,7 @@
                 if constexpr (PIPE) { if (r == 0) hc0 = hnew; else if (r == 1) hc1 = hnew; else if (r == 2) hc2 = hnew; else hc3 = hnew; }
                 else hc = hnew;
             } else {
-                const unsigned xo = xch_index(gpos, grow, j, B, D) * 4u;
+                const unsigned xo = xch_index(ring ? (p & (kGruRing - 1)) : gpos, grow, j, B, D) * 4u;
                 if (fast) bstore1(not_sentinel(hnew), rs_hs, xo); else bstore1_sc1(not_sentinel(hnew), rs_hs, xo);
             }
             if (real) {
@@ -649,6 +651,9 @@
             if (BF && p_hp16) __builtin_amdgcn_raw_buffer_store_b16(to_bf16(hprev), rs_hp16, (int)((rix * D + j) * 2u), 0, 0);
             else if (p_hpw) bstore1(hprev, rs_hpw, (rix * D + j) * 4u);
             }
+        }
+        if constexpr (RING) {
+            if (wk == KS - 1 && p >= 2 && p + 2 < p_stop) xch_rearm<1>(rs_hs, (p + 2) & (kGruRing - 1), row0, ht * 4, lane, B, D, fast);
         }
         len_a = len2; len_g = len2g; ge_cur = ge2;
         TSTAMP(3);
@@ -906,9 +911,10 @@
 }
 
 constexpr int kBwdTeamLdsBytes = (4 * 24 * 256 + 16 * 256 + 64) * 4 + 64;
-template <int NB, bool PIPE, int T, bool DIAG = false, bool BF = false, bool CMP = false>
+template <int NB, bool PIPE, int T, bool DIAG = false, bool BF = false, bool CMP = false, bool RING = false>
 __global__ __launch_bounds__(1024, 4) void gru_bwd_team_kernel(GruArgs a)
 {
+    static_assert(!RING || (!PIPE && !BF && !DIAG), "the exchange ring: fp32, one row block per workgroup");
     unsigned long long ph[8] = {0, 0, 0, 0, 0, 0, 0, 0}, tprev = DIAG ? __builtin_amdgcn_s_memrealtime() : 0ULL;
 #define BSTAMP(i) do { if constexpr (DIAG) { unsigned long long t_ = __builtin_amdgcn_s_memrealtime(); ph[i] += t_ - tprev; tprev = t_; } } while (0)
     constexpr int D = 512, HT = 32, PQ = 6, KS = 16 / T, WKB = 3 * D / KS, KPL = BF ? 32 : 16, NH = WKB / (PQ * KPL), KB4 = 96 / KS, RB = 16 * T;
@@ -984,7 +990,8 @@
     const int* const perm = a.perm;
     int* p_err = a.err;
     const int j_rev = J.reverse, ldg = a.ldg, ldh = a.ldh;
-    float* const xg = a.xbuf + (size_t)tm.jb * S * B * (3 * D) / (BF ? 2 : 1);
+    constexpr bool ring = RING;
+    float* const xg = a.xbuf + (size_t)tm.jb * (ring ? min(S, kGruRing) : S) * B * (3 * D) / (BF ? 2 : 1);
     const unsigned long long pa = (unsigned long long)xg;
     const i32x4 srd = {(int)(unsigned)(pa & 0xffffffffULL), (int)(unsigned)((pa >> 32) & 0xffffULL), -1, 0x00020000};
     float sb_r = 0.f, sb_u = 0.f, sb_n = 0.f, sb_nr = 0.f;
@@ -1004,7 +1011,7 @@
     const __amdgpu_buffer_rsrc_t rs_dgh16 = make_rsrc(reinterpret_cast<const float*>(p_dgh16 ? p_dgh16 : reinterpret_cast<unsigned short*>(p_dghw)));
     auto a_offset = [&](int p, int row0, int len_a) -> unsigned {
         if constexpr (BF) return xch_lane_offset(pos_map(p + 1, len_a, j_rev), row0, wk * (WKB / 8), n, kh, B, 3 * D / 2);
-        return xch_lane_offset(pos_map(p + 1, len_a, j_rev), row0, wk * (WKB / 4), n, kh, B, 3 * D);
+        return xch_lane_offset(ring ? ((done - 1) & (kGruRing - 1)) : pos_map(p + 1, len_a, j_rev), row0, wk * (WKB / 4), n, kh, B, 3 * D);
     };
     auto issue_piece = [&](int piece, u32x4 (&dst)[PQ], unsigned vo) __attribute__((always_inline)) {
         asm_issue6x(dst, vo, srd, 6144 * piece, 6144 * piece + 4096);
@@ -1152,7 +1159,7 @@
             auto probe = [&](SpinGuard& sg) __attribute__((always_inline)) {
                 const int len_p = PIPE ? (j_rev ? p_lens[row0 + 15] : 0) : len_p0;
                 const float* pp = BF ? xg + (xch16_index(pos_map(p + 1, len_p, j_rev), row0 + 15, (ln_l & 31) * 48 + 47, B, 3 * D) >> 1)
-                                     : xg + xch_index(pos_map(p + 1, len_p, j_rev), row0 + 15, (ln_l & 31) * 48 + 47, B, 3 * D);
+                                     : xg + xch_index(ring ? ((done - 1) & (kGruRing - 1)) : pos_map(p + 1, len_p, j_rev), row0 + 15, (ln_l & 31) * 48 + 47, B, 3 * D);
                 for (;;) {
                     unsigned v = 0u;
                     if (ln_l < 32) v = load4_sc1(pp);
@@ -1218,7 +1225,7 @@
                 }
             } else {
                 const float x0 = not_sentinel(dr), x1 = not_sentinel(du), x2 = not_sentinel(dn * r_);
-                const unsigned o0 = xch_index(gpos, grow, ht * 48 + gn_l, B, 3 * D) * 4u;
+                const unsigned o0 = xch_index(ring ? (done & (kGruRing - 1)) : gpos, grow, ht * 48 + gn_l, B, 3 * D) * 4u;
                 if (fast) { bstore1(x0, rs_dgh, o0); bstore1(x1, rs_dgh, o0 + 1024u); bstore1(x2, rs_dgh, o0 + 2048u); }
                 else { bstore1_sc1(x0, rs_dgh, o0); bstore1_sc1(x1, rs_dgh, o0 + 1024u); bstore1_sc1(x2, rs_dgh, o0 + 2048u); }
             }
@@ -1246,6 +1253,9 @@
             if (real || (dgi_by_pos && inb)) bstore3(dr, du, dn, rs_dgi, orow_i);
             }
             sb_r += dr; sb_u += du; sb_n += dn; sb_nr += dn * r_;
+        }
+        if constexpr (RING) {
+            if (wk == KS - 1 && done >= 2 && p >= 2) xch_rearm<3>(rs_dgh, (done + 2) & (kGruRing - 1), row0, ht * 12, lane, B, 3 * D, fast);
         }
         len_a = len2; len_g = len2g; ge_cur = ge2;
         BSTAMP(6);
@@ -1415,9 +1425,12 @@
         return hipGetLastError();
     }
     if (team) {
-        const size_t n16 = (size_t)a.njobs * rows * width / 4;
-        hipLaunchKernelGGL(gru_prepare_kernel, dim3(2048), dim3(256), 0, st, a.counters, kGruSyncWords,
-                           reinterpret_cast<uint4*>(a.xbuf), bf ? n16 / 2 : n16);
+        const size_t slots = p.ring ? (size_t)std::min(a.S, p.ring) : (size_t)a.S;
+        size_t n16 = (size_t)a.njobs * slots * Bg * width / 4;
+        if (bf) n16 /= 2;
+        const size_t blocks = (std::max(n16, (size_t)kGruSyncWords) + 255) / 256;
+        hipLaunchKernelGGL(gru_prepare_kernel, dim3((unsigned)std::min<size_t>(blocks, 2048)), dim3(256), 0, st, a.counters, kGruSyncWords,
+                           reinterpret_cast<uint4*>(a.xbuf), n16);
         return hipGetLastError();
     }
     float* base0 = fwd ? a.job[0].hs : a.job[0].dgh;
@@ -1488,6 +1501,7 @@
     p.T = T; p.C = C; p.cpj = C / a.njobs;
     p.pipe = a.njobs * (p.Bg / (16 * T)) > C;
     p.diag = kDiagBuild && (fwd ? a.ablate != 0 : (a.ablate & 128) != 0);
+    p.ring = (a.ring && p.form == GruForm::team && !p.pipe && !a.bf16 && !p.diag) ? kGruRing : 0;
     return p;
 }
 
@@ -1518,10 +1532,13 @@
     e = prepare_exchange(st, a, true, p); if (e != hipSuccess) return e;
     switch (p.form) {
     case GruForm::team: {
-        return team_dispatch(p.T, [&](auto T, auto PIPE, auto BF, auto CMP) {
-            if constexpr (kDiagBuild && T == 4 && !BF && !CMP) if (p.diag) return launch_team(st, gru_fwd_team_kernel<true, PIPE, 4>, a, kFwdTeamLdsBytes, p.C);
-            return launch_team(st, gru_fwd_team_kernel<false, PIPE, T, BF, CMP>, a, kFwdTeamLdsBytes, p.C);
-        }, p.pipe, a.bf16 && !p.diag, a.rowmap != nullptr);
+        return team_dispatch(p.T, [&](auto T, auto PIPE, auto BF, auto CMP, auto RING) {
+            if constexpr (RING && (PIPE || BF)) return hipErrorInvalidValue;
+            else {
+            if constexpr (kDiagBuild && T == 4 && !BF && !CMP && !RING) if (p.diag) return launch_team(st, gru_fwd_team_kernel<true, PIPE, 4>, a, kFwdTeamLdsBytes, p.C);
+            return launch_team(st, gru_fwd_team_kernel<false, PIPE, T, BF, CMP, RING>, a, kFwdTeamLdsBytes, p.C);
+            }
+        }, p.pipe, a.bf16 && !p.diag, a.rowmap != nullptr, p.ring != 0);
     }
     case GruForm::item:
         e = resident(gru_fwd_item_kernel, 256, 0, grid); if (e != hipSuccess) return e;
@@ -1545,10 +1562,13 @@
         return gru_bwd_rs_launch(st, a, p);
     case GruForm::team: {
         e = prepare_exchange(st, a, false, p); if (e != hipSuccess) return e;
-        return team_dispatch(p.T, [&](auto T, auto PIPE, auto BF, auto CMP) {
-            if constexpr (kDiagBuild && !BF && !CMP) if (p.diag) return launch_team(st, gru_bwd_team_kernel<2, PIPE, T, true>, a, kBwdTeamLdsBytes, p.C);
-            return launch_team(st, gru_bwd_team_kernel<2, PIPE, T, false, BF, CMP>, a, kBwdTeamLdsBytes, p.C);
-        }, p.pipe, a.bf16 && !p.diag, a.rowmap != nullptr);
+        return team_dispatch(p.T, [&](auto T, auto PIPE, auto BF, auto CMP, auto RING) {
+            if constexpr (RING && (PIPE || BF)) return hipErrorInvalidValue;
+            else {
+            if constexpr (kDiagBuild && !BF && !CMP && !RING) if (p.diag) return launch_team(st, gru_bwd_team_kernel<2, PIPE, T, true>, a, kBwdTeamLdsBytes, p.C);
+            return launch_team(st, gru_bwd_team_kernel<2, PIPE, T, false, BF, CMP, RING>, a, kBwdTeamLdsBytes, p.C);
+            }
+        }, p.pipe, a.bf16 && !p.diag, a.rowmap != nullptr, p.ring != 0);
     }
     case GruForm::persistent:
         e = prepare_exchange(st, a, false, p); if (e != hipSuccess) return e;
diff --git a/argsim_amd/csrc/gru_dev.h b/argsim_amd/csrc/gru_dev.h
--- a/argsim_amd/csrc/gru_dev.h
+++ b/argsim_amd/csrc/gru_dev.h
@@ -301,6 +301,20 @@
     return ((((unsigned)pos * (unsigned)(B >> 4) + (unsigned)(row0 >> 4)) * (unsigned)(K >> 2) + (unsigned)(kc0 + kh)) * 16u + (unsigned)n) * 16u;
 }
 
+template <int N16>
+__device__ __forceinline__ void xch_rearm(__amdgpu_buffer_rsrc_t rs, int slot, int row0, int kc0, int lane, int B, int K, bool fast)
+{
+    const unsigned off = ((((unsigned)slot * (unsigned)(B >> 4) + (unsigned)(row0 >> 4)) * (unsigned)(K >> 2) + (unsigned)kc0) * 16u + (unsigned)lane) * 16u;
+    const u32x4 s4 = {kSentinel, kSentinel, kSentinel, kSentinel};
+    if (fast) {
+#pragma unroll
+        for (int i = 0; i < N16; ++i) __builtin_amdgcn_raw_buffer_store_b128(s4, rs, (int)(off + 1024u * i), 0, 0);
+    } else {
+#pragma unroll
+        for (int i = 0; i < N16; ++i) __builtin_amdgcn_raw_buffer_store_b128(s4, rs, (int)(off + 1024u * i), 0, 16);
+    }
+}
+
 __device__ __forceinline__ void team_barrier(unsigned* word, unsigned target)
 {
     asm volatile("s_waitcnt lgkmcnt(0)" ::: "memory");
diff --git a/argsim_amd/csrc/handle.cpp b/argsim_amd/csrc/handle.cpp
--- a/argsim_amd/csrc/handle.cpp
+++ b/argsim_amd/csrc/handle.cpp
@@ -244,6 +244,7 @@
     if (!strcmp(key, "dyn_split")) { h->dyn_split = value != 0; return 0; }
     if (!strcmp(key, "shared_device")) { h->shared_device = value != 0; return 0; }
     if (!strcmp(key, "gru_spec")) { h->gru_spec = value; return 0; }
+    if (!strcmp(key, "gru_ring")) { h->gru_ring = value != 0; return 0; }
     if (!strcmp(key, "bf16_nt8")) { h->bf16_nt8 = value != 0; return 0; }
     if (!strcmp(key, "logits16")) { h->logits16 = value != 0; return 0; }
     if (!strcmp(key, "bf16_direct")) { h->bf16_direct = value != 0; return 0; }
diff --git a/argsim_amd/csrc/hooks.cpp b/argsim_amd/csrc/hooks.cpp
--- a/argsim_amd/csrc/hooks.cpp
+++ b/argsim_amd/csrc/hooks.cpp
@@ -240,7 +240,7 @@
 }
 static void gru_plan_out(const GruArgs& a, const GruPlan& p, int64_t out[10])
 {
-    const int64_t v[10] = {(int64_t)p.form, p.T, p.C, p.cpj, p.Bg, p.pipe, a.G, a.rows_per_group, (int64_t)gru_bwd_rs_xbuf_floats(a.njobs, p.Bg), 0};
+    const int64_t v[10] = {(int64_t)p.form, p.T, p.C, p.cpj, p.Bg, p.pipe, a.G, a.rows_per_group, (int64_t)gru_bwd_rs_xbuf_floats(a.njobs, p.Bg), p.ring};
     std::copy(v, v + 10, out);
 }
 int avae_debug_gru_plan(const int64_t* i, int fwd, int persistent, int64_t out[10])
@@ -249,7 +249,7 @@
     alignas(16) static float dummy[4] = {0.f, 0.f, 0.f, 0.f};
     GruArgs a{};
     gru_shape(i, a);
-    a.xbuf = a.xbuf_floats > 0 ? dummy : nullptr;
+    a.xbuf = a.xbuf_floats > 0 ? dummy : nullptr; a.ring = 1;
     gru_plan_out(a, gru_plan(a, fwd != 0, persistent != 0), out);
     return 0;
 }
@@ -274,6 +274,7 @@
     a.lens = static_cast<const int*>(shared[0]); a.slens = static_cast<const int*>(shared[1]); a.perm = static_cast<const int*>(shared[2]);
     a.rowmap = static_cast<const int*>(shared[3]); a.xbuf = static_cast<float*>(shared[4]);
     a.counters = h->counters; a.err = h->errw; a.stamps = reinterpret_cast<unsigned long long*>(h->errw + 16); a.ablate = 0;
+    a.ring = h->gru_ring;
     gru_plan_out(a, gru_plan(a, fwd != 0, persistent != 0), plan_out);
     AV_CHECK(hipSetDevice(h->device));
     AV_GRU(fwd ? gru_forward(h->stream, a, persistent != 0) : gru_backward(h->stream, a, persistent != 0));
diff --git a/argsim_amd/csrc/kernels.h b/argsim_amd/csrc/kernels.h
--- a/argsim_amd/csrc/kernels.h
+++ b/argsim_amd/csrc/kernels.h
@@ -85,13 +85,16 @@
     int bf16;
     int spec;
     int bwd_rs;
+    int ring;
     int ablate;
 };
+constexpr int kGruRing = 4;
 enum class GruForm { stepwise, persistent, item, team, team_rs };
 struct GruPlan {
     GruForm form;
     int T, C, cpj, Bg;
     bool pipe, diag;
+    int ring;
     bool team() const { return form == GruForm::team || form == GruForm::team_rs; }
     bool full() const { return team() && !diag; }
 };
diff --git a/argsim_amd/csrc/model.cpp b/argsim_amd/csrc/model.cpp
--- a/argsim_amd/csrc/model.cpp
+++ b/argsim_amd/csrc/model.cpp
@@ -310,6 +310,7 @@
     a.p_begin = 0; a.p_end = S; a.counters = h->counters; a.err = h->errw; a.ablate = h->gru_ablate; a.force_slow = h->gru_force_slow;
     a.bf16 = h->cfg.compute_dtype == 1 && h->gru_bf16; a.stagger = h->gru_stagger; a.item_pipeline = h->gru_item;
     a.xbuf = w.xbuf; a.xbuf_floats = w.xbuf_floats; a.stamps = reinterpret_cast<unsigned long long*>(h->errw + 16); a.bwd_rs = h->bwd_rs != 0;
+    a.ring = h->gru_ring;
 }
 int build_row_orders(avae_ctx* h, Ws& w, int B, int Ss, int T, bool with_dec, bool with_enc)
 {
```

After: 16000 sentences/sec (median of 6 runs). 2.4% higher.
